# yflyl613/Tiny-NewsRec

Measured on NVIDIA B200. Metric: kd_train_impressions_per_sec, higher is better.
Workload: dtype bf16

## Files before the change

include/tinyrec.h:

```cpp
#ifndef TINYREC_H_
#define TINYREC_H_

#include <stdint.h>

#ifdef __cplusplus
extern "C" {
#endif

#define TNR_ABI_VERSION 6

const char* tnr_last_error(void);
int tnr_abi_version(void);
int tnr_device_check(int* num_sms);
int tnr_set_sm_reserve(int n_sms);
int tnr_host_copy_mt(void* dst, const void* src, long long bytes, int n_threads);

typedef struct {
  const unsigned long long* seed;
  unsigned int site;
  float p;
} tnr_dropout;

int tnr_dropout_mask(const tnr_dropout* drop, long long n, unsigned char* keep, void* stream);

enum { TNR_ACT_NONE = 0, TNR_ACT_GELU = 1, TNR_ACT_TANH = 2, TNR_ACT_DGELU = 3,
       TNR_ACT_GELU_DAUX = 4,
       TNR_ACT_MULAUX = 5 };
enum { TNR_BF16 = 0, TNR_F32 = 1 };

typedef struct {
  int M, N, K;
  const void* A; int lda; int a_mn_major;
  const void* B; int ldb; int b_mn_major;
  void* C; int ldc; int c_dtype;
  const float* bias;
  const void* residual; int ldr;
  int act;
  void* aux; int ldaux;
  int split_k;
  int accumulate;
  const tnr_dropout* drop;
  float* colsum;
} tnr_gemm_args;
int tnr_gemm_bf16(const tnr_gemm_args* args, void* stream);

int tnr_embed_ln_fwd(const int64_t* ids, int ids_ld, int n_rows, int L, int vocab, const void* word,
                     int word_dtype, const float* pos, const float* type0, const float* gamma,
                     const float* beta, float eps, int E, void* out_bf16, const tnr_dropout* drop,
                     void* stream);

int tnr_layernorm_fwd(const void* x_bf16, int rows, int E, const float* gamma, const float* beta,
                      float eps, void* y_bf16, void* stream);
int tnr_layernorm_bwd(const void* dy_bf16, const void* x_bf16, int rows, int E, const float* gamma,
                      float eps, void* dx_bf16, float* dgamma, float* dbeta, void* dx_drop_bf16,
                      float* dsum, const tnr_dropout* drop, void* stream);
int tnr_colsum_bf16(const void* x_bf16, int rows, int cols, int ld, float* out, void* stream);

int tnr_attn_relpos_fwd(const void* qkv_bf16, const int64_t* mask, int mask_ld, const float* relbias,
                        void* ctx_bf16, int n_news, int L, int A, int E, const tnr_dropout* drop,
                        void* stream);
int tnr_attn_relpos_bwd(const void* qkv_bf16, const int64_t* mask, int mask_ld, const float* relbias,
                        const void* dctx_bf16, void* dqkv_bf16, float* dbias_qkv, float* workspace, int n_news,
                        int L, int A, int E, const tnr_dropout* drop, void* stream);

int tnr_attnpool_fwd(const void* x_bf16, const void* e_bf16, int ldq, int Q, const float* w2,
                     const float* b2, const float* mask, void* out_bf16, float* a_out, int n, int S,
                     int C, void* stream);
int tnr_attnpool_bwd(const void* x_bf16, const void* e_bf16, int ldq, int Q, const float* w2,
                     const float* a_in, const float* dout, void* dx_bf16, void* du_bf16, float* dw2,
                     float* db2, int n, int S, int C, void* stream);

int tnr_user_encoder_fwd(const float* vecs, const float* mask, const float* pad_doc, const float* W1,
                         const float* b1, const float* w2, const float* b2, int use_mask, float* user,
                         float* a_out, float* e_out, int B, int H, int D, int Q, void* stream);
typedef struct {
  const float *vecs, *pad_doc, *W1, *b1, *w2, *b2;
  float *user, *a_out, *e_out;
} tnr_user_encoder_io;
int tnr_user_encoder_fwd_multi(const tnr_user_encoder_io* enc, int n_enc, const float* mask, int use_mask,
                               int B, int H, int D, int Q, void* stream);
int tnr_user_encoder_fwd_gather(const float* table, long long n_rows, const int32_t* idx, const float* mask,
                                const float* pad_doc, const float* W1, const float* b1, const float* w2,
                                const float* b2, int use_mask, float* user, float* a_out, int B, int H, int D,
                                int Q, void* stream);
long long tnr_user_encoder_packed_w1_floats(int D);
int tnr_user_encoder_pack_w1(const float* W1, const float* pad_doc, const float* b1, const float* w2, float* packed,
                             int D, int Q, void* stream);
long long tnr_user_encoder_score_ws_bytes(int B, int H);
int tnr_user_encoder_score(const float* vecs, long long n_rows, const int32_t* idx, const float* mask,
                           const float* pad_doc, const float* w1_packed, const float* b1, const float* w2,
                           const float* b2, int use_mask, float* user, float* a_out, void* workspace, int B,
                           int H, int D, int Q, void* stream);
int tnr_user_encoder_bwd(const float* vecs, const float* mask, const float* pad_doc, const float* W1,
                         const float* w2, int use_mask, const float* a_in, const float* e_in,
                         const float* d_user, float* d_vecs, float* dpad, float* dW1, float* db1,
                         float* dw2, float* db2, float* scratch, int B, int H, int D, int Q, void* stream);

int tnr_kd_loss_fwdbwd(const float* s_news, const float* s_user, const int64_t* label,
                       const float* T_ext, const float* TP_ext, int M, int B, int H, int K, int D,
                       float temperature, float coef, int want_grad, float* score_out, float* losses,
                       float* d_news, float* d_user, float* G_ext, void* stream);

int tnr_sgemm_nt(const float* A, const float* B, const float* bias, float* C, int M, int N, int K,
                 int batch, long long sA, long long sB, long long sbias, long long sC, void* stream);
int tnr_sgemm_tn_acc(const float* A, const float* B, float* C, float* cbias, int R, int N1, int N2,
                     int batch, long long sA, long long sB, long long sC, long long sbias, void* stream);

int tnr_nrms_blend_fwd(const float* vecs, const float* mask, const float* pad_doc, float* out, int rows, int D,
                       void* stream);
int tnr_nrms_blend_bwd(const float* d_blend, const float* mask, float* d_vecs, float* dpad, int rows, int D,
                       void* stream);
int tnr_nrms_attn_fwd(const float* q, const float* k, const float* v, const float* mask, float* ctx, int B, int H,
                      int n_heads, void* stream);
int tnr_nrms_attn_bwd(const float* q, const float* k, const float* v, const float* mask, const float* d_ctx,
                      float* dq, float* dk, float* dv, int B, int H, int n_heads, void* stream);
int tnr_sgemm_nn(const float* A, const float* B, float* C, int M, int N, int K, int parts, long long sA,
                 long long sB, void* stream);

int tnr_adam_amsgrad(float* p, const float* g, float* m, float* v, float* vmax, void* shadow_bf16,
                     long long n, float lr, float beta1, float beta2, float eps, int step,
                     float grad_scale, void* stream);
int tnr_adam_amsgrad_devstep(float* p, const float* g, float* m, float* v, float* vmax, void* shadow_bf16,
                             long long n, float lr, float beta1, float beta2, float eps, int* step_dev,
                             float* bc_ws, float grad_scale, int advance, void* stream);
int tnr_cast_f32_bf16(const float* x, void* y_bf16, long long n, void* stream);

long long tnr_allreduce_p2p_flag_words(void);
int tnr_allreduce_p2p(void* const* ptrs_dev, void* multicast_ptr, void* const* flags_dev, int rank, int world,
                      long long off, long long n, int n_ctas, void* stream);

int tnr_gather_rows_i32_i64(const int32_t* table, long long n_rows_table, const int32_t* idx,
                            long long n, int W, int64_t* out, void* stream);
int tnr_train_batch_gather(const int32_t* news, long long n_rows, int W, const float* const* teacher_tables,
                           float* const* teacher_out, int M, int D, long long out_ld, const int32_t* hist_idx,
                           long long n_hist, const int32_t* cand_idx, long long n_cand, long long* tokens_out,
                           void* stream);
int tnr_gather_rows_f32(const float* table, long long n_rows_table, const int32_t* idx, long long n,
                        int D, float* out, long long out_ld, void* stream);

int tnr_eval_metrics(const float* table, long long n_rows, const float* user, const long long* ptr,
                     const int32_t* cand, const int8_t* label, long long n_imp, long long nnz, int D, int max_c,
                     double* per_imp, double* sums, float* scores, void* stream);

int tnr_doc_sim(const float* table, long long n_rows, const int32_t* pairs, long long n_pairs, int D,
                double* sum_out, void* stream);

#ifdef __cplusplus
}
#endif
#endif
```

tiny-newsrec_b200/_lib.py:

```python
import ctypes
import os
from ctypes import POINTER, Structure, c_char_p, c_float, c_int, c_int64, c_uint, c_void_p

PKG = os.path.dirname(os.path.abspath(__file__))
LIB_PATH = os.path.join(PKG, "libtinyrec.so")

ACT_NONE, ACT_GELU, ACT_TANH, ACT_DGELU, ACT_GELU_DAUX, ACT_MULAUX = 0, 1, 2, 3, 4, 5
BF16, F32 = 0, 1


class TinyRecError(RuntimeError):
    pass


class Dropout(Structure):
    _fields_ = [("seed", c_void_p), ("site", c_uint), ("p", c_float)]


class UserEncoderIO(Structure):
    _fields_ = [(n, c_void_p) for n in ("vecs", "pad_doc", "W1", "b1", "w2", "b2", "user", "a_out", "e_out")]


class GemmArgs(Structure):
    _fields_ = [("M", c_int), ("N", c_int), ("K", c_int),
                ("A", c_void_p), ("lda", c_int), ("a_mn_major", c_int),
                ("B", c_void_p), ("ldb", c_int), ("b_mn_major", c_int),
                ("C", c_void_p), ("ldc", c_int), ("c_dtype", c_int),
                ("bias", c_void_p),
                ("residual", c_void_p), ("ldr", c_int),
                ("act", c_int),
                ("aux", c_void_p), ("ldaux", c_int),
                ("split_k", c_int),
                ("accumulate", c_int),
                ("drop", POINTER(Dropout)),
                ("colsum", c_void_p)]


P = c_void_p
_SIGNATURES = {
    "tnr_abi_version": ([], c_int),
    "tnr_device_check": ([POINTER(c_int)], c_int),
    "tnr_set_sm_reserve": ([c_int], c_int),
    "tnr_host_copy_mt": ([P, P, c_int64, c_int], c_int),
    "tnr_allreduce_p2p_flag_words": ([], c_int64),
    "tnr_allreduce_p2p": ([P, P, P, c_int, c_int, c_int64, c_int64, c_int, P], c_int),
    "tnr_gemm_bf16": ([POINTER(GemmArgs), P], c_int),
    "tnr_dropout_mask": ([POINTER(Dropout), c_int64, P, P], c_int),
    "tnr_embed_ln_fwd": ([P, c_int, c_int, c_int, c_int, P, c_int, P, P, P, P, c_float, c_int, P, POINTER(Dropout), P], c_int),
    "tnr_layernorm_fwd": ([P, c_int, c_int, P, P, c_float, P, P], c_int),
    "tnr_layernorm_bwd": ([P, P, c_int, c_int, P, c_float, P, P, P, P, P, POINTER(Dropout), P], c_int),
    "tnr_colsum_bf16": ([P, c_int, c_int, c_int, P, P], c_int),
    "tnr_attn_relpos_fwd": ([P, P, c_int, P, P, c_int, c_int, c_int, c_int, POINTER(Dropout), P], c_int),
    "tnr_attn_relpos_bwd": ([P, P, c_int, P, P, P, P, P, c_int, c_int, c_int, c_int, POINTER(Dropout), P], c_int),
    "tnr_attnpool_fwd": ([P, P, c_int, c_int, P, P, P, P, P, c_int, c_int, c_int, P], c_int),
    "tnr_attnpool_bwd": ([P, P, c_int, c_int, P, P, P, P, P, P, P, c_int, c_int, c_int, P], c_int),
    "tnr_user_encoder_fwd": ([P, P, P, P, P, P, P, c_int, P, P, P, c_int, c_int, c_int, c_int, P], c_int),
    "tnr_user_encoder_fwd_multi": ([P, c_int, P, c_int, c_int, c_int, c_int, c_int, P], c_int),
    "tnr_user_encoder_fwd_gather": ([P, c_int64, P, P, P, P, P, P, P, c_int, P, P, c_int, c_int, c_int, c_int, P], c_int),
    "tnr_user_encoder_packed_w1_floats": ([c_int], c_int64),
    "tnr_user_encoder_pack_w1": ([P, P, P, P, P, c_int, c_int, P], c_int),
    "tnr_user_encoder_score_ws_bytes": ([c_int, c_int], c_int64),
    "tnr_user_encoder_score": ([P, c_int64, P, P, P, P, P, P, P, c_int, P, P, P, c_int, c_int, c_int, c_int, P], c_int),
    "tnr_user_encoder_bwd": ([P, P, P, P, P, c_int, P, P, P, P, P, P, P, P, P, P, c_int, c_int, c_int, c_int, P], c_int),
    "tnr_kd_loss_fwdbwd": ([P, P, P, P, P, c_int, c_int, c_int, c_int, c_int, c_float, c_float, c_int, P, P, P, P, P, P],
                           c_int),
    "tnr_sgemm_nt": ([P, P, P, P, c_int, c_int, c_int, c_int, c_int64, c_int64, c_int64, c_int64, P], c_int),
    "tnr_sgemm_tn_acc": ([P, P, P, P, c_int, c_int, c_int, c_int, c_int64, c_int64, c_int64, c_int64, P], c_int),
    "tnr_nrms_blend_fwd": ([P, P, P, P, c_int, c_int, P], c_int),
    "tnr_nrms_blend_bwd": ([P, P, P, P, c_int, c_int, P], c_int),
    "tnr_nrms_attn_fwd": ([P, P, P, P, P, c_int, c_int, c_int, P], c_int),
    "tnr_nrms_attn_bwd": ([P, P, P, P, P, P, P, P, c_int, c_int, c_int, P], c_int),
    "tnr_sgemm_nn": ([P, P, P, c_int, c_int, c_int, c_int, c_int64, c_int64, P], c_int),
    "tnr_adam_amsgrad": ([P, P, P, P, P, P, c_int64, c_float, c_float, c_float, c_float, c_int, c_float, P], c_int),
    "tnr_adam_amsgrad_devstep": ([P, P, P, P, P, P, c_int64, c_float, c_float, c_float, c_float, P, P, c_float, c_int, P], c_int),
    "tnr_cast_f32_bf16": ([P, P, c_int64, P], c_int),
    "tnr_gather_rows_i32_i64": ([P, c_int64, P, c_int64, c_int, P, P], c_int),
    "tnr_gather_rows_f32": ([P, c_int64, P, c_int64, c_int, P, c_int64, P], c_int),
    "tnr_train_batch_gather": ([P, c_int64, c_int, POINTER(c_void_p), POINTER(c_void_p), c_int, c_int, c_int64, P, c_int64, P,
                                c_int64, P, P], c_int),
    "tnr_doc_sim": ([P, c_int64, P, c_int64, c_int, P, P], c_int),
    "tnr_eval_metrics": ([P, c_int64, P, P, P, P, c_int64, c_int64, c_int, c_int, P, P, P, P], c_int),
}

_lib = None


def exported_names():
    return sorted(list(_SIGNATURES) + ["tnr_last_error"])


def load():
    global _lib
    if _lib is not None:
        return _lib
    if not os.path.exists(LIB_PATH):
        raise TinyRecError(
            f"{LIB_PATH} not found: build it with `python -c 'import __graft_entry__ as g; g.build()'` "
            "(nvcc, sm_100a). tiny-newsrec_b200 has no CPU or PyTorch fallback path.")
    lib = ctypes.CDLL(LIB_PATH)
    lib.tnr_last_error.argtypes = []
    lib.tnr_last_error.restype = c_char_p
    for name, (args, res) in _SIGNATURES.items():
        fn = getattr(lib, name)
        fn.argtypes = args
        fn.restype = res
    if lib.tnr_abi_version() != 6:
        raise TinyRecError("libtinyrec.so ABI version mismatch; rebuild")
    _lib = lib
    return lib


def check(rc, what):
    if rc != 0:
        msg = load().tnr_last_error().decode(errors="replace")
        raise TinyRecError(f"{what} failed (rc={rc}): {msg}")


_device_ok = set()


def require_device(index):
    if index in _device_ok:
        return
    n = c_int(0)
    check(load().tnr_device_check(ctypes.byref(n)), "tnr_device_check")
    _device_ok.add(index)
```

tiny-newsrec_b200/csrc/head_kernels.cu:

```cuda
#include "common.cuh"

namespace tnr {

constexpr int UE_THREADS = 1024;

constexpr int KD_MAXM = 8;
constexpr int KD_MAXK = 32;

__global__ void __launch_bounds__(UE_THREADS)
kd_loss_kernel(const float* __restrict__ s_news, const float* __restrict__ s_user, const int64_t* __restrict__ label,
               const float* __restrict__ T_ext, const float* __restrict__ TP_ext, int M, int B, int H, int K, int D,
               float temperature, float coef, int want_grad, float* __restrict__ score_out, float* __restrict__ losses,
               float* __restrict__ d_news, float* __restrict__ d_user, float* __restrict__ G_ext) {
  __shared__ float s_sc[KD_MAXK];
  __shared__ float s_tsc[KD_MAXM][KD_MAXK];
  __shared__ float s_w[KD_MAXM];
  __shared__ float s_ds[KD_MAXK];
  __shared__ float s_mse[KD_MAXM];
  __shared__ float s_part[KD_MAXM][UE_THREADS / 32];
  __shared__ int s_last;
  const int b = blockIdx.x, tid = threadIdx.x;
  const int warp = uniform_warp_id(), lane = tid & 31;
  const int R = B * (H + K);
  const size_t Rext = (size_t)R + B;
  const float* cand = s_news + ((size_t)B * H + (size_t)b * K) * D;
  const float* usr = s_user + (size_t)b * D;
  const long long lab_raw = label[b];
  const bool lab_bad = lab_raw < 0 || lab_raw >= (long long)K;
  const int lab = lab_bad ? 0 : (int)lab_raw;
  const float invB = 1.0f / (float)B;

  for (int item = warp; item < (1 + M) * K; item += UE_THREADS / 32) {
    const int i = item / K, k = item - i * K;
    const float *c, *u;
    if (i == 0) { c = cand + (size_t)k * D; u = usr; }
    else {
      const float* Ti = T_ext + (size_t)(i - 1) * Rext * D;
      c = Ti + ((size_t)B * H + (size_t)b * K + k) * D;
      u = Ti + ((size_t)R + b) * D;
    }
    float t = 0.f;
    for (int d = lane; d < D; d += 32) t = fmaf(c[d], u[d], t);
    t = warp_sum(t);
    if (lane == 0) { if (i == 0) s_sc[k] = t; else s_tsc[i - 1][k] = t; }
  }
  {
    float ne[KD_MAXM], ue[KD_MAXM];
#pragma unroll
    for (int i = 0; i < KD_MAXM; ++i) { ne[i] = 0.f; ue[i] = 0.f; }
    for (int idx = tid; idx < (H + K) * D; idx += UE_THREADS) {
      const int r = idx / D, d = idx - r * D;
      const size_t row = r < H ? (size_t)b * H + r : (size_t)B * H + (size_t)b * K + (r - H);
      const float sv = s_news[row * D + d];
#pragma unroll
      for (int i = 0; i < KD_MAXM; ++i)
        if (i < M) { const float diff = sv - TP_ext[((size_t)i * Rext + row) * D + d]; ne[i] = fmaf(diff, diff, ne[i]); }
    }
    for (int d = tid; d < D; d += UE_THREADS) {
      const float uv = usr[d];
#pragma unroll
      for (int i = 0; i < KD_MAXM; ++i)
        if (i < M) { const float diff = uv - TP_ext[((size_t)i * Rext + R + b) * D + d]; ue[i] = fmaf(diff, diff, ue[i]); }
    }
#pragma unroll
    for (int i = 0; i < KD_MAXM; ++i)
      if (i < M) {
        ne[i] = warp_sum(ne[i]);
        ue[i] = warp_sum(ue[i]);
        if (lane == 0) { s_part[i][warp] = ne[i] / (float)((H + K) * D) + ue[i] / (float)D; }
      }
    __syncthreads();
    if (tid < M) {
      float t = 0.f;
#pragma unroll
      for (int w = 0; w < UE_THREADS / 32; ++w) t += s_part[tid][w];
      s_mse[tid] = t;
    }
  }
  __syncthreads();
  if (tid == 0) {
    float mx = -INFINITY;
    for (int k = 0; k < K; ++k) mx = fmaxf(mx, s_sc[k]);
    float se = 0.f;
    for (int k = 0; k < K; ++k) se += expf(s_sc[k] - mx);
    const float lse = mx + logf(se);
    const float target = lab_bad ? __int_as_float(0x7fc00000) : lse - s_sc[lab];
    float distill = 0.f, emb = 0.f;
    float pT[KD_MAXK];
    for (int k = 0; k < K; ++k) pT[k] = 0.f;
    if (M > 0) {
      float tl[KD_MAXM];
      float mn = INFINITY;
      for (int i = 0; i < M; ++i) {
        float m2 = -INFINITY;
        for (int k = 0; k < K; ++k) m2 = fmaxf(m2, s_tsc[i][k]);
        float s2 = 0.f;
        for (int k = 0; k < K; ++k) s2 += expf(s_tsc[i][k] - m2);
        tl[i] = m2 + logf(s2) - s_tsc[i][lab];
        mn = fminf(mn, tl[i]);
      }
      float ws = 0.f;
      for (int i = 0; i < M; ++i) { s_w[i] = expf(-(tl[i] - mn)); ws += s_w[i]; }
      for (int i = 0; i < M; ++i) { s_w[i] /= ws; emb += s_w[i] * s_mse[i]; }
      float tmx = -INFINITY, smx = -INFINITY;
      float tsc[KD_MAXK];
      for (int k = 0; k < K; ++k) {
        float t = 0.f;
        for (int i = 0; i < M; ++i) t = fmaf(s_tsc[i][k], s_w[i], t);
        tsc[k] = t / temperature;
        tmx = fmaxf(tmx, tsc[k]);
        smx = fmaxf(smx, s_sc[k] / temperature);
      }
      float tsum = 0.f, ssum = 0.f;
      for (int k = 0; k < K; ++k) { pT[k] = expf(tsc[k] - tmx); tsum += pT[k]; ssum += expf(s_sc[k] / temperature - smx); }
      const float slse = smx + logf(ssum);
      for (int k = 0; k < K; ++k) {
        pT[k] /= tsum;
        distill -= pT[k] * (s_sc[k] / temperature - slse);
        s_ds[k] = (expf(s_sc[k] / temperature - slse) - pT[k]) / temperature;
      }
    } else {
      for (int k = 0; k < K; ++k) s_ds[k] = 0.f;
    }
    for (int k = 0; k < K; ++k)
      s_ds[k] = (s_ds[k] + coef * (expf(s_sc[k] - lse) - (k == lab ? 1.0f : 0.0f))) * invB;
    float* part = losses + 4 + 4 * (size_t)b;
    part[0] = distill; part[1] = emb; part[2] = target; part[3] = distill + coef * target + emb;
    __threadfence();
    unsigned int* ticket = reinterpret_cast<unsigned int*>(losses + 4 + 4 * (size_t)B);
    s_last = (atomicAdd(ticket, 1u) == (unsigned int)B - 1) ? 1 : 0;
  }
  __syncthreads();
  if (s_last && warp == 0) {
    __threadfence();
    float acc4[4] = {0.f, 0.f, 0.f, 0.f};
    for (int i = lane; i < B; i += 32) {
      const float4 v = __ldcg(reinterpret_cast<const float4*>(losses + 4) + i);
      acc4[0] += v.x; acc4[1] += v.y; acc4[2] += v.z; acc4[3] += v.w;
    }
#pragma unroll
    for (int c = 0; c < 4; ++c) acc4[c] = warp_sum(acc4[c]);
    if (lane == 0) {
      for (int c = 0; c < 4; ++c) losses[c] = acc4[c] * invB;
      *reinterpret_cast<unsigned int*>(losses + 4 + 4 * (size_t)B) = 0u;
    }
  }
  __syncthreads();
  for (int k = tid; k < K; k += UE_THREADS) score_out[(size_t)b * K + k] = s_sc[k];
  if (!want_grad) return;
  const float cne = 2.0f / (float)((H + K) * D) * invB;
  const float cue = 2.0f / (float)D * invB;
  for (int idx = tid; idx < (H + K) * D; idx += UE_THREADS) {
    const int r = idx / D, d = idx - r * D;
    const size_t row = r < H ? (size_t)b * H + r : (size_t)B * H + (size_t)b * K + (r - H);
    const float sv = s_news[row * D + d];
    float g = 0.f;
    for (int i = 0; i < M; ++i) {
      const float gi = s_w[i] * cne * (sv - TP_ext[((size_t)i * Rext + row) * D + d]);
      g += gi;
      G_ext[((size_t)i * Rext + row) * D + d] = -gi;
    }
    if (r >= H) g = fmaf(s_ds[r - H], usr[d], g);
    d_news[row * D + d] = g;
  }
  for (int d = tid; d < D; d += UE_THREADS) {
    float g = 0.f;
    for (int k = 0; k < K; ++k) g = fmaf(s_ds[k], cand[(size_t)k * D + d], g);
    for (int i = 0; i < M; ++i) {
      const float gi = s_w[i] * cue * (usr[d] - TP_ext[((size_t)i * Rext + R + b) * D + d]);
      g += gi;
      G_ext[((size_t)i * Rext + R + b) * D + d] = -gi;
    }
    d_user[(size_t)b * D + d] = g;
  }
}

}

using namespace tnr;

#define TNR_API extern "C" __attribute__((visibility("default")))

TNR_API int tnr_kd_loss_fwdbwd(const float* s_news, const float* s_user, const int64_t* label, const float* T_ext,
                               const float* TP_ext, int M, int B, int H, int K, int D, float temperature, float coef,
                               int want_grad, float* score_out, float* losses, float* d_news, float* d_user,
                               float* G_ext, void* stream) {
  TNR_REQUIRE(M >= 0 && M <= KD_MAXM, "tnr_kd_loss_fwdbwd: num_teachers %d out of range (0..%d)", M, KD_MAXM);
  TNR_REQUIRE(K >= 1 && K <= KD_MAXK, "tnr_kd_loss_fwdbwd: candidates per impression %d out of range (1..%d)", K, KD_MAXK);
  if (B == 0) return 0;
  kd_loss_kernel<<<B, UE_THREADS, 0, reinterpret_cast<cudaStream_t>(stream)>>>(
      s_news, s_user, label, T_ext, TP_ext, M, B, H, K, D, temperature, coef, want_grad, score_out, losses, d_news, d_user,
      G_ext);
  TNR_LAUNCH_CHECK();
  return 0;
}
```

tiny-newsrec_b200/csrc/misc_kernels.cu:

```cuda
#include "common.cuh"

#define TNR_API extern "C" __attribute__((visibility("default")))

namespace tnr {

__global__ void __launch_bounds__(256)
adam_amsgrad_kernel(float* __restrict__ p, const float* __restrict__ g, float* __restrict__ m, float* __restrict__ v,
                    float* __restrict__ vmax, __nv_bfloat16* __restrict__ shadow, long long n, float lr, float b1,
                    float b2, float eps, float bc1, float rsqrt_bc2, float grad_scale, const float* __restrict__ bc_dev) {
  const long long i4 = ((long long)blockIdx.x * blockDim.x + threadIdx.x) * 4;
  if (i4 >= n) return;
  if (bc_dev != nullptr) { bc1 = bc_dev[0]; rsqrt_bc2 = bc_dev[1]; }
  if (i4 + 4 <= n) {
    float4 pp = *reinterpret_cast<float4*>(p + i4);
    const float4 gg = *reinterpret_cast<const float4*>(g + i4);
    float4 mm = *reinterpret_cast<float4*>(m + i4);
    float4 vv = *reinterpret_cast<float4*>(v + i4);
    const bool ams = vmax != nullptr;
    float4 vx = ams ? *reinterpret_cast<float4*>(vmax + i4) : make_float4(0.f, 0.f, 0.f, 0.f);
    float* P = reinterpret_cast<float*>(&pp);
    const float* G = reinterpret_cast<const float*>(&gg);
    float* Mm = reinterpret_cast<float*>(&mm);
    float* V = reinterpret_cast<float*>(&vv);
    float* VX = reinterpret_cast<float*>(&vx);
#pragma unroll
    for (int k = 0; k < 4; ++k) {
      const float gr = G[k] * grad_scale;
      Mm[k] = b1 * Mm[k] + (1.0f - b1) * gr;
      V[k] = b2 * V[k] + (1.0f - b2) * gr * gr;
      VX[k] = fmaxf(VX[k], V[k]);
      P[k] -= (lr / bc1) * Mm[k] / (sqrtf(VX[k]) * rsqrt_bc2 + eps);
    }
    *reinterpret_cast<float4*>(p + i4) = pp;
    *reinterpret_cast<float4*>(m + i4) = mm;
    *reinterpret_cast<float4*>(v + i4) = vv;
    if (ams) *reinterpret_cast<float4*>(vmax + i4) = vx;
    if (shadow != nullptr) {
      uint2 o;
      o.x = pack_bf16(P[0], P[1]);
      o.y = pack_bf16(P[2], P[3]);
      *reinterpret_cast<uint2*>(shadow + i4) = o;
    }
  } else {
    for (long long i = i4; i < n; ++i) {
      const float gr = g[i] * grad_scale;
      m[i] = b1 * m[i] + (1.0f - b1) * gr;
      v[i] = b2 * v[i] + (1.0f - b2) * gr * gr;
      float vm = v[i];
      if (vmax != nullptr) { vm = fmaxf(vmax[i], v[i]); vmax[i] = vm; }
      p[i] -= (lr / bc1) * m[i] / (sqrtf(vm) * rsqrt_bc2 + eps);
      if (shadow != nullptr) shadow[i] = __float2bfloat16_rn(p[i]);
    }
  }
}

__global__ void __launch_bounds__(256)
cast_f32_bf16_kernel(const float* __restrict__ x, __nv_bfloat16* __restrict__ y, long long n) {
  const long long i4 = ((long long)blockIdx.x * blockDim.x + threadIdx.x) * 4;
  if (i4 >= n) return;
  if (i4 + 4 <= n && (((uintptr_t)(x + i4) & 15) == 0) && (((uintptr_t)(y + i4) & 7) == 0)) {
    const float4 a = *reinterpret_cast<const float4*>(x + i4);
    uint2 o;
    o.x = pack_bf16(a.x, a.y);
    o.y = pack_bf16(a.z, a.w);
    *reinterpret_cast<uint2*>(y + i4) = o;
  } else {
    for (long long i = i4; i < n && i < i4 + 4; ++i) y[i] = __float2bfloat16_rn(x[i]);
  }
}

constexpr int GI_ROWS = 4;
__global__ void __launch_bounds__(256)
gather_rows_i32_i64_kernel(const int32_t* __restrict__ table, long long n_rows_table, const int32_t* __restrict__ idx,
                           long long n, int W, int64_t* __restrict__ out) {
  const long long r0 = ((long long)blockIdx.x * 8 + uniform_warp_id()) * GI_ROWS;
  if (r0 >= n) return;
  const int lane = threadIdx.x & 31;
  long long src[GI_ROWS];
#pragma unroll
  for (int k = 0; k < GI_ROWS; ++k) {
    src[k] = r0 + k < n ? idx[r0 + k] : 0;
    if (src[k] < 0 || src[k] >= n_rows_table) src[k] = 0;
  }
  if ((W & 1) == 0) {
    for (int c = lane; c < (W >> 1); c += 32) {
      int2 v[GI_ROWS];
#pragma unroll
      for (int k = 0; k < GI_ROWS; ++k) v[k] = reinterpret_cast<const int2*>(table + src[k] * W)[c];
#pragma unroll
      for (int k = 0; k < GI_ROWS; ++k)
        if (r0 + k < n) reinterpret_cast<longlong2*>(out + (r0 + k) * W)[c] = make_longlong2((long long)v[k].x, (long long)v[k].y);
    }
  } else {
    for (int k = 0; k < GI_ROWS && r0 + k < n; ++k)
      for (int c = lane; c < W; c += 32) out[(r0 + k) * W + c] = (int64_t)table[src[k] * W + c];
  }
}

__global__ void __launch_bounds__(256)
gather_rows_f32_kernel(const float* __restrict__ table, long long n_rows_table, const int32_t* __restrict__ idx,
                       long long n, int D, float* __restrict__ out, long long out_ld) {
  const long long r = (long long)blockIdx.x * 8 + uniform_warp_id();
  if (r >= n) return;
  long long src = idx[r];
  if (src < 0 || src >= n_rows_table) src = 0;
  const int lane = threadIdx.x & 31;
  const float4* s = reinterpret_cast<const float4*>(table + src * D);
  float4* d = reinterpret_cast<float4*>(out + r * out_ld);
  for (int c = lane; c < D / 4; c += 32) d[c] = s[c];
}

constexpr int TB_MAX_TEACHERS = 8;
struct TrainBatchGather {
  const int32_t* news; long long n_rows; int W;
  const float* teacher[TB_MAX_TEACHERS]; float* teacher_out[TB_MAX_TEACHERS]; int M, D; long long out_ld;
  const int32_t *hist_idx, *cand_idx; long long n_hist, n_cand;
  long long* tokens_out;
};

__global__ void __launch_bounds__(256)
train_batch_gather_kernel(const __grid_constant__ TrainBatchGather g) {
  const long long r = (long long)blockIdx.x * 8 + uniform_warp_id();
  if (r >= g.n_hist + g.n_cand) return;
  const int lane = threadIdx.x & 31, job = blockIdx.y;
  long long src = r < g.n_hist ? g.hist_idx[r] : g.cand_idx[r - g.n_hist];
  if (src < 0 || src >= g.n_rows) src = 0;
  if (job == 0) {
    const int32_t* s = g.news + src * g.W;
    long long* d = g.tokens_out + r * g.W;
    for (int c = lane; c < g.W; c += 32) d[c] = (long long)s[c];
  } else {
    const float4* s = reinterpret_cast<const float4*>(g.teacher[job - 1] + src * g.D);
    float4* d = reinterpret_cast<float4*>(g.teacher_out[job - 1] + r * g.out_ld);
    for (int c = lane; c < g.D / 4; c += 32) d[c] = s[c];
  }
}

__global__ void __launch_bounds__(256)
doc_sim_kernel(const float* __restrict__ table, long long n_rows, const int32_t* __restrict__ pairs, long long n_pairs,
               int D, double* __restrict__ sum_out) {
  __shared__ double s_part[8];
  const int warp = uniform_warp_id(), lane = threadIdx.x & 31;
  const long long pidx = (long long)blockIdx.x * 8 + warp;
  double c = 0.0;
  if (pidx < n_pairs) {
    const long long i = pairs[2 * pidx], j = pairs[2 * pidx + 1];
    if (i != j && i >= 0 && j >= 0 && i < n_rows && j < n_rows) {
      const float4* a = reinterpret_cast<const float4*>(table + i * D);
      const float4* b = reinterpret_cast<const float4*>(table + j * D);
      float dot = 0.f, na = 0.f, nb = 0.f;
      for (int k = lane; k < D / 4; k += 32) {
        const float4 x = a[k], y = b[k];
        dot = fmaf(x.x, y.x, fmaf(x.y, y.y, fmaf(x.z, y.z, fmaf(x.w, y.w, dot))));
        na = fmaf(x.x, x.x, fmaf(x.y, x.y, fmaf(x.z, x.z, fmaf(x.w, x.w, na))));
        nb = fmaf(y.x, y.x, fmaf(y.y, y.y, fmaf(y.z, y.z, fmaf(y.w, y.w, nb))));
      }
      dot = warp_sum(dot); na = warp_sum(na); nb = warp_sum(nb);
      c = (double)(dot / (sqrtf(na) * sqrtf(nb)));
    }
  }
  if (lane == 0) s_part[warp] = c;
  __syncthreads();
  if (threadIdx.x == 0) {
    double t = 0.0;
#pragma unroll
    for (int w = 0; w < 8; ++w) t += s_part[w];
    atomicAdd(sum_out, t);
  }
}

__constant__ double c_disc[10] = {1.0, 0.6309297535714575, 0.5, 0.43067655807339306, 0.38685280723454163,
                                  0.3562071871080222, 0.3333333333333333, 0.31546487678572877, 0.3010299956639812,
                                  0.2890648263178879};

constexpr int ES_WARPS = 8;
constexpr int ES_CPW = 32;

template <int VPL>
__global__ void __launch_bounds__(ES_WARPS * 32)
eval_score_kernel(const float* __restrict__ table, long long n_rows, const float* __restrict__ user,
                  const long long* __restrict__ ptr, const int32_t* __restrict__ cand, long long n_imp, long long nnz,
                  float* __restrict__ score) {
  const int lane = threadIdx.x & 31, grp = lane >> 3, gl = lane & 7;
  const long long warp_global = (long long)blockIdx.x * ES_WARPS + uniform_warp_id();
  const long long n_items = (nnz + ES_CPW - 1) / ES_CPW;
  constexpr int D = 32 * VPL;
  for (long long item = warp_global; item < n_items; item += (long long)gridDim.x * ES_WARPS) {
    const long long c0 = item * ES_CPW;
    const long long ci = c0 + lane;
    long long row = 0, imp = 0;
    if (ci < nnz) {
      const long long v = cand[ci];
      row = (v >= 0 && v < n_rows) ? v : 0;
      long long lo = 0, hi = n_imp;
      while (hi - lo > 1) {
        const long long mid = (lo + hi) >> 1;
        if (__ldg(ptr + mid) <= ci) lo = mid; else hi = mid;
      }
      imp = lo;
    }
    float out = 0.f;
#pragma unroll 2
    for (int pass = 0; pass < ES_CPW / 4; ++pass) {
      const int src = pass * 4 + grp;
      const long long r = __shfl_sync(0xffffffffu, row, src);
      const long long b = __shfl_sync(0xffffffffu, imp, src);
      const bool live = c0 + src < nnz;
      const float4* xr = reinterpret_cast<const float4*>(table + r * D) + gl;
      const float4* ur = reinterpret_cast<const float4*>(user + b * D) + gl;
      float4 x[VPL], u[VPL];
#pragma unroll
      for (int v = 0; v < VPL; ++v) x[v] = live ? __ldg(xr + v * 8) : make_float4(0.f, 0.f, 0.f, 0.f);
#pragma unroll
      for (int v = 0; v < VPL; ++v) u[v] = live ? __ldg(ur + v * 8) : make_float4(0.f, 0.f, 0.f, 0.f);
      float t = 0.f;
#pragma unroll
      for (int v = 0; v < VPL; ++v)
        t = fmaf(x[v].x, u[v].x, fmaf(x[v].y, u[v].y, fmaf(x[v].z, u[v].z, fmaf(x[v].w, u[v].w, t))));
      t += __shfl_xor_sync(0xffffffffu, t, 1);
      t += __shfl_xor_sync(0xffffffffu, t, 2);
      t += __shfl_xor_sync(0xffffffffu, t, 4);
      const float mine = __shfl_sync(0xffffffffu, t, (lane & 3) * 8);
      if ((lane >> 2) == pass) out = mine;
    }
    if (ci < nnz) score[ci] = out;
  }
}

constexpr int ER_WARPS = 4;

__device__ __forceinline__ double shfl_xor_f64(double v, int o) {
  return __hiloint2double(__shfl_xor_sync(0xffffffffu, __double2hiint(v), o), __shfl_xor_sync(0xffffffffu, __double2loint(v), o));
}

__device__ __forceinline__ uint32_t order_key(float f) {
  const uint32_t u = __float_as_uint(f + 0.0f);
  return u ^ ((uint32_t)((int32_t)u >> 31) | 0x80000000u);
}

__global__ void __launch_bounds__(ER_WARPS * 32)
eval_rank_kernel(const float* __restrict__ score, const long long* __restrict__ ptr, const int8_t* __restrict__ label,
                 long long n_imp, int cap, double* __restrict__ out) {
  extern __shared__ __align__(16) float sm[];
  const int warp = uniform_warp_id(), lane = threadIdx.x & 31;
  const int wpb = blockDim.x >> 5;
  const long long b = (long long)blockIdx.x * wpb + warp;
  if (b >= n_imp) return;
  uint32_t* s_key = reinterpret_cast<uint32_t*>(sm) + (size_t)warp * cap;
  int* s_pos = reinterpret_cast<int*>(sm + (size_t)wpb * cap) + (size_t)warp * cap;
  int8_t* s_lab = reinterpret_cast<int8_t*>(sm + (size_t)2 * wpb * cap) + (size_t)warp * cap;
  const long long p0 = ptr[b];
  const int C = (int)(ptr[b + 1] - p0);
  const int C4 = (C + 3) & ~3;
  for (int c = lane; c < C4; c += 32) {
    if (c < C) {
      s_key[c] = order_key(score[p0 + c]);
      s_lab[c] = label[p0 + c];
    } else {
      s_key[c] = 0u;
      s_lab[c] = 1;
    }
  }
  __syncwarp();
  int P = 0;
  for (int c0 = 0; c0 < C; c0 += 32) {
    const int c = c0 + lane;
    const bool pos = c < C && s_lab[c] != 0;
    const unsigned bal = __ballot_sync(0xffffffffu, pos);
    if (pos) s_pos[P + __popc(bal & ((1u << lane) - 1u))] = c;
    P += __popc(bal);
  }
  __syncwarp();
  const int N = C - P;
  if (P == 0 || N == 0) {
    if (lane < 5) out[(size_t)b * 5 + lane] = 0.0;
    return;
  }
  long long auc2 = 0;
  double mrr = 0.0, d5 = 0.0, d10 = 0.0;
  const int G4 = C4 >> 2;
  for (int k0 = 0; k0 < P; k0 += 32) {
    const int np = min(32, P - k0);
    int slots = 1;
    while (slots < np) slots <<= 1;
    const int nseg = 32 / slots, slot = lane & (slots - 1), seg = lane / slots;
    const bool have = slot < np;
    const int c = have ? s_pos[k0 + slot] : 0;
    const uint32_t kc = have ? s_key[c] : 0xffffffffu;
    int above = 0, lt = 0, eq = 0;
    for (int g = seg; g < G4; g += nseg) {
      const uint4 k4 = *reinterpret_cast<const uint4*>(s_key + 4 * g);
      const uint32_t l4 = *reinterpret_cast<const uint32_t*>(s_lab + 4 * g);
      const uint32_t kj[4] = {k4.x, k4.y, k4.z, k4.w};
#pragma unroll
      for (int u = 0; u < 4; ++u) {
        const int neg = ((l4 >> (8 * u)) & 0xffu) == 0u;
        const int gt = kj[u] > kc, e = kj[u] == kc;
        above += gt | (e & (int)(4 * g + u > c));
        lt += neg & (int)(kj[u] < kc);
        eq += neg & e;
      }
    }
    for (int o = slots; o < 32; o <<= 1) {
      above += __shfl_xor_sync(0xffffffffu, above, o);
      lt += __shfl_xor_sync(0xffffffffu, lt, o);
      eq += __shfl_xor_sync(0xffffffffu, eq, o);
    }
    if (have && seg == 0) {
      const int rank = above + 1;
      auc2 += 2 * lt + eq;
      mrr += 1.0 / (double)rank;
      if (rank <= 10) {
        const double disc = c_disc[rank - 1];
        if (rank <= 5) d5 += disc;
        d10 += disc;
      }
    }
  }
#pragma unroll
  for (int o = 16; o > 0; o >>= 1) {
    auc2 += __shfl_xor_sync(0xffffffffu, auc2, o);
    mrr += shfl_xor_f64(mrr, o);
    d5 += shfl_xor_f64(d5, o);
    d10 += shfl_xor_f64(d10, o);
  }
  if (lane == 0) {
    double i5 = 0.0, i10 = 0.0;
    for (int r = 1; r <= min(P, 10); ++r) {
      const double disc = c_disc[r - 1];
      if (r <= 5) i5 += disc;
      i10 += disc;
    }
    out[(size_t)b * 5 + 0] = 0.5 * (double)auc2 / ((double)P * (double)N);
    out[(size_t)b * 5 + 1] = mrr / (double)P;
    out[(size_t)b * 5 + 2] = d5 / i5;
    out[(size_t)b * 5 + 3] = d10 / i10;
    out[(size_t)b * 5 + 4] = 1.0;
  }
}

__global__ void __launch_bounds__(256)
eval_reduce_kernel(const double* __restrict__ per_imp, long long n, double* __restrict__ sums) {
  double acc[5] = {0, 0, 0, 0, 0};
  for (long long i = (long long)blockIdx.x * blockDim.x + threadIdx.x; i < n; i += (long long)gridDim.x * blockDim.x)
#pragma unroll
    for (int k = 0; k < 5; ++k) acc[k] += per_imp[i * 5 + k];
#pragma unroll
  for (int k = 0; k < 5; ++k) {
    double v = acc[k];
#pragma unroll
    for (int o = 16; o > 0; o >>= 1) v += __shfl_xor_sync(0xffffffffu, v, o);
    if ((threadIdx.x & 31) == 0) atomicAdd(sums + k, v);
  }
}

__global__ void __launch_bounds__(256)
dropout_mask_kernel(const tnr_dropout drop, long long n, unsigned char* __restrict__ keep) {
  const DropCfg dc = load_drop(drop);
  const long long g = (long long)blockIdx.x * blockDim.x + threadIdx.x;
  if (g * 8 >= n) return;
  const uint32_t m = dc.thr16 != 0 ? dropout_keep8(dc, (uint64_t)g) : 0xffu;
  for (int e = 0; e < 8 && g * 8 + e < n; ++e) keep[g * 8 + e] = (m >> e) & 1u;
}

}

using namespace tnr;

TNR_API int tnr_dropout_mask(const tnr_dropout* drop, long long n, unsigned char* keep, void* stream) {
  if (n == 0) return 0;
  const long long groups = (n + 7) / 8;
  dropout_mask_kernel<<<(int)((groups + 255) / 256), 256, 0, reinterpret_cast<cudaStream_t>(stream)>>>(drop_or_none(drop), n, keep);
  TNR_LAUNCH_CHECK();
  return 0;
}

TNR_API int tnr_adam_amsgrad(float* p, const float* g, float* m, float* v, float* vmax, void* shadow_bf16, long long n,
                             float lr, float beta1, float beta2, float eps, int step, float grad_scale, void* stream) {
  TNR_REQUIRE(step >= 1, "tnr_adam_amsgrad: step must be >= 1");
  if (n == 0) return 0;
  const double bc1 = 1.0 - pow((double)beta1, (double)step);
  const double bc2 = 1.0 - pow((double)beta2, (double)step);
  const long long threads = (n + 3) / 4;
  const int grid = (int)((threads + 255) / 256);
  adam_amsgrad_kernel<<<grid, 256, 0, reinterpret_cast<cudaStream_t>(stream)>>>(
      p, g, m, v, vmax, reinterpret_cast<__nv_bfloat16*>(shadow_bf16), n, lr, beta1, beta2, eps, (float)bc1,
      (float)(1.0 / sqrt(bc2)), grad_scale, nullptr);
  TNR_LAUNCH_CHECK();
  return 0;
}

__global__ void adam_step_prep_kernel(int* __restrict__ step_dev, float* __restrict__ bc, float b1, float b2) {
  const int step = ++(*step_dev);
  bc[0] = (float)(1.0 - pow((double)b1, (double)step));
  bc[1] = (float)(1.0 / sqrt(1.0 - pow((double)b2, (double)step)));
}

TNR_API int tnr_adam_amsgrad_devstep(float* p, const float* g, float* m, float* v, float* vmax, void* shadow_bf16,
                                     long long n, float lr, float beta1, float beta2, float eps, int* step_dev,
                                     float* bc_ws, float grad_scale, int advance, void* stream) {
  TNR_REQUIRE(step_dev != nullptr && bc_ws != nullptr, "tnr_adam_amsgrad_devstep: step_dev (int32) and bc_ws (2 floats) are required");
  cudaStream_t st = reinterpret_cast<cudaStream_t>(stream);
  if (advance) {
    adam_step_prep_kernel<<<1, 1, 0, st>>>(step_dev, bc_ws, beta1, beta2);
    TNR_LAUNCH_CHECK();
  }
  if (n == 0) return 0;
  const long long threads = (n + 3) / 4;
  const int grid = (int)((threads + 255) / 256);
  adam_amsgrad_kernel<<<grid, 256, 0, st>>>(p, g, m, v, vmax, reinterpret_cast<__nv_bfloat16*>(shadow_bf16), n, lr, beta1,
                                            beta2, eps, 1.0f, 1.0f, grad_scale, bc_ws);
  TNR_LAUNCH_CHECK();
  return 0;
}

TNR_API int tnr_cast_f32_bf16(const float* x, void* y_bf16, long long n, void* stream) {
  if (n == 0) return 0;
  const long long threads = (n + 3) / 4;
  cast_f32_bf16_kernel<<<(int)((threads + 255) / 256), 256, 0, reinterpret_cast<cudaStream_t>(stream)>>>(
      x, reinterpret_cast<__nv_bfloat16*>(y_bf16), n);
  TNR_LAUNCH_CHECK();
  return 0;
}

TNR_API int tnr_gather_rows_i32_i64(const int32_t* table, long long n_rows_table, const int32_t* idx, long long n, int W,
                                    int64_t* out, void* stream) {
  if (n == 0) return 0;
  gather_rows_i32_i64_kernel<<<(int)((n + 8 * GI_ROWS - 1) / (8 * GI_ROWS)), 256, 0, reinterpret_cast<cudaStream_t>(stream)>>>(
      table, n_rows_table, idx, n, W, out);
  TNR_LAUNCH_CHECK();
  return 0;
}

TNR_API int tnr_gather_rows_f32(const float* table, long long n_rows_table, const int32_t* idx, long long n, int D,
                                float* out, long long out_ld, void* stream) {
  TNR_REQUIRE(D % 4 == 0 && out_ld % 4 == 0, "tnr_gather_rows_f32: D and out_ld must be multiples of 4");
  if (n == 0) return 0;
  gather_rows_f32_kernel<<<(int)((n + 7) / 8), 256, 0, reinterpret_cast<cudaStream_t>(stream)>>>(table, n_rows_table, idx,
                                                                                                  n, D, out, out_ld);
  TNR_LAUNCH_CHECK();
  return 0;
}

TNR_API int tnr_train_batch_gather(const int32_t* news, long long n_rows, int W, const float* const* teacher_tables,
                                   float* const* teacher_out, int M, int D, long long out_ld, const int32_t* hist_idx,
                                   long long n_hist, const int32_t* cand_idx, long long n_cand, long long* tokens_out,
                                   void* stream) {
  TNR_REQUIRE(M >= 0 && M <= TB_MAX_TEACHERS, "tnr_train_batch_gather: at most %d teacher tables (got %d)", TB_MAX_TEACHERS, M);
  TNR_REQUIRE(M == 0 || (D % 4 == 0 && out_ld % 4 == 0 && teacher_tables != nullptr && teacher_out != nullptr),
              "tnr_train_batch_gather: D and out_ld must be multiples of 4");
  TNR_REQUIRE(news != nullptr && tokens_out != nullptr && n_rows >= 1 && W >= 1, "tnr_train_batch_gather: token table / output required");
  if (n_hist + n_cand == 0) return 0;
  TrainBatchGather g;
  g.news = news; g.n_rows = n_rows; g.W = W; g.M = M; g.D = D; g.out_ld = out_ld;
  for (int i = 0; i < TB_MAX_TEACHERS; ++i) {
    g.teacher[i] = i < M ? teacher_tables[i] : nullptr;
    g.teacher_out[i] = i < M ? teacher_out[i] : nullptr;
  }
  g.hist_idx = hist_idx; g.cand_idx = cand_idx; g.n_hist = n_hist; g.n_cand = n_cand; g.tokens_out = tokens_out;
  const dim3 grid((unsigned)((n_hist + n_cand + 7) / 8), (unsigned)(1 + M));
  train_batch_gather_kernel<<<grid, 256, 0, reinterpret_cast<cudaStream_t>(stream)>>>(g);
  TNR_LAUNCH_CHECK();
  return 0;
}

TNR_API int tnr_doc_sim(const float* table, long long n_rows, const int32_t* pairs, long long n_pairs, int D,
                        double* sum_out, void* stream) {
  TNR_REQUIRE(D % 4 == 0 && D > 0, "tnr_doc_sim: D=%d must be a positive multiple of 4", D);
  TNR_REQUIRE(sum_out != nullptr, "tnr_doc_sim: sum_out (one double, caller-initialised) is required");
  if (n_pairs == 0) return 0;
  doc_sim_kernel<<<(int)((n_pairs + 7) / 8), 256, 0, reinterpret_cast<cudaStream_t>(stream)>>>(table, n_rows, pairs, n_pairs, D,
                                                                                             sum_out);
  TNR_LAUNCH_CHECK();
  return 0;
}

template <int VPL>
static void eval_score_launch(int grid, cudaStream_t st, const float* table, long long n_rows, const float* user,
                              const long long* ptr, const int32_t* cand, long long n_imp, long long nnz, float* score) {
  eval_score_kernel<VPL><<<grid, ES_WARPS * 32, 0, st>>>(table, n_rows, user, ptr, cand, n_imp, nnz, score);
}

TNR_API int tnr_eval_metrics(const float* table, long long n_rows, const float* user, const long long* ptr,
                             const int32_t* cand, const int8_t* label, long long n_imp, long long nnz, int D, int max_c,
                             double* per_imp, double* sums, float* scores, void* stream) {
  TNR_REQUIRE(D % 32 == 0 && D >= 32 && D <= 512, "tnr_eval_metrics: D=%d must be a multiple of 32 in 32..512", D);
  TNR_REQUIRE(scores != nullptr || nnz == 0, "tnr_eval_metrics: scores fp32 [nnz] is required (output and workspace)");
  TNR_REQUIRE(n_rows >= 1, "tnr_eval_metrics: empty table");
  if (n_imp == 0) return 0;
  cudaStream_t st = reinterpret_cast<cudaStream_t>(stream);
  if (nnz > 0) {
    const long long items = (nnz + ES_CPW - 1) / ES_CPW;
    long long blocks = (items + ES_WARPS - 1) / ES_WARPS;
    const long long cap_blocks = (long long)num_sms() * 8;
    const int grid = (int)(blocks < cap_blocks ? blocks : cap_blocks);
    switch (D / 32) {
      case 1: eval_score_launch<1>(grid, st, table, n_rows, user, ptr, cand, n_imp, nnz, scores); break;
      case 2: eval_score_launch<2>(grid, st, table, n_rows, user, ptr, cand, n_imp, nnz, scores); break;
      case 4: eval_score_launch<4>(grid, st, table, n_rows, user, ptr, cand, n_imp, nnz, scores); break;
      case 8: eval_score_launch<8>(grid, st, table, n_rows, user, ptr, cand, n_imp, nnz, scores); break;
      case 16: eval_score_launch<16>(grid, st, table, n_rows, user, ptr, cand, n_imp, nnz, scores); break;
      default:
        set_error("tnr_eval_metrics: D=%d not instantiated (32, 64, 128, 256, 512)", D);
        return 1;
    }
    TNR_LAUNCH_CHECK();
  }
  const int cap = ((max_c > 1 ? max_c : 1) + 15) / 16 * 16;
  int wpb = ER_WARPS;
  while (wpb > 1 && (size_t)wpb * cap * 9 > 160 * 1024) wpb >>= 1;
  const size_t smem = (size_t)wpb * cap * 9;
  TNR_REQUIRE(smem <= 200 * 1024, "tnr_eval_metrics: max candidates %d too large", max_c);
  if (smem > 48 * 1024) TNR_SET_SMEM(eval_rank_kernel, smem);
  eval_rank_kernel<<<(unsigned)((n_imp + wpb - 1) / wpb), wpb * 32, smem, st>>>(scores, ptr, label, n_imp, cap, per_imp);
  TNR_LAUNCH_CHECK();
  if (sums != nullptr) {
    int grid = (int)((n_imp + 255) / 256);
    if (grid > 592) grid = 592;
    eval_reduce_kernel<<<grid, 256, 0, st>>>(per_imp, n_imp, sums);
    TNR_LAUNCH_CHECK();
  }
  return 0;
}
```

tiny-newsrec_b200/csrc/norm_kernels.cu:

```cuda
#include "common.cuh"
#include <cstdlib>

namespace tnr {

constexpr int ROWS_PER_BLOCK = 8;
constexpr int LNF_ROWS = 3;

template <int VPL, bool WORD_BF16>
__device__ __forceinline__ void embed_load_row(bf16x8 (&raw)[VPL * (WORD_BF16 ? 1 : 2)], const void* __restrict__ word,
                                               long long id, int lane) {
  constexpr int E = VPL * 256;
#pragma unroll
  for (int v = 0; v < VPL; ++v) {
    const int col = (v * 32 + lane) * 8;
    if (WORD_BF16) {
      raw[v] = *reinterpret_cast<const bf16x8*>(reinterpret_cast<const __nv_bfloat16*>(word) + (size_t)id * E + col);
    } else {
      const float* wp = reinterpret_cast<const float*>(word) + (size_t)id * E + col;
      raw[2 * v] = *reinterpret_cast<const bf16x8*>(wp);
      raw[2 * v + 1] = *reinterpret_cast<const bf16x8*>(wp + 4);
    }
  }
}

// ... 51 lines not shown
            w2 = pk2(bf16_lo(u), bf16_hi(u));
          } else {
            const bf16x8& rr = (k ? raw1 : raw0)[2 * v + (i >> 1)];
            w2 = pk2(__uint_as_float(rr.u[(i & 1) * 2]), __uint_as_float(rr.u[(i & 1) * 2 + 1]));
          }
          x[v * 4 + i] = add2(w2, pt[v * 4 + i]);
          s2 = add2(s2, x[v * 4 + i]);
        }
      float s0, s1;
      upk2(s2, s0, s1);
      const float mean = warp_sum(s0 + s1) * (1.0f / E);
      const f32x2 nmean2 = pk2(-mean, -mean);
      f32x2 q2 = pk2(0.f, 0.f);
#pragma unroll
      for (int i = 0; i < VPL * 4; ++i) { const f32x2 d = add2(x[i], nmean2); q2 = fma2(d, d, q2); }
      upk2(q2, s0, s1);
      const float rstd = rsqrtf(warp_sum(s0 + s1) * (1.0f / E) + eps);
      const f32x2 rstd2 = pk2(rstd, rstd), nmr2 = pk2(-mean * rstd, -mean * rstd);
      const size_t t = (size_t)n * L + l;
#pragma unroll
      for (int v = 0; v < VPL; ++v) {
        const int col = (v * 32 + lane) * 8;
        f32x2 yv[4];
#pragma unroll
        for (int i = 0; i < 4; ++i) yv[i] = fma2(fma2(x[v * 4 + i], rstd2, nmr2), g[v * 4 + i], bt[v * 4 + i]);
        if (dc.thr16 != 0) {
          f32x2 m[4];
          dropout_mul8(dc, ((uint64_t)t * (uint64_t)E + (uint64_t)col) >> 3, m);
#pragma unroll
          for (int i = 0; i < 4; ++i) yv[i] = mul2(yv[i], m[i]);
        }
        bf16x8 o;
#pragma unroll
        for (int i = 0; i < 4; ++i) { float lo, hi; upk2(yv[i], lo, hi); o.u[i] = pack_bf16(lo, hi); }
        *reinterpret_cast<bf16x8*>(out + t * E + col) = o;
      }
    }
  }
}

template <int VPL>
__global__ void __launch_bounds__(ROWS_PER_BLOCK * 32)
layernorm_fwd_kernel(const __nv_bfloat16* __restrict__ x, int rows, const float* __restrict__ gamma,
                     const float* __restrict__ beta, float eps, __nv_bfloat16* __restrict__ y, int reverse) {
  constexpr int E = VPL * 256;
  constexpr int NR = LNF_ROWS;
  const int warp = uniform_warp_id(), lane = threadIdx.x & 31;
  f32x2 g[VPL * 4], bt[VPL * 4];
#pragma unroll
  for (int v = 0; v < VPL; ++v) {
    const int col = (v * 32 + lane) * 8;
#pragma unroll
    for (int h = 0; h < 2; ++h) {
      const float4 gg = *reinterpret_cast<const float4*>(gamma + col + 4 * h);
      const float4 bb = *reinterpret_cast<const float4*>(beta + col + 4 * h);
      g[v * 4 + 2 * h] = pk2(gg.x, gg.y); g[v * 4 + 2 * h + 1] = pk2(gg.z, gg.w);
      bt[v * 4 + 2 * h] = pk2(bb.x, bb.y); bt[v * 4 + 2 * h + 1] = pk2(bb.z, bb.w);
    }
  }
  const int stride = gridDim.x * ROWS_PER_BLOCK;
  for (int r0 = blockIdx.x * ROWS_PER_BLOCK + warp; r0 < rows; r0 += NR * stride) {
    bf16x8 raw[NR][VPL];
#pragma unroll
    for (int k = 0; k < NR; ++k) {
      const int rk = r0 + k * stride;
      if (rk < rows) {
        const int a = reverse ? rows - 1 - rk : rk;
#pragma unroll
        for (int v = 0; v < VPL; ++v) raw[k][v] = *reinterpret_cast<const bf16x8*>(x + (size_t)a * E + (v * 32 + lane) * 8);
      }
    }
#pragma unroll
    for (int k = 0; k < NR; ++k) {
      const int rk = r0 + k * stride;
      if (rk >= rows) break;
      const int r = reverse ? rows - 1 - rk : rk;
      f32x2 xv[VPL * 4];
      f32x2 s2 = pk2(0.f, 0.f);
#pragma unroll
      for (int v = 0; v < VPL; ++v)
#pragma unroll
        for (int i = 0; i < 4; ++i) {
          xv[v * 4 + i] = pk2(bf16_lo(raw[k][v].u[i]), bf16_hi(raw[k][v].u[i]));
          s2 = add2(s2, xv[v * 4 + i]);
        }
      float s0, s1;
      upk2(s2, s0, s1);
      const float mean = warp_sum(s0 + s1) * (1.0f / E);
      const f32x2 nmean2 = pk2(-mean, -mean);
      f32x2 q2 = pk2(0.f, 0.f);
#pragma unroll
      for (int i = 0; i < VPL * 4; ++i) { const f32x2 d = add2(xv[i], nmean2); q2 = fma2(d, d, q2); }
      upk2(q2, s0, s1);
      const float rstd = rsqrtf(warp_sum(s0 + s1) * (1.0f / E) + eps);
      const f32x2 rstd2 = pk2(rstd, rstd), nmr2 = pk2(-mean * rstd, -mean * rstd);
#pragma unroll
      for (int v = 0; v < VPL; ++v) {
        bf16x8 o;
#pragma unroll
        for (int i = 0; i < 4; ++i) {
          float lo, hi;
          upk2(fma2(fma2(xv[v * 4 + i], rstd2, nmr2), g[v * 4 + i], bt[v * 4 + i]), lo, hi);
          o.u[i] = pack_bf16(lo, hi);
        }
        *reinterpret_cast<bf16x8*>(y + (size_t)r * E + (v * 32 + lane) * 8) = o;
      }
    }
  }
}

__device__ __forceinline__ void ln_cp_async16(void* smem_dst, const void* src) {
  const uint32_t dst = (uint32_t)__cvta_generic_to_shared(smem_dst);
  asm volatile("cp.async.cg.shared.global [%0], [%1], 16;" ::"r"(dst), "l"(src) : "memory");
}

constexpr int LNB_WARPS = 12;
constexpr int LNB_STAGES = 3;

template <int VPL>
__global__ void __launch_bounds__(LNB_WARPS * 32, 1)
layernorm_bwd_kernel(const __nv_bfloat16* __restrict__ dy, const __nv_bfloat16* __restrict__ x, int rows,
                     const float* __restrict__ gamma, float eps, __nv_bfloat16* __restrict__ dx,
                     float* __restrict__ dgamma, float* __restrict__ dbeta, __nv_bfloat16* __restrict__ dx_drop,
                     float* __restrict__ dsum, const tnr_dropout drop) {
  constexpr int E = VPL * 256;
  extern __shared__ __align__(16) uint8_t ln_smem[];
  const DropCfg dc = load_drop(drop);
  const int warp = uniform_warp_id(), lane = threadIdx.x & 31;
  __nv_bfloat16* stage = reinterpret_cast<__nv_bfloat16*>(ln_smem) + (size_t)warp * LNB_STAGES * 2 * E;
  f32x2 gm[VPL * 4], acc_dg[VPL * 4], acc_db[VPL * 4], acc_ds[VPL * 4];
#pragma unroll
  for (int v = 0; v < VPL; ++v) {
    const int col = (v * 32 + lane) * 8;
    const float4 g0 = __ldg(reinterpret_cast<const float4*>(gamma + col));
    const float4 g1 = __ldg(reinterpret_cast<const float4*>(gamma + col + 4));
    gm[v * 4 + 0] = pk2(g0.x, g0.y); gm[v * 4 + 1] = pk2(g0.z, g0.w);
    gm[v * 4 + 2] = pk2(g1.x, g1.y); gm[v * 4 + 3] = pk2(g1.z, g1.w);
  }
#pragma unroll
  for (int i = 0; i < VPL * 4; ++i) { acc_dg[i] = pk2(0.f, 0.f); acc_db[i] = pk2(0.f, 0.f); acc_ds[i] = pk2(0.f, 0.f); }
  const int stride = gridDim.x * LNB_WARPS;
  auto prefetch = [&](int st, int r) {
    if (r < rows) {
      __nv_bfloat16* sx = stage + st * 2 * E;
#pragma unroll
      for (int v = 0; v < VPL; ++v) {
        const int col = (v * 32 + lane) * 8;
        ln_cp_async16(sx + col, x + (size_t)r * E + col);
        ln_cp_async16(sx + E + col, dy + (size_t)r * E + col);
      }
    }
    asm volatile("cp.async.commit_group;" ::: "memory");
  };
  int r = blockIdx.x * LNB_WARPS + warp;
#pragma unroll
  for (int i = 0; i < LNB_STAGES - 1; ++i) prefetch(i, r + i * stride);
  int st = 0;
  for (; r < rows; r += stride) {
    int st2 = st + LNB_STAGES - 1; if (st2 >= LNB_STAGES) st2 -= LNB_STAGES;
    prefetch(st2, r + (LNB_STAGES - 1) * stride);
    asm volatile("cp.async.wait_group %0;" ::"n"(LNB_STAGES - 1) : "memory");
    __syncwarp();
    bf16x8 rx[VPL], rd[VPL];
    {
      const __nv_bfloat16* sx = stage + st * 2 * E;
#pragma unroll
      for (int v = 0; v < VPL; ++v) {
        rx[v] = *reinterpret_cast<const bf16x8*>(sx + (v * 32 + lane) * 8);
        rd[v] = *reinterpret_cast<const bf16x8*>(sx + E + (v * 32 + lane) * 8);
      }
    }
    __syncwarp();
    if (++st == LNB_STAGES) st = 0;
    const float shift = __shfl_sync(0xffffffffu, bf16_lo(rx[0].u[0]), 0);
    const f32x2 nshift2 = pk2(-shift, -shift);
    f32x2 s2 = pk2(0.f, 0.f), q2 = pk2(0.f, 0.f);
#pragma unroll
    for (int v = 0; v < VPL; ++v)
#pragma unroll
      for (int i = 0; i < 4; ++i) {
        const f32x2 d = add2(pk2(bf16_lo(rx[v].u[i]), bf16_hi(rx[v].u[i])), nshift2);
        s2 = add2(s2, d);
        q2 = fma2(d, d, q2);
      }
    float s, q;
    { float a0, a1; upk2(s2, a0, a1); s = a0 + a1; upk2(q2, a0, a1); q = a0 + a1; }
#pragma unroll
    for (int o = 16; o > 0; o >>= 1) {
      s += __shfl_xor_sync(0xffffffffu, s, o);
      q += __shfl_xor_sync(0xffffffffu, q, o);
    }
    const float ms = s * (1.0f / E);
    const float mean = shift + ms;
    const float rstd = rsqrtf(fmaxf(q * (1.0f / E) - ms * ms, 0.f) + eps);
    const f32x2 rstd2 = pk2(rstd, rstd), nmr2 = pk2(-mean * rstd, -mean * rstd);
    f32x2 sg2 = pk2(0.f, 0.f), sgx2 = pk2(0.f, 0.f);
#pragma unroll
    for (int v = 0; v < VPL; ++v)
#pragma unroll
      for (int i = 0; i < 4; ++i) {
        const f32x2 xh = fma2(pk2(bf16_lo(rx[v].u[i]), bf16_hi(rx[v].u[i])), rstd2, nmr2);
        const f32x2 d = pk2(bf16_lo(rd[v].u[i]), bf16_hi(rd[v].u[i]));
        acc_dg[v * 4 + i] = fma2(d, xh, acc_dg[v * 4 + i]);
        acc_db[v * 4 + i] = add2(acc_db[v * 4 + i], d);
        const f32x2 gg = mul2(d, gm[v * 4 + i]);
        sg2 = add2(sg2, gg);
        sgx2 = fma2(gg, xh, sgx2);
      }
    float sg, sgx;
    { float a0, a1; upk2(sg2, a0, a1); sg = a0 + a1; upk2(sgx2, a0, a1); sgx = a0 + a1; }
#pragma unroll
    for (int o = 16; o > 0; o >>= 1) {
      sg += __shfl_xor_sync(0xffffffffu, sg, o);
      sgx += __shfl_xor_sync(0xffffffffu, sgx, o);
    }
    sg *= (1.0f / E);
    sgx *= (1.0f / E);
    const f32x2 c0 = pk2(-rstd * sg, -rstd * sg), c1 = pk2(-rstd * sgx, -rstd * sgx);
#pragma unroll
    for (int v = 0; v < VPL; ++v) {
      const int col = (v * 32 + lane) * 8;
      f32x2 o[4];
#pragma unroll
      for (int i = 0; i < 4; ++i) {
        const f32x2 xh = fma2(pk2(bf16_lo(rx[v].u[i]), bf16_hi(rx[v].u[i])), rstd2, nmr2);
        const f32x2 gg = mul2(pk2(bf16_lo(rd[v].u[i]), bf16_hi(rd[v].u[i])), gm[v * 4 + i]);
        o[i] = fma2(xh, c1, fma2(gg, rstd2, c0));
      }
      bf16x8 ob;
#pragma unroll
      for (int i = 0; i < 4; ++i) { float lo, hi; upk2(o[i], lo, hi); ob.u[i] = pack_bf16(lo, hi); }
      *reinterpret_cast<bf16x8*>(dx + (size_t)r * E + col) = ob;
      if (dc.thr16 != 0) {
        f32x2 m[4];
        dropout_mul8(dc, ((uint64_t)r * (uint64_t)E + (uint64_t)col) >> 3, m);
#pragma unroll
        for (int i = 0; i < 4; ++i) o[i] = mul2(o[i], m[i]);
#pragma unroll
        for (int i = 0; i < 4; ++i) { float lo, hi; upk2(o[i], lo, hi); ob.u[i] = pack_bf16(lo, hi); }
      }
      if (dx_drop != nullptr) *reinterpret_cast<bf16x8*>(dx_drop + (size_t)r * E + col) = ob;
#pragma unroll
      for (int i = 0; i < 4; ++i) acc_ds[v * 4 + i] = add2(acc_ds[v * 4 + i], o[i]);
    }
  }
  asm volatile("cp.async.wait_group 0;" ::: "memory");
  __syncwarp();
  static_assert(LNB_STAGES >= 3, "the ring doubles as the per-warp accumulator slot");
  {
    float* mine = reinterpret_cast<float*>(stage);
#pragma unroll
    for (int v = 0; v < VPL; ++v)
#pragma unroll
      for (int i = 0; i < 4; ++i) {
        const int col = (v * 32 + lane) * 8 + 2 * i;
        float lo, hi;
        upk2(acc_dg[v * 4 + i], lo, hi);
        *reinterpret_cast<float2*>(mine + col) = make_float2(lo, hi);
        upk2(acc_db[v * 4 + i], lo, hi);
        *reinterpret_cast<float2*>(mine + E + col) = make_float2(lo, hi);
        upk2(acc_ds[v * 4 + i], lo, hi);
        *reinterpret_cast<float2*>(mine + 2 * E + col) = make_float2(lo, hi);
      }
  }
  __syncthreads();
  const float* part0 = reinterpret_cast<const float*>(ln_smem);
  constexpr int PART_STRIDE = LNB_STAGES * 2 * E * 2 / 4;
  for (int i = threadIdx.x; i < 3 * E; i += blockDim.x) {
    if (i >= 2 * E && dsum == nullptr) break;
    float t = 0.f;
#pragma unroll
    for (int w = 0; w < LNB_WARPS; ++w) t += part0[w * PART_STRIDE + i];
    float* dst = i < E ? dgamma + i : (i < 2 * E ? dbeta + (i - E) : dsum + (i - 2 * E));
    atomicAdd(dst, t);
  }
}

__global__ void __launch_bounds__(256)
colsum_kernel(const __nv_bfloat16* __restrict__ x, int rows, int cols, int ld, float* __restrict__ out) {
  const int cgroup = threadIdx.x & 7;
  const int rlane = threadIdx.x >> 3;
  const int col = (blockIdx.x * 8 + cgroup) * 8;
  float acc[8];
#pragma unroll
  for (int i = 0; i < 8; ++i) acc[i] = 0.f;
  if (col < cols) {
    for (int r = blockIdx.y * 32 + rlane; r < rows; r += gridDim.y * 32) {
      float v[8];
      unpack8(*reinterpret_cast<const bf16x8*>(x + (size_t)r * ld + col), v);
#pragma unroll
      for (int i = 0; i < 8; ++i) acc[i] += v[i];
    }
  }
  __shared__ float red[32][65];
#pragma unroll
  for (int i = 0; i < 8; ++i) red[rlane][cgroup * 8 + i] = acc[i];
  __syncthreads();
  if (threadIdx.x < 64) {
    float s = 0.f;
#pragma unroll
    for (int r = 0; r < 32; ++r) s += red[r][threadIdx.x];
    const int c = blockIdx.x * 64 + threadIdx.x;
    if (c < cols) atomicAdd(out + c, s);
  }
}

}

using namespace tnr;

#define DISPATCH_VPL(E, CALL)                                   \
  switch ((E) / 256) {                                          \
    case 1: { constexpr int VPL = 1; CALL; break; }             \
    case 2: { constexpr int VPL = 2; CALL; break; }             \
    case 3: { constexpr int VPL = 3; CALL; break; }             \
    case 4: { constexpr int VPL = 4; CALL; break; }             \
    default: set_error("hidden size %d not supported (need 256/512/768/1024)", (E)); return 1; \
  }

extern "C" __attribute__((visibility("default"))) int tnr_embed_ln_fwd(const int64_t* ids, int ids_ld, int n_rows, int L, int vocab, const void* word,
                                int word_dtype, const float* pos, const float* type0, const float* gamma,
                                const float* beta, float eps, int E, void* out_bf16, const tnr_dropout* drop, void* stream) {
  TNR_REQUIRE(E % 256 == 0, "tnr_embed_ln_fwd: E=%d must be a multiple of 256", E);
  TNR_REQUIRE(n_rows >= 0 && L > 0, "tnr_embed_ln_fwd: bad shape");
  if (n_rows == 0) return 0;
  const long long want_warps = (long long)num_sms() * EMB_WARPS;
  int groups = (int)(want_warps / L);
  if (groups < 1) groups = 1;
  if (groups > n_rows) groups = n_rows;
  const int grid = (int)(((long long)groups * L + EMB_WARPS - 1) / EMB_WARPS);
  cudaStream_t st = reinterpret_cast<cudaStream_t>(stream);
  __nv_bfloat16* out = reinterpret_cast<__nv_bfloat16*>(out_bf16);
  if (word_dtype == TNR_BF16) {
    DISPATCH_VPL(E, (embed_ln_kernel<VPL, true><<<grid, EMB_WARPS * 32, 0, st>>>(
                        ids, ids_ld, L, n_rows, groups, vocab, word, pos, type0, gamma, beta, eps, out, drop_or_none(drop))));
  } else {
    DISPATCH_VPL(E, (embed_ln_kernel<VPL, false><<<grid, EMB_WARPS * 32, 0, st>>>(
                        ids, ids_ld, L, n_rows, groups, vocab, word, pos, type0, gamma, beta, eps, out, drop_or_none(drop))));
  }
  TNR_LAUNCH_CHECK();
  return 0;
}

extern "C" __attribute__((visibility("default"))) int tnr_layernorm_fwd(const void* x_bf16, int rows, int E, const float* gamma, const float* beta, float eps,
                                 void* y_bf16, void* stream) {
  if (rows == 0) return 0;
  int grid = (rows + 2 * ROWS_PER_BLOCK - 1) / (2 * ROWS_PER_BLOCK);
  const int cap_f = num_sms() * 2;
  if (grid > cap_f) grid = cap_f;
  cudaStream_t st = reinterpret_cast<cudaStream_t>(stream);
  const int reverse = 0;
  DISPATCH_VPL(E, (layernorm_fwd_kernel<VPL><<<grid, ROWS_PER_BLOCK * 32, 0, st>>>(
                      reinterpret_cast<const __nv_bfloat16*>(x_bf16), rows, gamma, beta, eps,
                      reinterpret_cast<__nv_bfloat16*>(y_bf16), reverse)));
  TNR_LAUNCH_CHECK();
  return 0;
}

extern "C" __attribute__((visibility("default"))) int tnr_layernorm_bwd(const void* dy_bf16, const void* x_bf16, int rows, int E, const float* gamma, float eps,
                                 void* dx_bf16, float* dgamma, float* dbeta, void* dx_drop_bf16, float* dsum,
                                 const tnr_dropout* drop, void* stream) {
  if (rows == 0) return 0;
  int grid = (rows + LNB_WARPS - 1) / LNB_WARPS;
  const int cap = num_sms();
  if (grid > cap) grid = cap;
  cudaStream_t st = reinterpret_cast<cudaStream_t>(stream);
  const int smem = LNB_WARPS * LNB_STAGES * 2 * E * 2;
  DISPATCH_VPL(E, (cudaFuncSetAttribute(layernorm_bwd_kernel<VPL>, cudaFuncAttributeMaxDynamicSharedMemorySize, smem)));
  DISPATCH_VPL(E, (layernorm_bwd_kernel<VPL><<<grid, LNB_WARPS * 32, smem, st>>>(
                      reinterpret_cast<const __nv_bfloat16*>(dy_bf16), reinterpret_cast<const __nv_bfloat16*>(x_bf16),
                      rows, gamma, eps, reinterpret_cast<__nv_bfloat16*>(dx_bf16), dgamma, dbeta,
                      reinterpret_cast<__nv_bfloat16*>(dx_drop_bf16), dsum, drop_or_none(drop))));
  TNR_LAUNCH_CHECK();
  return 0;
}

extern "C" __attribute__((visibility("default"))) int tnr_colsum_bf16(const void* x_bf16, int rows, int cols, int ld, float* out, void* stream) {
  TNR_REQUIRE(cols % 8 == 0 && ld % 8 == 0, "tnr_colsum_bf16: cols/ld must be multiples of 8");
  if (rows == 0) return 0;
  dim3 grid((cols + 63) / 64, 1);
  int gy = (num_sms() * 8) / (int)grid.x;
  if (gy < 1) gy = 1;
  const int max_gy = (rows + 31) / 32;
  grid.y = gy < max_gy ? gy : max_gy;
  colsum_kernel<<<grid, 256, 0, reinterpret_cast<cudaStream_t>(stream)>>>(
      reinterpret_cast<const __nv_bfloat16*>(x_bf16), rows, cols, ld, out);
  TNR_LAUNCH_CHECK();
  return 0;
}
```

tiny-newsrec_b200/csrc/pooling.cu:

```cuda
#include "common.cuh"

namespace tnr {

constexpr int POOL_SMAX = 512;
constexpr int PW_WARPS = 4;
constexpr int PW_THREADS = PW_WARPS * 32;
constexpr int PW_RING = 6;

__device__ __forceinline__ void pw_cp16(void* smem_dst, const void* src) {
  const uint32_t dst = (uint32_t)__cvta_generic_to_shared(smem_dst);
  asm volatile("cp.async.cg.shared.global [%0], [%1], 16;" ::"r"(dst), "l"(src) : "memory");
}
__device__ __forceinline__ void pw_commit() { asm volatile("cp.async.commit_group;" ::: "memory"); }
template <int N>
__device__ __forceinline__ void pw_wait() { asm volatile("cp.async.wait_group %0;" ::"n"(N) : "memory"); }

template <int VPL>
__global__ void __launch_bounds__(PW_THREADS)
attnpool_fwd_kernel(const __nv_bfloat16* __restrict__ x, const __nv_bfloat16* __restrict__ e, int ldq, int Q,
                    const float* __restrict__ w2, const float* __restrict__ b2, const float* __restrict__ mask,
                    __nv_bfloat16* __restrict__ out, float* __restrict__ a_out, int n_news, int S) {
  constexpr int C = VPL * 256;
  constexpr int ROW16 = (VPL + 1) * 32;
  extern __shared__ __align__(16) unsigned char pw_sm[];
  const int warp = uniform_warp_id(), lane = threadIdx.x & 31;
  const int n = blockIdx.x * PW_WARPS + warp;
  if (n >= n_news) return;
  bf16x8* ring = reinterpret_cast<bf16x8*>(pw_sm) + (size_t)warp * PW_RING * ROW16;
  float* s_a = reinterpret_cast<float*>(pw_sm + (size_t)PW_WARPS * PW_RING * ROW16 * 16) + warp * POOL_SMAX;
  const float bias2 = b2[0];
  const int q0 = lane * 8;
  const bool has_e = q0 < Q;
  float wv[8];
#pragma unroll
  for (int i = 0; i < 8; ++i) wv[i] = has_e ? w2[q0 + i] : 0.f;
  const __nv_bfloat16* xn = x + (size_t)n * S * C;
  const __nv_bfloat16* en = e + (size_t)n * S * ldq;
  auto issue = [&](int s, int slot) {
    if (s < S) {
      bf16x8* dst = ring + slot * ROW16;
#pragma unroll
      for (int v = 0; v < VPL; ++v) pw_cp16(dst + v * 32 + lane, xn + (size_t)s * C + (v * 32 + lane) * 8);
      if (has_e) pw_cp16(dst + VPL * 32 + lane, en + (size_t)s * ldq + q0);
    }
    pw_commit();
  };
#pragma unroll
  for (int s = 0; s < PW_RING; ++s) issue(s, s);
  float acc[VPL * 8];
#pragma unroll
  for (int i = 0; i < VPL * 8; ++i) acc[i] = 0.f;
  float asum = 0.f;
  int slot = 0;
  for (int s = 0; s < S; ++s) {
    pw_wait<PW_RING - 1>();
    const bf16x8* row = ring + slot * ROW16;
    float f[8];
    float d = 0.f;
    if (has_e) {
      unpack8(row[VPL * 32 + lane], f);
#pragma unroll
      for (int i = 0; i < 8; ++i) d = fmaf(f[i], wv[i], d);
    }
    for (int q = q0 + 256; q < Q; q += 256) {
      unpack8(*reinterpret_cast<const bf16x8*>(en + (size_t)s * ldq + q), f);
#pragma unroll
      for (int i = 0; i < 8; ++i) d = fmaf(f[i], w2[q + i], d);
    }
    bf16x8 xr[VPL];
#pragma unroll
    for (int v = 0; v < VPL; ++v) xr[v] = row[v * 32 + lane];
    issue(s + PW_RING, slot);
    slot = slot + 1 == PW_RING ? 0 : slot + 1;
    d = warp_sum(d);
    float al = __expf(d + bias2);
    if (mask != nullptr) al *= mask[(size_t)n * S + s];
    if (lane == 0) s_a[s] = al;
    asum += al;
#pragma unroll
    for (int v = 0; v < VPL; ++v) {
      unpack8(xr[v], f);
#pragma unroll
      for (int i = 0; i < 8; ++i) acc[v * 8 + i] = fmaf(al, f[i], acc[v * 8 + i]);
    }
  }
  pw_wait<0>();
  const float inv = 1.0f / (asum + 1e-8f);
  __syncwarp();
  for (int s = lane; s < S; s += 32) a_out[(size_t)n * S + s] = s_a[s] * inv;
#pragma unroll
  for (int v = 0; v < VPL; ++v) {
    float o[8];
#pragma unroll
    for (int i = 0; i < 8; ++i) o[i] = acc[v * 8 + i] * inv;
    *reinterpret_cast<bf16x8*>(out + (size_t)n * C + (v * 32 + lane) * 8) = pack8(o);
  }
}

template <int VPL>
__global__ void __launch_bounds__(PW_THREADS)
attnpool_bwd_kernel(const __nv_bfloat16* __restrict__ x, const __nv_bfloat16* __restrict__ e, int ldq, int Q,
                    const float* __restrict__ w2, const float* __restrict__ a_in, const float* __restrict__ dout,
                    __nv_bfloat16* __restrict__ dx, __nv_bfloat16* __restrict__ du, float* __restrict__ dw2,
                    float* __restrict__ db2, int n_news, int S) {
  constexpr int C = VPL * 256;
  constexpr int ROW16 = VPL * 32;
  extern __shared__ __align__(16) unsigned char pw_sm[];
  __shared__ float s_gw[PW_WARPS][256];
  __shared__ float s_gb[PW_WARPS];
  const int warp = uniform_warp_id(), lane = threadIdx.x & 31;
  const int n = blockIdx.x * PW_WARPS + warp;
  const bool active = n < n_news;
  bf16x8* ring = reinterpret_cast<bf16x8*>(pw_sm) + (size_t)warp * PW_RING * ROW16;
  float* s_a = reinterpret_cast<float*>(pw_sm + (size_t)PW_WARPS * PW_RING * ROW16 * 16) + warp * 2 * POOL_SMAX;
  float* s_dz = s_a + POOL_SMAX;
  const int q0 = lane * 8;
  const bool has_e = q0 < Q;
  float gw[8];
#pragma unroll
  for (int i = 0; i < 8; ++i) gw[i] = 0.f;
  float gb = 0.f;
  if (active) {
    const __nv_bfloat16* xn = x + (size_t)n * S * C;
    const __nv_bfloat16* en = e + (size_t)n * S * ldq;
    __nv_bfloat16* dxn = dx + (size_t)n * S * C;
    __nv_bfloat16* dun = du + (size_t)n * S * ldq;
    for (int s = lane; s < S; s += 32) s_a[s] = a_in[(size_t)n * S + s];
    float dr[VPL * 8];
#pragma unroll
    for (int v = 0; v < VPL; ++v) {
      const float4 d0 = *reinterpret_cast<const float4*>(dout + (size_t)n * C + (v * 32 + lane) * 8);
      const float4 d1 = *reinterpret_cast<const float4*>(dout + (size_t)n * C + (v * 32 + lane) * 8 + 4);
      dr[v * 8 + 0] = d0.x; dr[v * 8 + 1] = d0.y; dr[v * 8 + 2] = d0.z; dr[v * 8 + 3] = d0.w;
      dr[v * 8 + 4] = d1.x; dr[v * 8 + 5] = d1.y; dr[v * 8 + 6] = d1.z; dr[v * 8 + 7] = d1.w;
    }
    __syncwarp();
    auto issue_x = [&](int s, int slot) {
      if (s < S) {
#pragma unroll
        for (int v = 0; v < VPL; ++v) pw_cp16(ring + slot * ROW16 + v * 32 + lane, xn + (size_t)s * C + (v * 32 + lane) * 8);
      }
      pw_commit();
    };
#pragma unroll
    for (int s = 0; s < PW_RING; ++s) issue_x(s, s);
    int slot = 0;
    for (int s = 0; s < S; ++s) {
      pw_wait<PW_RING - 1>();
      bf16x8 xr[VPL];
#pragma unroll
      for (int v = 0; v < VPL; ++v) xr[v] = ring[slot * ROW16 + v * 32 + lane];
      issue_x(s + PW_RING, slot);
      slot = slot + 1 == PW_RING ? 0 : slot + 1;
      const float a = s_a[s];
      float da = 0.f;
#pragma unroll
      for (int v = 0; v < VPL; ++v) {
        float f[8], o[8];
        unpack8(xr[v], f);
#pragma unroll
        for (int i = 0; i < 8; ++i) { da = fmaf(dr[v * 8 + i], f[i], da); o[i] = a * dr[v * 8 + i]; }
        *reinterpret_cast<bf16x8*>(dxn + (size_t)s * C + (v * 32 + lane) * 8) = pack8(o);
      }
      da = warp_sum(da);
      if (lane == 0) s_dz[s] = da;
    }
    pw_wait<0>();
    __syncwarp();
    float dot = 0.f;
    for (int s = lane; s < S; s += 32) dot = fmaf(s_a[s], s_dz[s], dot);
    dot = warp_sum(dot);
    for (int s = lane; s < S; s += 32) {
      const float dz = s_a[s] * (s_dz[s] - dot);
      s_dz[s] = dz;
      gb += dz;
    }
    __syncwarp();
    float wv[8];
#pragma unroll
    for (int i = 0; i < 8; ++i) wv[i] = has_e ? w2[q0 + i] : 0.f;
    auto issue_e = [&](int s, int sl) {
      if (s < S && has_e) pw_cp16(ring + sl * ROW16 + lane, en + (size_t)s * ldq + q0);
      pw_commit();
    };
#pragma unroll
    for (int s = 0; s < PW_RING; ++s) issue_e(s, s);
    slot = 0;
    for (int s = 0; s < S; ++s) {
      pw_wait<PW_RING - 1>();
      const float dz = s_dz[s];
      if (has_e) {
        float f[8], o[8];
        unpack8(ring[slot * ROW16 + lane], f);
#pragma unroll
        for (int i = 0; i < 8; ++i) {
          gw[i] = fmaf(dz, f[i], gw[i]);
          o[i] = dz * wv[i] * (1.0f - f[i] * f[i]);
        }
        *reinterpret_cast<bf16x8*>(dun + (size_t)s * ldq + q0) = pack8(o);
      }
      issue_e(s + PW_RING, slot);
      slot = slot + 1 == PW_RING ? 0 : slot + 1;
      for (int q = q0 + 256; q < Q; q += 256) {
        float f[8], o[8];
        unpack8(*reinterpret_cast<const bf16x8*>(en + (size_t)s * ldq + q), f);
#pragma unroll
        for (int i = 0; i < 8; ++i) {
          atomicAdd(dw2 + q + i, dz * f[i]);
          o[i] = dz * w2[q + i] * (1.0f - f[i] * f[i]);
        }
        *reinterpret_cast<bf16x8*>(dun + (size_t)s * ldq + q) = pack8(o);
      }
    }
    pw_wait<0>();
    gb = warp_sum(gb);
  }
#pragma unroll
  for (int i = 0; i < 8; ++i) s_gw[warp][q0 + i] = gw[i];
  if (lane == 0) s_gb[warp] = gb;
  __syncthreads();
  for (int q = threadIdx.x; q < min(Q, 256); q += PW_THREADS) {
    float t = 0.f;
#pragma unroll
    for (int w = 0; w < PW_WARPS; ++w) t += s_gw[w][q];
    atomicAdd(dw2 + q, t);
  }
  if (threadIdx.x == 0) {
    float t = 0.f;
#pragma unroll
    for (int w = 0; w < PW_WARPS; ++w) t += s_gb[w];
    atomicAdd(db2, t);
  }
}

}

using namespace tnr;

template <int VPL>
static int pool_fwd_launch(const void* x, const void* e, int ldq, int Q, const float* w2, const float* b2, const float* mask,
                           void* out, float* a_out, int n, int S, cudaStream_t st) {
  const int smem = PW_WARPS * (PW_RING * (VPL + 1) * 512 + POOL_SMAX * 4);
  TNR_SET_SMEM(attnpool_fwd_kernel<VPL>, smem);
  attnpool_fwd_kernel<VPL><<<(n + PW_WARPS - 1) / PW_WARPS, PW_THREADS, smem, st>>>(
      reinterpret_cast<const __nv_bfloat16*>(x), reinterpret_cast<const __nv_bfloat16*>(e), ldq, Q, w2, b2, mask,
      reinterpret_cast<__nv_bfloat16*>(out), a_out, n, S);
  TNR_LAUNCH_CHECK();
  return 0;
}

template <int VPL>
static int pool_bwd_launch(const void* x, const void* e, int ldq, int Q, const float* w2, const float* a_in, const float* dout,
                           void* dx, void* du, float* dw2, float* db2, int n, int S, cudaStream_t st) {
  const int smem = PW_WARPS * (PW_RING * VPL * 512 + 2 * POOL_SMAX * 4);
  TNR_SET_SMEM(attnpool_bwd_kernel<VPL>, smem);
  attnpool_bwd_kernel<VPL><<<(n + PW_WARPS - 1) / PW_WARPS, PW_THREADS, smem, st>>>(
      reinterpret_cast<const __nv_bfloat16*>(x), reinterpret_cast<const __nv_bfloat16*>(e), ldq, Q, w2, a_in, dout,
      reinterpret_cast<__nv_bfloat16*>(dx), reinterpret_cast<__nv_bfloat16*>(du), dw2, db2, n, S);
  TNR_LAUNCH_CHECK();
  return 0;
}

extern "C" __attribute__((visibility("default"))) int tnr_attnpool_fwd(const void* x_bf16, const void* e_bf16, int ldq, int Q, const float* w2, const float* b2,
                                const float* mask, void* out_bf16, float* a_out, int n, int S, int C, void* stream) {
  TNR_REQUIRE(S >= 1 && S <= POOL_SMAX, "tnr_attnpool_fwd: S=%d out of range (1..%d)", S, POOL_SMAX);
  TNR_REQUIRE(C % 256 == 0 && C <= 1024 && Q % 8 == 0 && ldq % 8 == 0,
              "tnr_attnpool_fwd: C must be 256/512/768/1024 and Q, ldq multiples of 8 (C=%d Q=%d ldq=%d)", C, Q, ldq);
  TNR_REQUIRE(((uintptr_t)x_bf16 | (uintptr_t)e_bf16 | (uintptr_t)out_bf16) % 16 == 0, "tnr_attnpool_fwd: 16-byte alignment required");
  if (n == 0) return 0;
  cudaStream_t st = reinterpret_cast<cudaStream_t>(stream);
  switch (C / 256) {
    case 1: return pool_fwd_launch<1>(x_bf16, e_bf16, ldq, Q, w2, b2, mask, out_bf16, a_out, n, S, st);
    case 2: return pool_fwd_launch<2>(x_bf16, e_bf16, ldq, Q, w2, b2, mask, out_bf16, a_out, n, S, st);
    case 3: return pool_fwd_launch<3>(x_bf16, e_bf16, ldq, Q, w2, b2, mask, out_bf16, a_out, n, S, st);
    default: return pool_fwd_launch<4>(x_bf16, e_bf16, ldq, Q, w2, b2, mask, out_bf16, a_out, n, S, st);
  }
}

extern "C" __attribute__((visibility("default"))) int tnr_attnpool_bwd(const void* x_bf16, const void* e_bf16, int ldq, int Q, const float* w2, const float* a_in,
                                const float* dout, void* dx_bf16, void* du_bf16, float* dw2, float* db2, int n, int S,
                                int C, void* stream) {
  TNR_REQUIRE(S >= 1 && S <= POOL_SMAX, "tnr_attnpool_bwd: S=%d out of range (1..%d)", S, POOL_SMAX);
  TNR_REQUIRE(C % 256 == 0 && C <= 1024 && Q % 8 == 0 && ldq % 8 == 0,
              "tnr_attnpool_bwd: C must be 256/512/768/1024 and Q, ldq multiples of 8 (C=%d Q=%d ldq=%d)", C, Q, ldq);
  TNR_REQUIRE(((uintptr_t)x_bf16 | (uintptr_t)e_bf16 | (uintptr_t)dx_bf16 | (uintptr_t)du_bf16 | (uintptr_t)dout) % 16 == 0,
              "tnr_attnpool_bwd: 16-byte alignment required");
  if (n == 0) return 0;
  cudaStream_t st = reinterpret_cast<cudaStream_t>(stream);
  switch (C / 256) {
    case 1: return pool_bwd_launch<1>(x_bf16, e_bf16, ldq, Q, w2, a_in, dout, dx_bf16, du_bf16, dw2, db2, n, S, st);
    case 2: return pool_bwd_launch<2>(x_bf16, e_bf16, ldq, Q, w2, a_in, dout, dx_bf16, du_bf16, dw2, db2, n, S, st);
    case 3: return pool_bwd_launch<3>(x_bf16, e_bf16, ldq, Q, w2, a_in, dout, dx_bf16, du_bf16, dw2, db2, n, S, st);
    default: return pool_bwd_launch<4>(x_bf16, e_bf16, ldq, Q, w2, a_in, dout, dx_bf16, du_bf16, dw2, db2, n, S, st);
  }
}
```

tiny-newsrec_b200/engine.py:

```python
import math

import torch

from . import ops
from ._lib import TinyRecError

BF = torch.bfloat16
F32 = torch.float32
LN_EPS = 1e-12

SITE_EMB = 0
KIND_ATTN, KIND_ATT_OUT, KIND_FFN_OUT = 0, 1, 2


def drop_site(layer, kind):
    return 8 * (layer + 1) + kind


class DropState:

    def __init__(self, device, p_hidden=0.1, p_attn=0.1, seed=None):
        self.p_hidden, self.p_attn = float(p_hidden), float(p_attn)
        if seed is None:
            seed = torch.initial_seed() & 0x7FFFFFFFFFFFFFFF
        self.seed = torch.tensor([seed], device=device, dtype=torch.int64)

    def advance(self):
        self.seed.add_(1)

    def make(self, site, p):
        return ops.make_drop(self.seed, site, p)

    def offset(self, site_base):
        return _DropView(self, site_base)


class _DropView:
    def __init__(self, state, site_base):
        self.p_hidden, self.p_attn, self.seed, self.site_base = state.p_hidden, state.p_attn, state.seed, int(site_base)

    def make(self, site, p):
        return ops.make_drop(self.seed, site + self.site_base, p)


def _align8(n):
    return (n + 7) // 8 * 8


def rel_pos_bucket_table(L, num_buckets=32, max_distance=128):
    pos = torch.arange(L)
    rel = pos[None, :] - pos[:, None]
    half = num_buckets // 2
    ret = (rel > 0).long() * half
    n = rel.abs()
    exact = half // 2
    big = exact + (torch.log(n.float() / exact) / math.log(max_distance / exact) * (half - exact)).to(torch.long)
    big = torch.min(big, torch.full_like(big, half - 1))
    return ret + torch.where(n < exact, n, big)


class LayerRefs:

    def __init__(self, layer):
        s, a = layer.attention.self, layer.attention.output
        self.q, self.k, self.v = s.query, s.key, s.value
        self.o, self.ln1 = a.dense, a.LayerNorm
        self.f1, self.f2, self.ln2 = layer.intermediate.dense, layer.output.dense, layer.output.LayerNorm

    def params(self):
        return [self.q.weight, self.k.weight, self.v.weight, self.q.bias, self.k.bias, self.v.bias,
                self.o.weight, self.o.bias, self.ln1.weight, self.ln1.bias,
                self.f1.weight, self.f1.bias, self.f2.weight, self.f2.bias, self.ln2.weight, self.ln2.bias]


class FlatParams:

    def __init__(self, ordered_params, device):
        self.params = ordered_params
        self.offsets = []
        off = 0
        for p in ordered_params:
            self.offsets.append(off)
            off += p.numel()
            off = _align8(off)
        self.numel = off
        self.data = torch.zeros(off, device=device, dtype=F32)
        self.symm, self.symm_error = None, None
        from . import parallel as _par
        if _par.SymmetricGradBuffer.wanted() and torch.device(device).type == "cuda":
            try:
                self.symm = _par.SymmetricGradBuffer(off, torch.device(device))
            except Exception as exc:
                self.symm, self.symm_error = None, f"{type(exc).__name__}: {exc}"
        self.grad = self.symm.grad if self.symm is not None else torch.zeros(off, device=device, dtype=F32)
        self.shadow = torch.zeros(off, device=device, dtype=BF)
        for p, o in zip(ordered_params, self.offsets):
            view = self.data[o:o + p.numel()].view(p.shape)
            view.copy_(p.data)
            p.data = view
            p.grad = self.grad[o:o + p.numel()].view(p.shape)
        self._index = {id(p): i for i, p in enumerate(ordered_params)}
        self.refresh_shadow()

    def refresh_shadow(self):
        ops.cast_f32_bf16(self.data, self.shadow)
        self.versions = [p._version for p in self.params]

    def stale(self):
        return any(p._version != v for p, v in zip(self.params, self.versions))

    def attached(self):
        for p, o in zip(self.params, self.offsets):
            if p.data_ptr() != self.data.data_ptr() + 4 * o:
                return False
        return True

    def reattach_grads(self):
        for p, o in zip(self.params, self.offsets):
            g = p.grad
            if g is None or g.data_ptr() != self.grad.data_ptr() + 4 * o:
                view = self.grad[o:o + p.numel()].view(p.shape)
                if g is None:
                    view.zero_()
                else:
                    view.copy_(g)
                p.grad = view

    def has(self, p):
        return id(p) in self._index

    def off(self, p):
        return self.offsets[self._index[id(p)]]

    def w_shadow(self, p, rows=None):
        o = self.off(p)
        n = p.numel() if rows is None else rows * p.shape[1]
        return self.shadow[o:o + n].view(-1, p.shape[1])

    def g_view(self, p, numel=None, shape=None):
        o = self.off(p)
        n = p.numel() if numel is None else numel
        v = self.grad[o:o + n]
        return v.view(shape) if shape is not None else v.view(p.shape) if numel is None else v


class _Frozen:

    def __init__(self):
        self.cache = {}

    def get(self, key, tensors, build):
        sig = tuple((t.data_ptr(), t._version) for t in tensors)
        hit = self.cache.get(key)
        if hit is not None and hit[0] == sig:
            return hit[1]
        val = build()
        self.cache[key] = (sig, val)
        return val


class Encoder:

    def __init__(self, news_encoder_module):
        self.mod = news_encoder_module
        bert = news_encoder_module.bert_model.bert
        self.bert = bert
        self.layers = [LayerRefs(l) for l in bert.encoder.layer]
        self.E = bert.embeddings.word_embeddings.weight.shape[1]
        self.A = bert.rel_pos_bias.weight.shape[0]
        self.F = self.layers[0].f1.weight.shape[0] if self.layers else 4 * self.E
        self.Q = news_encoder_module.attn.att_fc1.weight.shape[0]
        self.D = news_encoder_module.dense.weight.shape[0]
        cfg = getattr(news_encoder_module, "bert_config", None) or {}
        self.ln_eps = float(cfg.get("layer_norm_eps", LN_EPS))
        self.rel_bins = int(cfg.get("rel_pos_bins", 32))
        self.max_rel = int(cfg.get("max_rel_pos", 128))
        if bert.rel_pos_bias.weight.shape[1] != self.rel_bins:
            raise TinyRecError(f"rel_pos_bias has {bert.rel_pos_bias.weight.shape[1]} buckets, config says {self.rel_bins}")
        self.frozen = _Frozen()
        self.ws = {}
        self.scratch_ln = None

    def trainable_order(self):
        out = []
        for lr in self.layers:
            ps = lr.params()
            flags = [p.requires_grad for p in ps]
            if any(flags):
                if not all(flags):
                    raise TinyRecError("a BertLayer must be trainable or frozen as a whole (run.py:101-112 policy)")
                out += ps
        for p in (self.mod.attn.att_fc1.weight, self.mod.attn.att_fc1.bias, self.mod.attn.att_fc2.weight,
                  self.mod.attn.att_fc2.bias, self.mod.dense.weight, self.mod.dense.bias):
            if p.requires_grad:
                out.append(p)
        return out

    def lowest_trainable_layer(self):
        for i, lr in enumerate(self.layers):
            if lr.q.weight.requires_grad:
                return i
        return len(self.layers)

    def check_supported(self):
        emb = self.bert.embeddings
        for p in list(emb.parameters()) + [self.bert.rel_pos_bias.weight]:
            if p.requires_grad:
                raise TinyRecError(
                    "training the embeddings / rel_pos_bias is outside the supported hot path "
                    "(the reference freezes them, run.py:103-104); set requires_grad=False")

    def _w(self, flat, p):
        if flat is not None and flat.has(p):
            return flat.w_shadow(p)
        return self.frozen.get(("w", id(p)), [p], lambda: p.detach().to(BF).contiguous())

    def layer_weights(self, flat, i):
        lr = self.layers[i]
        if flat is not None and flat.has(lr.q.weight):
            E = self.E
            o = flat.off(lr.q.weight)
            wqkv = flat.shadow[o:o + 3 * E * E].view(3 * E, E)
            ob = flat.off(lr.q.bias)
            bqkv = flat.data[ob:ob + 3 * E]
        else:
            wqkv = self.frozen.get(("wqkv", i), [lr.q.weight, lr.k.weight, lr.v.weight],
                                   lambda: torch.cat([lr.q.weight, lr.k.weight, lr.v.weight], 0).detach().to(BF).contiguous())
            bqkv = self.frozen.get(("bqkv", i), [lr.q.bias, lr.k.bias, lr.v.bias],
                                   lambda: torch.cat([lr.q.bias, lr.k.bias, lr.v.bias], 0).detach().float().contiguous())
        return wqkv, bqkv, self._w(flat, lr.o.weight), self._w(flat, lr.f1.weight), self._w(flat, lr.f2.weight)

    def relpos(self, L):
        w = self.bert.rel_pos_bias.weight

        def build():
            tab = rel_pos_bucket_table(L, self.rel_bins, self.max_rel)
            vec = torch.cat([tab[1:, 0].flip(0), tab[0, :]])
            return w.detach().float()[:, vec.to(w.device)].contiguous()
        return self.frozen.get(("relpos", L), [w], build)

    def word_table(self):
        w = self.bert.embeddings.word_embeddings.weight
        return self.frozen.get(("word",), [w], lambda: w.detach().to(BF).contiguous())

    def workspace(self, n, L, n_saved_layers, dev, tag=None):
        key = (n, L, n_saved_layers, tag)
        ws = self.ws.get(key)
        if ws is not None:
            return ws
        T, E, Fd = n * L, self.E, self.F
        mk = lambda *s, dt=BF: torch.empty(*s, device=dev, dtype=dt)
        ws = dict(x0=mk(T, E), xa=mk(T, E), xb=mk(T, E), qkv=mk(T, 3 * E), ctx=mk(T, E), pre=mk(T, E), x1=mk(T, E),
                  h=mk(T, Fd), e=mk(T, self.Q), a=mk(n, L, dt=F32), pooled=mk(n, E), saved=[])
        for _ in range(n_saved_layers):
            ws["saved"].append(dict(xin=None, qkv=mk(T, 3 * E), ctx=mk(T, E), pre1=mk(T, E), x1=mk(T, E),
                                    z=mk(T, Fd), h=mk(T, Fd), pre2=mk(T, E), xout=mk(T, E)))
        if n_saved_layers:
            ws.update(dx=mk(T, E), dx2=mk(T, E), dpre=mk(T, E), dpre_drop=mk(T, E), dz=mk(T, Fd), dqkv=mk(T, 3 * E), dctx=mk(T, E),
                      du=mk(T, self.Q), dnews_bf=mk(n, self.D), dpooled=mk(n, E, dt=F32))
        if len(self.ws) > 8:
            self.ws.clear()
        self.ws[key] = ws
        return ws

    def forward(self, x, flat=None, save=False, out=None, drop=None, tag=None):
        if x.dtype != torch.int64 or x.dim() != 2 or x.shape[1] % 2:
            raise TinyRecError(f"news encoder input must be int64 [n, 2L], got {x.dtype} {tuple(x.shape)}")
        x = x.contiguous()
        n, L = x.shape[0], x.shape[1] // 2
        dev = x.device
        nl = len(self.layers)
        low = self.lowest_trainable_layer() if save else nl
        ws = self.workspace(n, L, nl - low if save else 0, dev, tag)
        emb = self.bert.embeddings
        relpos = self.relpos(L)
        cur = ws["x0"]
        dmk = (lambda site, p: drop.make(site, p)) if drop is not None else (lambda site, p: None)
        ph, pa = (drop.p_hidden, drop.p_attn) if drop is not None else (0.0, 0.0)
        ops.embed_ln(x, L, self.word_table(), emb.position_embeddings.weight, emb.token_type_embeddings.weight[0],
                     emb.LayerNorm.weight, emb.LayerNorm.bias, self.ln_eps, cur, drop=dmk(SITE_EMB, ph))
        for i, lr in enumerate(self.layers):
            wqkv, bqkv, wo, w1, w2 = self.layer_weights(flat, i)
            if i >= low:
                sv = ws["saved"][i - low]
                sv["xin"] = cur
                qkv, ctx, pre1, x1, h, pre2, xout, z = sv["qkv"], sv["ctx"], sv["pre1"], sv["x1"], sv["h"], sv["pre2"], sv["xout"], sv["z"]
            else:
                qkv, ctx, pre1, x1, h, pre2, z = ws["qkv"], ws["ctx"], ws["pre"], ws["x1"], ws["h"], ws["pre"], None
                xout = ws["xb"] if cur is ws["xa"] else ws["xa"]
            ops.gemm(cur, wqkv, qkv, bias=bqkv)
            ops.attn_fwd(qkv, x, L, relpos, ctx, self.A, drop=dmk(drop_site(i, KIND_ATTN), pa))
            ops.gemm(ctx, wo, pre1, bias=lr.o.bias, residual=cur, drop=dmk(drop_site(i, KIND_ATT_OUT), ph))
            ops.layernorm_fwd(pre1, lr.ln1.weight, lr.ln1.bias, self.ln_eps, x1)
            ops.gemm(x1, w1, h, bias=lr.f1.bias, act=ops.ACT_GELU_DAUX if z is not None else ops.ACT_GELU, aux=z)
            ops.gemm(h, w2, pre2, bias=lr.f2.bias, residual=x1, drop=dmk(drop_site(i, KIND_FFN_OUT), ph))
            ops.layernorm_fwd(pre2, lr.ln2.weight, lr.ln2.bias, self.ln_eps, xout)
            cur = xout
        at = self.mod.attn
        ops.gemm(cur, self._w(flat, at.att_fc1.weight), ws["e"], bias=at.att_fc1.bias, act=ops.ACT_TANH)
        ops.attnpool_fwd(cur, ws["e"], self.Q, at.att_fc2.weight.view(-1), at.att_fc2.bias, None, ws["pooled"], ws["a"], n, L)
        if out is None:
            out = torch.empty(n, self.D, device=dev, dtype=F32)
        ops.gemm(ws["pooled"], self._w(flat, self.mod.dense.weight), out, bias=self.mod.dense.bias)
        if save:
            ws["xlast"], ws["x"], ws["n"], ws["L"], ws["low"], ws["drop"] = cur, x, n, L, low, drop
        self.last_ws = ws
        return out

    def _splitk(self, M, N, K):
        tiles = ((M + 127) // 128) * ((N + (255 if N > 128 else 127)) // (256 if N > 128 else 128))
        sms = 148
        s = max(1, int(round(2.0 * sms / tiles)))
        return max(1, min(s, (K + 63) // 64 // 4 or 1))

    def _wgrad(self, flat, p, dy, xin, rows=None):
        M = dy.shape[1]
        g = flat.g_view(p) if rows is None else flat.grad[flat.off(p):flat.off(p) + rows * p.shape[1]].view(rows, p.shape[1])
        ops.gemm(dy, xin, g, a_t=True, b_t=True, split_k=self._splitk(M, xin.shape[1], dy.shape[0]), accumulate=True)

    def backward(self, d_news, flat, on_layer_done=None, ws=None, on_grads_ready=None):
        ws = self.last_ws if ws is None else ws
        n, L, low, x = ws["n"], ws["L"], ws["low"], ws["x"]
        drop = ws.get("drop")
        dmk = (lambda site, p: drop.make(site, p)) if drop is not None else (lambda site, p: None)
        ph, pa = (drop.p_hidden, drop.p_attn) if drop is not None else (0.0, 0.0)
        T, E = n * L, self.E
        nl = len(self.layers)
        at, dense = self.mod.attn, self.mod.dense
        if self.scratch_ln is None or self.scratch_ln.device != d_news.device:
            self.scratch_ln = torch.zeros(2 * E, device=d_news.device, dtype=F32)
        ops.cast_f32_bf16(d_news, ws["dnews_bf"])
        dnb = ws["dnews_bf"]
        if flat.has(dense.weight):
            self._wgrad(flat, dense.weight, dnb, ws["pooled"])
            ops.colsum(dnb, flat.g_view(dense.bias))
        ops.gemm(dnb, self._w(flat, dense.weight), ws["dpooled"], b_t=True)
        xl = ws["xlast"]
        if flat.has(at.att_fc1.weight):
            dw2, db2 = flat.g_view(at.att_fc2.weight).view(-1), flat.g_view(at.att_fc2.bias)
        else:
            dw2, db2 = self.scratch_ln[:self.Q], self.scratch_ln[E:E + 1]
        ops.attnpool_bwd(xl, ws["e"], self.Q, at.att_fc2.weight.view(-1), ws["a"], ws["dpooled"], ws["dx2"], ws["du"],
                         dw2, db2, n, L)
        if flat.has(at.att_fc1.weight):
            self._wgrad(flat, at.att_fc1.weight, ws["du"], xl)
            ops.colsum(ws["du"], flat.g_view(at.att_fc1.bias))
        if low >= nl:
            return
        dx = ws["dx"]
        ops.gemm(ws["du"], self._w(flat, at.att_fc1.weight), dx, b_t=True, residual=ws["dx2"])
        for i in range(nl - 1, low - 1, -1):
            lr, sv = self.layers[i], ws["saved"][i - low]
            train = flat.has(lr.q.weight)
            fine = train and i == low and on_grads_ready is not None
            wqkv, bqkv, wo, w1, w2 = self.layer_weights(flat, i)
            dpre, dz, dqkv, dctx, dx2 = ws["dpre"], ws["dz"], ws["dqkv"], ws["dctx"], ws["dx2"]
            sg, sb = (flat.g_view(lr.ln2.weight), flat.g_view(lr.ln2.bias)) if train else (self.scratch_ln[:E], self.scratch_ln[E:])
            d2 = dmk(drop_site(i, KIND_FFN_OUT), ph)
            dd = ws["dpre_drop"] if d2 is not None else dpre
            ops.layernorm_bwd(dx, sv["pre2"], lr.ln2.weight, self.ln_eps, dpre, sg, sb,
                              dx_drop=dd if d2 is not None else None, drop=d2,
                              dsum=flat.g_view(lr.f2.bias) if train else None)
            if train:
                self._wgrad(flat, lr.f2.weight, dd, sv["h"])
                if fine:
                    on_grads_ready(lr.f2.weight, lr.ln2.bias)
            ops.gemm(dd, w2, dz, b_t=True, act=ops.ACT_MULAUX, aux=sv["z"],
                     colsum=flat.g_view(lr.f1.bias) if train else None)
            if train:
                self._wgrad(flat, lr.f1.weight, dz, sv["x1"])
                if fine:
                    on_grads_ready(lr.f1.weight, lr.f1.bias)
            ops.gemm(dz, w1, dx2, b_t=True, residual=dpre)
            sg, sb = (flat.g_view(lr.ln1.weight), flat.g_view(lr.ln1.bias)) if train else (self.scratch_ln[:E], self.scratch_ln[E:])
            d1 = dmk(drop_site(i, KIND_ATT_OUT), ph)
            dd = ws["dpre_drop"] if d1 is not None else dpre
            ops.layernorm_bwd(dx2, sv["pre1"], lr.ln1.weight, self.ln_eps, dpre, sg, sb,
                              dx_drop=dd if d1 is not None else None, drop=d1,
                              dsum=flat.g_view(lr.o.bias) if train else None)
            if train and not fine:
                self._wgrad(flat, lr.o.weight, dd, sv["ctx"])
            ops.gemm(dd, wo, dctx, b_t=True)
            dbq = None
            if train:
                ob = flat.off(lr.q.bias)
                dbq = flat.grad[ob:ob + 3 * E]
            ops.attn_bwd(sv["qkv"], x, L, self.relpos(L), dctx, dqkv, self.A, drop=dmk(drop_site(i, KIND_ATTN), pa),
                         dbias=dbq)
            if train:
                self._wgrad(flat, lr.q.weight, dqkv, sv["xin"], rows=3 * E)
            if fine:
                on_grads_ready(lr.q.weight, lr.v.bias)
                self._wgrad(flat, lr.o.weight, dd, sv["ctx"])
                on_grads_ready(lr.o.weight, lr.ln1.bias)
            if i > low:
                ops.gemm(dqkv, wqkv, dx, b_t=True, residual=dpre)
            if on_layer_done is not None and train:
                on_layer_done(i)
```

tiny-newsrec_b200/model_bert.py:

```python
import json

import torch
from torch import nn

from . import ops
from ._lib import TinyRecError
from .engine import F32, DropState, Encoder, FlatParams, _align8
from .synth import BERT_BASE



class _Holder(nn.Module):
    def forward(self, *a, **k):
        raise TinyRecError(f"{type(self).__name__} is a parameter holder; compute goes through the CUDA engine")


def _bert_init(module, std):
    if isinstance(module, (nn.Linear, nn.Embedding)):
        module.weight.data.normal_(mean=0.0, std=std)
    elif isinstance(module, nn.LayerNorm):
        module.bias.data.zero_()
        module.weight.data.fill_(1.0)
    if isinstance(module, nn.Linear) and module.bias is not None:
        module.bias.data.zero_()


def load_bert_config(config_name, **over):
    cfg = dict(BERT_BASE, initializer_range=0.02)
    if config_name:
        with open(config_name, "r", encoding="utf-8") as f:
            cfg.update(json.load(f))
    cfg.update(over)
    return cfg


def _bert_layer(cfg):
    E, Fd, eps = cfg["hidden_size"], cfg["intermediate_size"], cfg["layer_norm_eps"]
    layer = _Holder()
    layer.attention = _Holder()
    layer.attention.self = _Holder()
    layer.attention.self.query = nn.Linear(E, E)
    layer.attention.self.key = nn.Linear(E, E)
    layer.attention.self.value = nn.Linear(E, E)
    layer.attention.output = _Holder()
    layer.attention.output.dense = nn.Linear(E, E)
    layer.attention.output.LayerNorm = nn.LayerNorm(E, eps=eps)
    layer.intermediate = _Holder()
    layer.intermediate.dense = nn.Linear(E, Fd)
    layer.output = _Holder()
    layer.output.dense = nn.Linear(Fd, E)
    layer.output.LayerNorm = nn.LayerNorm(E, eps=eps)
    return layer


def build_bert_model(cfg, num_layers):
    E = cfg["hidden_size"]
    m = _Holder()
    m.bert = _Holder()
    emb = _Holder()
    emb.word_embeddings = nn.Embedding(cfg["vocab_size"], E, padding_idx=0)
    emb.position_embeddings = nn.Embedding(cfg["max_position_embeddings"], E)
    emb.token_type_embeddings = nn.Embedding(cfg["type_vocab_size"], E)
    emb.LayerNorm = nn.LayerNorm(E, eps=cfg["layer_norm_eps"])
    m.bert.embeddings = emb
    m.bert.encoder = _Holder()
    m.bert.encoder.layer = nn.ModuleList([_bert_layer(cfg) for _ in range(num_layers)])
    m.bert.pooler = _Holder()
    m.bert.pooler.dense = nn.Linear(E, E)
    m.bert.rel_pos_bias = nn.Linear(cfg["rel_pos_bins"], cfg["num_attention_heads"], bias=False)
    m.classifier = nn.Linear(E, cfg.get("num_labels", 2))
    std = cfg.get("initializer_range", 0.02)
    m.apply(lambda mod: _bert_init(mod, std))
    return m


class AttentionPooling(nn.Module):

    def __init__(self, emb_size, hidden_size):
        super().__init__()
        self.att_fc1 = nn.Linear(emb_size, hidden_size)
        self.att_fc2 = nn.Linear(hidden_size, 1)

    def forward(self, x, attn_mask=None):
        B, S, C = x.shape
        x = x.contiguous().float()
        mask = torch.ones(B, S, device=x.device, dtype=F32) if attn_mask is None else attn_mask.contiguous().float()
        out = torch.empty(B, C, device=x.device, dtype=F32)
        a = torch.empty(B, S, device=x.device, dtype=F32)
        ops.user_encoder_fwd(x.view(B * S, C), mask, self.att_fc1.bias, self.att_fc1.weight, self.att_fc1.bias,
                             self.att_fc2.weight.view(-1), self.att_fc2.bias, True, out, a, None, B, S)
        return out


class NewsEncoder(nn.Module):

    def __init__(self, args, is_teacher=False, num_layers=None):
        super().__init__()
        if getattr(args, "pooling", "att") != "att":
            raise TinyRecError("only pooling='att' is on the supported hot path (demo.sh:28)")
        if getattr(args, "model_type", "tnlrv3") != "tnlrv3":
            raise TinyRecError("only model_type='tnlrv3' is supported (the reference's bert/roberta branch is broken)")
        if num_layers is None:
            num_layers = args.num_teacher_layers if is_teacher else args.num_student_layers
        self.pooling = args.pooling
        self.bert_config = load_bert_config(getattr(args, "config_name", None), num_hidden_layers=num_layers)
        self.bert_model = build_bert_model(self.bert_config, num_layers)
        model_name = getattr(args, "model_name", None)
        if model_name:
            import os
            from . import checkpoint
            if not os.path.isfile(model_name):
                raise TinyRecError(f"args.model_name={model_name!r} is not a file: pass the UniLM/TNLRv3 .bin the reference "
                                   "loads with from_pretrained, or model_name=None for a random-init encoder")
            missing, _ = checkpoint.load_unilm_bin(self.bert_model, model_name,
                                                   initializer_range=self.bert_config.get("initializer_range", 0.02))
            self.pretrained_missing_keys = missing
        self.attn = AttentionPooling(self.bert_config["hidden_size"], args.news_query_vector_dim)
        self.dense = nn.Linear(self.bert_config["hidden_size"], args.news_dim)
        self._engine = None
        self._flat = None
        self._drop = None

    def drop_state(self, device):
        if self._drop is None or self._drop.seed.device != device:
            c = self.bert_config
            self._drop = DropState(device, c.get("hidden_dropout_prob", 0.1), c.get("attention_probs_dropout_prob", 0.1))
        return self._drop

    def engine(self):
        if self._engine is None:
            self._engine = Encoder(self)
        return self._engine

    def forward(self, x, chunk=2048):
        if not x.is_cuda:
            raise TinyRecError("tinyrec NewsEncoder needs CUDA tensors (no CPU path)")
        eng = self.engine()
        flat = self._flat
        if flat is not None:
            if not flat.attached():
                flat = self._flat = None
            elif flat.stale():
                flat.refresh_shadow()
        n = x.shape[0]
        drop = None
        if self.training:
            drop = self.drop_state(x.device)
        out = torch.empty(n, eng.D, device=x.device, dtype=F32)
        for s in range(0, n, chunk):
            if drop is not None:
                drop.advance()
            eng.forward(x[s:s + chunk], flat, out=out[s:s + chunk], drop=drop)
        return out


class MultiHeadSelfAttention(_Holder):

    def __init__(self, d_model, n_heads, d_k, d_v):
        super().__init__()
        if d_k != 16 or d_v != 16:
            raise TinyRecError("NRMS self-attention: d_k = d_v = 16 (as the reference hard-wires, model_bert.py:146)")
        self.d_model, self.n_heads, self.d_k, self.d_v = d_model, n_heads, d_k, d_v
        self.W_Q = nn.Linear(d_model, d_k * n_heads)
        self.W_K = nn.Linear(d_model, d_k * n_heads)
        self.W_V = nn.Linear(d_model, d_v * n_heads)
        for m in (self.W_Q, self.W_K, self.W_V):
            nn.init.xavier_uniform_(m.weight, gain=1)

    def stacked(self):
        ws = [self.W_Q.weight, self.W_K.weight, self.W_V.weight]
        bs = [self.W_Q.bias, self.W_K.bias, self.W_V.bias]
        sw, sb = _const_stride(ws), _const_stride(bs)
        if sw is not None and sb is not None:
            return ws[0].detach(), bs[0].detach(), sw, sb
        Dh, D = ws[0].shape
        return (torch.stack([w.detach() for w in ws]).contiguous(), torch.stack([b.detach() for b in bs]).contiguous(),
                Dh * D, Dh)


def nrms_self_attention(mh, pad_doc, vecs, mask, use_mask, B, H, buf=None):
    R, D = vecs.shape
    Dh = mh.W_Q.weight.shape[0]
    dev = vecs.device
    buf = {} if buf is None else buf

    def get(name, *shape):
        t = buf.get(name)
        if t is None or tuple(t.shape) != shape:
            t = buf[name] = torch.empty(*shape, device=dev, dtype=F32)
        return t

    if use_mask:
        xb, pool_mask = vecs, mask
    else:
        xb = ops.nrms_blend_fwd(vecs, mask.reshape(-1), pad_doc.reshape(-1), get("xb", R, D))
        pool_mask = buf.get("ones")
        if pool_mask is None or tuple(pool_mask.shape) != (B, H):
            pool_mask = buf["ones"] = torch.ones(B, H, device=dev, dtype=F32)
    Wc, bc, sw, sb = mh.stacked()
    qkv = get("qkv", 3, R, Dh)
    ops.sgemm_nt(xb, Wc, bc, qkv, R, Dh, D, 3, 0, sw, sb, R * Dh)
    ctx = ops.nrms_attn_fwd(qkv, mask if use_mask else None, get("ctx", R, Dh), B, H)
    return dict(xb=xb, qkv=qkv, ctx=ctx, pool_mask=pool_mask, Wc=Wc, sw=sw)


class UserEncoder(nn.Module):

    def __init__(self, args):
        super().__init__()
        self.args = args
        self.nrms = getattr(args, "model", "NAML") == "NRMS"
        if self.nrms:
            self.multi_head_self_attn = MultiHeadSelfAttention(args.news_dim, args.num_attention_heads, 16, 16)
            self.attn = AttentionPooling(args.num_attention_heads * 16, args.user_query_vector_dim)
        else:
            self.attn = AttentionPooling(args.news_dim, args.user_query_vector_dim)
        self.pad_doc = nn.Parameter(torch.empty(1, args.news_dim).uniform_(-1, 1))

    def _packed_w1(self):
        at = self.attn
        src = (at.att_fc1.weight, self.pad_doc, at.att_fc1.bias, at.att_fc2.weight)
        key = tuple((t.data_ptr(), t._version) for t in src) + (src[0].device, ops.param_generation)
        c = getattr(self, "_w1_pack", None)
        if c is None or c[0] != key:
            c = (key, ops.user_encoder_pack_w1(src[0].detach(), src[1].detach().view(-1), src[2].detach(),
                                               src[3].detach().view(-1)))
            object.__setattr__(self, "_w1_pack", c)
        return c[1]

    def _pool(self, v, idx, m, use_mask, B, H):
        at = self.attn
        Q, D = at.att_fc1.weight.shape
        user = torch.empty(B, D, device=v.device, dtype=F32)
        a = torch.empty(B, H, device=v.device, dtype=F32)
        if ops.user_encoder_score_supported(B, H, D, Q):
            return ops.user_encoder_score(v, idx, m, self.pad_doc.view(-1), self._packed_w1(), Q, at.att_fc1.bias,
                                          at.att_fc2.weight.view(-1), at.att_fc2.bias, use_mask, user, a, B, H)
        if idx is not None:
            return ops.user_encoder_fwd_gather(v, idx, m, self.pad_doc.view(-1), at.att_fc1.weight, at.att_fc1.bias,
                                               at.att_fc2.weight.view(-1), at.att_fc2.bias, use_mask, user, a)
        return ops.user_encoder_fwd(v, m, self.pad_doc.view(-1), at.att_fc1.weight, at.att_fc1.bias,
                                    at.att_fc2.weight.view(-1), at.att_fc2.bias, use_mask, user, a, None, B, H)

    def forward(self, news_vecs, log_mask=None):
        B, H, D = news_vecs.shape
        v = news_vecs.contiguous().float().view(B * H, D)
        m = log_mask.contiguous().float()
        use_mask = bool(self.args.user_log_mask)
        if self.nrms:
            fr = nrms_self_attention(self.multi_head_self_attn, self.pad_doc, v, m, use_mask, B, H)
            v, m, use_mask = fr["ctx"], fr["pool_mask"], True
        return self._pool(v, None, m, use_mask, B, H)

    def forward_gather(self, table, idx, log_mask):
        B, H = idx.shape
        if self.nrms:
            vecs = torch.empty(B * H, table.shape[1], device=table.device, dtype=F32)
            ops.gather_rows_f32(table, idx.reshape(-1), vecs)
            return self.forward(vecs.view(B, H, -1), log_mask)
        return self._pool(table, idx.contiguous(), log_mask.contiguous().float(), bool(self.args.user_log_mask), B, H)


class TrainState:

    def __init__(self, news_encoder, user_encoder, teachers, transform, device):
        self.ne, self.ue, self.teachers, self.transform = news_encoder, user_encoder, teachers, transform
        self.enc = news_encoder.engine()
        self.enc.check_supported()
        enc_params = self.enc.trainable_order()
        at = user_encoder.attn
        head_all = [user_encoder.pad_doc, at.att_fc1.weight, at.att_fc1.bias, at.att_fc2.weight, at.att_fc2.bias]
        self.nrms = bool(getattr(user_encoder, "nrms", False))
        if self.nrms:
            mh = user_encoder.multi_head_self_attn
            head_all += [mh.W_Q.weight, mh.W_K.weight, mh.W_V.weight, mh.W_Q.bias, mh.W_K.bias, mh.W_V.bias]
        head = [p for p in head_all if p.requires_grad]
        if head and len(head) != len(head_all):
            raise TinyRecError("the user encoder must be trainable or frozen as a whole")
        self.ue_trainable = bool(head)
        tparams = []
        for lin in transform:
            if lin.weight.requires_grad != lin.bias.requires_grad:
                raise TinyRecError("transform_matrix weight/bias must share requires_grad")
            if lin.weight.requires_grad:
                tparams += [lin.weight, lin.bias]
        self.tm_trainable = bool(tparams)
        if tparams and len(tparams) != 2 * len(transform):
            raise TinyRecError("transform_matrix modules must be trainable or frozen together")
        ordered = enc_params + head + tparams
        self.sig = tuple(id(p) for p in ordered)
        self.flat = FlatParams(ordered, device) if ordered else None
        self.head_begin = self.flat.off(head[0]) if head else (self.flat.off(tparams[0]) if tparams else (self.flat.numel if self.flat else 0))
        self.head_end = self.flat.numel if self.flat else 0
        self.stage = torch.zeros(max(self.head_end - self.head_begin, 1), device=device, dtype=F32)
        news_encoder._flat = self.flat
        self.hw = {}
        self.anchor = torch.zeros(1, device=device, requires_grad=True)
        self.comm_hook = None

    def valid(self, module):
        want = tuple(id(p) for p in _trainable_signature(module))
        if set(want) != set(self.sig):
            return False
        return self.flat is None or self.flat.attached()

    def _stage_view(self, p):
        o = self.flat.off(p) - self.head_begin
        return self.stage[o:o + p.numel()]

    def head_ws(self, B, H, K, M, D, Q, dev):
        key = (B, H, K, M)
        w = self.hw.get(key)
        if w is None:
            R = B * (H + K)
            mk = lambda *s: torch.empty(*s, device=dev, dtype=F32)
            w = dict(news=mk(R, D), user=mk(B, D), a=mk(B, H), e=mk(B, H, Q), ta=mk(max(M, 1), B, H), score=mk(B, K),
                     ue_scratch=mk(B * H * (Q + D)),
                     losses=torch.zeros(4 + 4 * B + 1, device=dev, dtype=F32), d_news=mk(R, D), d_user=mk(B, D),
                     T=mk(max(M, 1), R + B, D), TP=mk(max(M, 1), R + B, D), G=mk(max(M, 1), R + B, D))
            self.hw[key] = w
        return w

    def step_forward(self, history, history_mask, candidate, label, th_list, tc_list, temperature, coef, use_mask,
                     want_grad, training=False):
        B, H, W = history.shape
        K = candidate.shape[1]
        M = len(th_list)
        dev = history.device
        flat = self.flat
        if flat is not None:
            if flat.stale():
                flat.refresh_shadow()
            if want_grad:
                flat.reattach_grads()
        x = _rows_of(history, candidate)
        D = self.enc.D
        Q = self.ue.attn.att_fc1.weight.shape[0]
        w = self.head_ws(B, H, K, M, D, Q, dev)
        R = B * (H + K)
        drop = None
        if training:
            drop = self.ne.drop_state(dev)
            drop.advance()
        news = self.enc.forward(x, flat, save=want_grad, out=w["news"], drop=drop)
        mask = history_mask.contiguous().float()
        label = label.contiguous()
        at = self.ue.attn
        T, TP, G = w["T"], w["TP"], w["G"]
        ext = getattr(th_list, "ext", None)
        adopted = (M > 0 and ext is not None and ext is getattr(tc_list, "ext", None) and ext.is_cuda
                   and tuple(ext.shape) == tuple(T.shape) and ext.dtype == F32 and ext.is_contiguous())
        if adopted:
            T = ext
        pool_vecs, pool_mask, pool_use_mask = news[:B * H], mask, use_mask
        if self.nrms:
            nb = w.setdefault("nrms", [dict() for _ in range(1 + M)])
            fr = w["fr"] = nrms_self_attention(self.ue.multi_head_self_attn, self.ue.pad_doc, news[:B * H], mask, use_mask,
                                               B, H, nb[0])
            if fr["ctx"].shape[1] != D:
                raise TinyRecError("NRMS: num_attention_heads * 16 must equal news_dim (the click score is a dot product)")
            pool_vecs, pool_mask, pool_use_mask = fr["ctx"], fr["pool_mask"], True
        encs = [dict(vecs=pool_vecs, pad_doc=self.ue.pad_doc.view(-1), W1=at.att_fc1.weight, b1=at.att_fc1.bias,
                     w2=at.att_fc2.weight.view(-1), b2=at.att_fc2.bias, user=w["user"], a=w["a"], e=w["e"])]
        for i in range(M):
            if not adopted:
                T[i, :B * H].copy_(th_list[i].reshape(B * H, D))
                T[i, B * H:R].copy_(tc_list[i].reshape(B * K, D))
            t = self.teachers[i]
            tv = T[i, :B * H]
            if self.nrms:
                tv = nrms_self_attention(t.multi_head_self_attn, t.pad_doc, tv, mask, use_mask, B, H, nb[1 + i])["ctx"]
            encs.append(dict(vecs=tv, pad_doc=t.pad_doc.view(-1), W1=t.attn.att_fc1.weight, b1=t.attn.att_fc1.bias,
                             w2=t.attn.att_fc2.weight.view(-1), b2=t.attn.att_fc2.bias, user=T[i, R:], a=w["ta"][i], e=None))
        ops.user_encoder_fwd_multi(encs, pool_mask, pool_use_mask, B, H)
        if M:
            ws, bs = [lin.weight for lin in self.transform], [lin.bias for lin in self.transform]
            sw, sb = _const_stride(ws), _const_stride(bs)
            if sw is not None and sb is not None:
                ops.sgemm_nt(T, ws[0], bs[0], TP, R + B, D, D, M, (R + B) * D, sw, sb, (R + B) * D)
            else:
                for i in range(M):
                    ops.sgemm_nt(T[i], ws[i], bs[i], TP[i], R + B, D, D, 1, 0, 0, 0, 0)
        ops.kd_loss(news, w["user"], label, T if M else None, TP if M else None, M, B, H, K, D, temperature, coef,
                    want_grad, w["score"], w["losses"], w["d_news"], w["d_user"], G if M else None)
        if want_grad:
            self.stage.zero_()
            if self.ue_trainable:
                sv = self._stage_view
                dpad, dW1, db1, dw2, db2 = (sv(self.ue.pad_doc), sv(at.att_fc1.weight), sv(at.att_fc1.bias),
                                            sv(at.att_fc2.weight), sv(at.att_fc2.bias))
            else:
                scratch = torch.zeros(D + Q * D + 2 * Q + 1, device=dev, dtype=F32)
                dpad, dW1, db1 = scratch[:D], scratch[D:D + Q * D], scratch[D + Q * D:D + Q * D + Q]
                dw2, db2 = scratch[D + Q * D + Q:D + Q * D + 2 * Q], scratch[D + Q * D + 2 * Q:]
            if not self.nrms:
                ops.user_encoder_bwd(news[:B * H], mask, self.ue.pad_doc.view(-1), at.att_fc1.weight, at.att_fc2.weight.view(-1),
                                     use_mask, w["a"], w["e"], w["d_user"], w["d_news"], dpad, dW1, db1, dw2, db2, w["ue_scratch"],
                                     B, H)
            else:
                self._nrms_backward(w, mask, use_mask, dpad, dW1, db1, dw2, db2, B, H, D)
            if self.tm_trainable and M:
                gw = [self._stage_view(lin.weight) for lin in self.transform]
                gb = [self._stage_view(lin.bias) for lin in self.transform]
                sw, sb = _const_stride(gw), _const_stride(gb)
                if sw is not None and sb is not None:
                    ops.sgemm_tn_acc(G, T, gw[0], gb[0], R + B, D, D, M, (R + B) * D, (R + B) * D, sw, sb)
                else:
                    for i in range(M):
                        ops.sgemm_tn_acc(G[i], T[i], gw[i], gb[i], R + B, D, D, 1, 0, 0, 0, 0)
        self.last = w
        return w

    def _nrms_backward(self, w, mask, use_mask, dpad, dW1, db1, dw2, db2, B, H, D):
        fr, at, mh = w["fr"], self.ue.attn, self.ue.multi_head_self_attn
        Rh, Dh, dev = B * H, fr["ctx"].shape[1], mask.device
        nb = w["nrms"][0]
        for name, shape in (("d_ctx", (Rh, Dh)), ("dqkv", (3, Rh, Dh)), ("dxb", (Rh, D))):
            if name not in nb:
                nb[name] = torch.empty(*shape, device=dev, dtype=F32)
        d_ctx = nb["d_ctx"].zero_()
        ops.user_encoder_bwd(fr["ctx"], fr["pool_mask"], self.ue.pad_doc.view(-1), at.att_fc1.weight, at.att_fc2.weight.view(-1),
                             True, w["a"], w["e"], w["d_user"], d_ctx, dpad, dW1, db1, dw2, db2, w["ue_scratch"], B, H)
        ops.nrms_attn_bwd(fr["qkv"], mask if use_mask else None, d_ctx, nb["dqkv"], B, H)
        if self.ue_trainable:
            o = self.flat.off(mh.W_Q.weight) - self.head_begin
            gW = self.stage[o:o + 3 * Dh * D]
            o = self.flat.off(mh.W_Q.bias) - self.head_begin
            gb = self.stage[o:o + 3 * Dh]
            if self.flat.off(mh.W_V.weight) - self.flat.off(mh.W_Q.weight) != 2 * Dh * D or \
                    self.flat.off(mh.W_V.bias) - self.flat.off(mh.W_Q.bias) != 2 * Dh:
                raise TinyRecError("NRMS: W_Q / W_K / W_V are not contiguous in the flat buffer")
            ops.sgemm_tn_acc(nb["dqkv"], fr["xb"], gW, gb, Rh, Dh, D, 3, Rh * Dh, 0, Dh * D, Dh)
        ops.sgemm_nn(nb["dqkv"], fr["Wc"], nb["dxb"], Rh, D, Dh, 3, Rh * Dh, fr["sw"])
        ops.nrms_blend_bwd(nb["dxb"], None if use_mask else mask.reshape(-1), w["d_news"][:Rh], dpad)

    def step_backward(self, g_total):
        w = self.last
        flat = self.flat
        w["d_news"].mul_(g_total)
        if self.head_end > self.head_begin:
            self.stage.mul_(g_total)
            flat.grad[self.head_begin:self.head_end].add_(self.stage[:self.head_end - self.head_begin])
        if self.comm_hook is None:
            self.enc.backward(w["d_news"], flat)
            return
        done_to = [flat.numel]
        sent = []

        def layer_done(i):
            lo = flat.off(self.enc.layers[i].q.weight)
            if lo >= done_to[0]:
                return
            if sent:
                cur = lo
                for a, b in sorted(sent):
                    if a > cur:
                        self.comm_hook(flat, cur, a)
                    cur = max(cur, b)
                if done_to[0] > cur:
                    self.comm_hook(flat, cur, done_to[0])
            else:
                self.comm_hook(flat, lo, done_to[0])
            done_to[0] = lo

        def grads_ready(first, last):
            if not sent:
                lr_low = self.enc.layers[self.enc.lowest_trainable_layer()]
                top = _align8(flat.off(lr_low.ln2.bias) + lr_low.ln2.bias.numel())
                if done_to[0] > top:
                    self.comm_hook(flat, top, done_to[0])
                    done_to[0] = top
            lo, hi = flat.off(first), _align8(flat.off(last) + last.numel())
            hi = min(hi, done_to[0])
            if hi > lo:
                self.comm_hook(flat, lo, hi)
                sent.append((lo, hi))

        self.enc.backward(w["d_news"], flat, on_layer_done=layer_done,
                          on_grads_ready=grads_ready if getattr(self, "fine_grained_comm", True) else None)
        if done_to[0] > 0:
            self.comm_hook(flat, 0, done_to[0])


def _rows_of(history, candidate):
    B, H, W = history.shape
    K = candidate.shape[1]
    if (history.is_contiguous() and candidate.is_contiguous() and history.dtype == candidate.dtype
            and history.untyped_storage().data_ptr() == candidate.untyped_storage().data_ptr()
            and candidate.storage_offset() == history.storage_offset() + B * H * W):
        return torch.as_strided(history, (B * (H + K), W), (W, 1))
    return torch.cat([history.reshape(B * H, W), candidate.reshape(B * K, W)], 0)


def _const_stride(tensors):
    if len(tensors) == 1:
        return 0
    base = tensors[0].data_ptr()
    d = tensors[1].data_ptr() - base
    if d <= 0 or d % 16:
        return None
    for i, t in enumerate(tensors):
        if t.data_ptr() - base != i * d or not t.is_contiguous():
            return None
    return d // 4


def _trainable_signature(module):
    return [p for p in module.parameters() if p.requires_grad]


class _StepFn(torch.autograd.Function):
    @staticmethod
    def forward(ctx, anchor, state, args):
        w = state.step_forward(*args)
        ctx.state = state
        losses = w["losses"]
        return losses[3].clone(), losses[0].clone(), losses[1].clone(), losses[2].clone(), w["score"].clone()

    @staticmethod
    def backward(ctx, g_total, g_distill, g_emb, g_target, g_score):
        ctx.state.step_backward(g_total)
        return None, None, None


def _get_state(module, build):
    st = getattr(module, "_tnr_state", None)
    if st is None or not st.valid(module):
        st = build()
        object.__setattr__(module, "_tnr_state", st)
    return st


class ModelBert(nn.Module):

    def __init__(self, args, is_teacher=False):
        super().__init__()
        self.args = args
        self.news_encoder = NewsEncoder(args, is_teacher)
        self.user_encoder = UserEncoder(args)

    def forward(self, history, history_mask, candidate):
        B, H, W = history.shape
        K = candidate.shape[1]
        x = torch.cat([history.reshape(B * H, W), candidate.reshape(B * K, W)], 0)
        vec = self.news_encoder(x)
        hist = vec[:B * H].view(B, H, -1)
        cand = vec[B * H:].view(B, K, -1)
        user = self.user_encoder(hist, history_mask)
        w = torch.zeros(4 + 4 * B + 1, device=vec.device, dtype=F32)
        score = torch.empty(B, K, device=vec.device, dtype=F32)
        label = torch.zeros(B, device=vec.device, dtype=torch.int64)
        ops.kd_loss(vec, user, label, None, None, 0, B, H, K, vec.shape[1], 1.0, 1.0, False, score, w, None, None, None)
        return score, hist, cand, user


def kd_ce_loss(logits_S, logits_T, temperature=1):
    p_T = torch.softmax(logits_T / temperature, dim=-1)
    return -(p_T * torch.log_softmax(logits_S / temperature, dim=-1)).sum(dim=-1).mean()


def hid_mse_loss(state_S, state_T, mask=None, reduce=True):
    se = (state_S - state_T) ** 2
    if mask is None:
        return se.mean() if reduce else se.mean(dim=-1)
    if not reduce:
        return (se * mask.unsqueeze(-1)).mean(dim=-1)
    return (se * mask.unsqueeze(-1)).sum() / (mask.sum() * state_S.size(-1))


class Model(nn.Module):

    def __init__(self, args):
        super().__init__()
        self.args = args
        self.teachers = nn.ModuleList([UserEncoder(args) for _ in range(args.num_teachers)])
        self.student = ModelBert(args, is_teacher=False)
        self.target_loss_fn = nn.CrossEntropyLoss()
        self.transform_matrix = nn.ModuleList([nn.Linear(args.news_dim, args.news_dim) for _ in range(args.num_teachers)])
        for module in self.transform_matrix:
            nn.init.xavier_uniform_(module.weight, gain=1.0)
            nn.init.constant_(module.bias, 0.0)

    def train_state(self):
        dev = self.transform_matrix[0].weight.device if len(self.transform_matrix) else self.student.user_encoder.pad_doc.device
        if dev.type != "cuda":
            raise TinyRecError("tinyrec Model needs its parameters on a CUDA device (no CPU path)")
        return _get_state(self, lambda: TrainState(self.student.news_encoder, self.student.user_encoder,
                                                   list(self.teachers), list(self.transform_matrix), dev))

    def forward(self, history, history_mask, candidate, label, teacher_history_embs, teacher_candidate_embs):
        st = self.train_state()
        want_grad = torch.is_grad_enabled() and st.flat is not None
        keep = lambda t: t if isinstance(t, list) else list(t)
        args = (history, history_mask, candidate, label, keep(teacher_history_embs), keep(teacher_candidate_embs),
                float(self.args.temperature), float(self.args.coef), bool(self.args.user_log_mask), want_grad,
                bool(self.training))
        if want_grad:
            return _StepFn.apply(st.anchor, st, args)
        w = st.step_forward(*args)
        ls = w["losses"]
        return ls[3].clone(), ls[0].clone(), ls[1].clone(), ls[2].clone(), w["score"].clone()
```

tiny-newsrec_b200/ops.py:

```python
import ctypes

import torch

from . import _lib
from ._lib import ACT_DGELU, ACT_GELU, ACT_GELU_DAUX, ACT_MULAUX, ACT_NONE, ACT_TANH, BF16, F32, Dropout, GemmArgs

_bf16 = torch.bfloat16
_f32 = torch.float32


def _stream():
    return ctypes.c_void_p(torch.cuda.current_stream().cuda_stream)


def _chk(t, dtype, name):
    if t.dtype != dtype or not t.is_cuda:
        raise _lib.TinyRecError(f"{name}: expected CUDA {dtype}, got {t.dtype} on {t.device}")
    return t


def _ptr(t):
    return ctypes.c_void_p(t.data_ptr()) if t is not None else ctypes.c_void_p(0)


def make_drop(seed_tensor, site, p):
    if seed_tensor is None or not p > 0.0:
        return None
    d = Dropout()
    d.seed, d.site, d.p = seed_tensor.data_ptr(), int(site), float(p)
    return d


def _dp(d):
    return ctypes.byref(d) if d is not None else None


def dropout_mask(drop, n, device):
    keep = torch.empty(n, device=device, dtype=torch.uint8)
    lib = _ready(keep)
    _lib.check(lib.tnr_dropout_mask(_dp(drop), n, _ptr(keep), _stream()), "tnr_dropout_mask")
    return keep


class _Stats:
    launches = 0
    gemm_events = None
    op_events = None


stats = _Stats()

param_generation = 0


def bump_param_generation():
    global param_generation
    param_generation += 1


def _timed(fn):
    import functools

    @functools.wraps(fn)
    def wrap(*a, **k):
        if stats.op_events is None:
            return fn(*a, **k)
        e0, e1 = torch.cuda.Event(enable_timing=True), torch.cuda.Event(enable_timing=True)
        e0.record()
        r = fn(*a, **k)
        e1.record()
        tag = ""
        if fn.__name__ == "gemm":
            A, Bm = a[0], a[1]
            M, K = (A.shape[1], A.shape[0]) if k.get("a_t") else (A.shape[0], A.shape[1])
            N = Bm.shape[1] if k.get("b_t") else Bm.shape[0]
            tag = f"{M}x{N}x{K}" + ("/wgrad" if k.get("a_t") else "/dgrad" if k.get("b_t") else "") + \
                  {ACT_NONE: "", ACT_GELU: "+gelu", ACT_TANH: "+tanh", ACT_DGELU: "+dgelu", ACT_GELU_DAUX: "+gelu",
                   ACT_MULAUX: "+mulaux"}[k.get("act", ACT_NONE)] + \
                  ("+aux" if k.get("aux") is not None and k.get("act") in (ACT_GELU, ACT_GELU_DAUX) else "") + \
                  ("+res" if k.get("residual") is not None else "") + ("+bias" if k.get("bias") is not None else "")
        stats.op_events.append((fn.__name__, tag, e0, e1))
        return r
    return wrap


def _ready(t, kernels=1):
    _lib.require_device(t.device.index)
    stats.launches += kernels
    return _lib.load()


@_timed
def gemm(a, b, out, *, a_t=False, b_t=False, bias=None, residual=None, act=ACT_NONE, aux=None,
         split_k=1, accumulate=False, drop=None, colsum=None):
    lib = _ready(a)
    _chk(a, _bf16, "gemm.a"); _chk(b, _bf16, "gemm.b")
    if a.stride(1) != 1 or b.stride(1) != 1 or out.stride(1) != 1:
        raise _lib.TinyRecError("gemm: operands must have unit inner stride")
    M, K = (a.shape[1], a.shape[0]) if a_t else (a.shape[0], a.shape[1])
    N, Kb = (b.shape[1], b.shape[0]) if b_t else (b.shape[0], b.shape[1])
    if K != Kb or out.shape[0] != M or out.shape[1] != N:
        raise _lib.TinyRecError(f"gemm: shape mismatch A{tuple(a.shape)} B{tuple(b.shape)} C{tuple(out.shape)} "
                                f"a_t={a_t} b_t={b_t}")
    g = GemmArgs()
    g.M, g.N, g.K = M, N, K
    g.A, g.lda, g.a_mn_major = a.data_ptr(), a.stride(0), int(a_t)
    g.B, g.ldb, g.b_mn_major = b.data_ptr(), b.stride(0), int(b_t)
    g.C, g.ldc = out.data_ptr(), out.stride(0)
    if out.dtype == _bf16:
        g.c_dtype = BF16
    elif out.dtype == _f32:
        g.c_dtype = F32
    else:
        raise _lib.TinyRecError("gemm: out must be bf16 or fp32")
    g.bias = _chk(bias, _f32, "gemm.bias").data_ptr() if bias is not None else None
    if residual is not None:
        _chk(residual, _bf16, "gemm.residual")
        g.residual, g.ldr = residual.data_ptr(), residual.stride(0)
    g.act = act
    if aux is not None:
        _chk(aux, _bf16, "gemm.aux")
        g.aux, g.ldaux = aux.data_ptr(), aux.stride(0)
    g.split_k = split_k
    g.accumulate = int(accumulate)
    if drop is not None:
        g.drop = ctypes.pointer(drop)
    if colsum is not None:
        g.colsum = _chk(colsum, _f32, "gemm.colsum").data_ptr()
    if stats.gemm_events is not None:
        e0, e1 = torch.cuda.Event(enable_timing=True), torch.cuda.Event(enable_timing=True)
        e0.record()
        _lib.check(lib.tnr_gemm_bf16(ctypes.byref(g), _stream()), "tnr_gemm_bf16")
        e1.record()
        stats.gemm_events.append((2.0 * M * N * K, e0, e1))
        return out
    _lib.check(lib.tnr_gemm_bf16(ctypes.byref(g), _stream()), "tnr_gemm_bf16")
    return out


@_timed
def embed_ln(x, L, word, pos, type0, gamma, beta, eps, out, drop=None):
    lib = _ready(x)
    _chk(x, torch.int64, "embed_ln.x")
    n = x.shape[0]
    E = word.shape[1]
    wd = BF16 if word.dtype == _bf16 else F32
    _lib.check(lib.tnr_embed_ln_fwd(_ptr(x), x.stride(0), n, L, word.shape[0], _ptr(word), wd,
                                    _ptr(_chk(pos, _f32, "pos")), _ptr(_chk(type0, _f32, "type0")),
                                    _ptr(_chk(gamma, _f32, "gamma")), _ptr(_chk(beta, _f32, "beta")),
                                    eps, E, _ptr(_chk(out, _bf16, "out")), _dp(drop), _stream()), "tnr_embed_ln_fwd")
    return out


@_timed
def layernorm_fwd(x, gamma, beta, eps, out):
    lib = _ready(x)
    rows, E = x.shape
    _lib.check(lib.tnr_layernorm_fwd(_ptr(_chk(x, _bf16, "ln.x")), rows, E, _ptr(gamma), _ptr(beta), eps,
                                     _ptr(_chk(out, _bf16, "ln.out")), _stream()), "tnr_layernorm_fwd")
    return out


@_timed
def layernorm_bwd(dy, x, gamma, eps, dx, dgamma, dbeta, dx_drop=None, drop=None, dsum=None):
    lib = _ready(x)
    rows, E = x.shape
    _lib.check(lib.tnr_layernorm_bwd(_ptr(_chk(dy, _bf16, "ln.dy")), _ptr(_chk(x, _bf16, "ln.x")), rows, E,
                                     _ptr(gamma), eps, _ptr(_chk(dx, _bf16, "ln.dx")),
                                     _ptr(_chk(dgamma, _f32, "dgamma")), _ptr(_chk(dbeta, _f32, "dbeta")),
                                     _ptr(dx_drop), _ptr(dsum), _dp(drop), _stream()), "tnr_layernorm_bwd")
    return dx


@_timed
def colsum(x, out):
    lib = _ready(x)
    _lib.check(lib.tnr_colsum_bf16(_ptr(_chk(x, _bf16, "colsum.x")), x.shape[0], x.shape[1], x.stride(0),
                                   _ptr(_chk(out, _f32, "colsum.out")), _stream()), "tnr_colsum_bf16")
    return out


def _chk_relbias(relpos, A, L):
    _chk(relpos, _f32, "relpos")
    if tuple(relpos.shape) != (A, 2 * L - 1) or not relpos.is_contiguous():
        raise _lib.TinyRecError(f"attention: rel-pos bias must be contiguous fp32 [A, 2L-1] = [{A}, {2 * L - 1}], "
                                f"got {tuple(relpos.shape)}")


@_timed
def attn_fwd(qkv, x, L, relpos, ctx, A, drop=None):
    lib = _ready(qkv)
    n = x.shape[0]
    E = qkv.shape[1] // 3
    mask_ptr = ctypes.c_void_p(x.data_ptr() + 8 * L)
    _chk_relbias(relpos, A, L)
    _lib.check(lib.tnr_attn_relpos_fwd(_ptr(_chk(qkv, _bf16, "attn.qkv")), mask_ptr, x.stride(0),
                                       _ptr(_chk(relpos, _f32, "relpos")), _ptr(_chk(ctx, _bf16, "ctx")),
                                       n, L, A, E, _dp(drop), _stream()), "tnr_attn_relpos_fwd")
    return ctx


_attn_ws = {}


@_timed
def attn_bwd(qkv, x, L, relpos, dctx, dqkv, A, drop=None, dbias=None, workspace=None):
    n = x.shape[0]
    lib = _ready(qkv, 1 if L <= 32 else 2)
    E = qkv.shape[1] // 3
    mask_ptr = ctypes.c_void_p(x.data_ptr() + 8 * L)
    _chk_relbias(relpos, A, L)
    if L > 32 and workspace is None:
        key = (qkv.device, 2 * n * A * L)
        workspace = _attn_ws.get(key)
        if workspace is None:
            _attn_ws.clear()
            workspace = _attn_ws[key] = torch.empty(2 * n * A * L, device=qkv.device, dtype=_f32)
    if workspace is not None:
        _chk(workspace, _f32, "attn.workspace")
        if workspace.numel() < 2 * n * A * L:
            raise _lib.TinyRecError("attn_bwd: workspace too small")
    _lib.check(lib.tnr_attn_relpos_bwd(_ptr(_chk(qkv, _bf16, "attn.qkv")), mask_ptr, x.stride(0),
                                       _ptr(relpos), _ptr(_chk(dctx, _bf16, "dctx")),
                                       _ptr(_chk(dqkv, _bf16, "dqkv")), _ptr(dbias), _ptr(workspace), n, L, A, E, _dp(drop),
                                       _stream()),
               "tnr_attn_relpos_bwd")
    return dqkv


@_timed
def attnpool_fwd(x, e, Q, w2, b2, mask, out, a_out, n, S):
    lib = _ready(x)
    C = x.shape[1]
    _lib.check(lib.tnr_attnpool_fwd(_ptr(_chk(x, _bf16, "pool.x")), _ptr(_chk(e, _bf16, "pool.e")), e.stride(0), Q,
                                    _ptr(_chk(w2, _f32, "w2")), _ptr(_chk(b2, _f32, "b2")), _ptr(mask),
                                    _ptr(_chk(out, _bf16, "pool.out")), _ptr(_chk(a_out, _f32, "a_out")),
                                    n, S, C, _stream()), "tnr_attnpool_fwd")
    return out


@_timed
def attnpool_bwd(x, e, Q, w2, a_in, dout, dx, du, dw2, db2, n, S):
    lib = _ready(x)
    C = x.shape[1]
    _lib.check(lib.tnr_attnpool_bwd(_ptr(x), _ptr(e), e.stride(0), Q, _ptr(w2), _ptr(_chk(a_in, _f32, "a_in")),
                                    _ptr(_chk(dout, _f32, "dout")), _ptr(_chk(dx, _bf16, "dx")),
                                    _ptr(_chk(du, _bf16, "du")), _ptr(_chk(dw2, _f32, "dw2")),
                                    _ptr(_chk(db2, _f32, "db2")), n, S, C, _stream()), "tnr_attnpool_bwd")


@_timed
def cast_f32_bf16(x, y):
    lib = _ready(x)
    _lib.check(lib.tnr_cast_f32_bf16(_ptr(_chk(x, _f32, "cast.x")), _ptr(_chk(y, _bf16, "cast.y")), x.numel(),
                                     _stream()), "tnr_cast_f32_bf16")
    return y


@_timed
def user_encoder_fwd(vecs, mask, pad_doc, W1, b1, w2, b2, use_mask, user, a_out, e_out, B, H):
    lib = _ready(vecs)
    D, Q = W1.shape[1], W1.shape[0]
    for t, nm in ((vecs, "vecs"), (mask, "mask"), (pad_doc, "pad_doc"), (W1, "W1"), (b1, "b1"), (w2, "w2"), (b2, "b2"),
                  (user, "user"), (a_out, "a")):
        _chk(t, _f32, "user_encoder." + nm)
    _lib.check(lib.tnr_user_encoder_fwd(_ptr(vecs), _ptr(mask), _ptr(pad_doc), _ptr(W1), _ptr(b1), _ptr(w2), _ptr(b2),
                                        int(use_mask), _ptr(user), _ptr(a_out), _ptr(e_out), B, H, D, Q, _stream()),
               "tnr_user_encoder_fwd")
    return user


@_timed
def user_encoder_fwd_gather(table, idx, mask, pad_doc, W1, b1, w2, b2, use_mask, user, a_out=None):
    lib = _ready(table)
    B, H = idx.shape
    D, Q = W1.shape[1], W1.shape[0]
    for t, nm in ((table, "table"), (mask, "mask"), (pad_doc, "pad_doc"), (W1, "W1"), (b1, "b1"), (w2, "w2"), (b2, "b2"),
                  (user, "user")):
        _chk(t, _f32, "user_encoder_gather." + nm)
    _chk(idx, torch.int32, "user_encoder_gather.idx")
    if table.shape[1] != D or not table.is_contiguous() or not idx.is_contiguous() or tuple(mask.shape) != (B, H):
        raise _lib.TinyRecError("user_encoder_fwd_gather: shape / layout mismatch")
    _lib.check(lib.tnr_user_encoder_fwd_gather(_ptr(table), table.shape[0], _ptr(idx), _ptr(mask), _ptr(pad_doc), _ptr(W1),
                                               _ptr(b1), _ptr(w2), _ptr(b2), int(use_mask), _ptr(user), _ptr(a_out), B, H, D, Q,
                                               _stream()), "tnr_user_encoder_fwd_gather")
    return user


def user_encoder_score_supported(B, H, D, Q):
    return B >= 64 and H <= 64 and D % 32 == 0 and D <= 256 and Q <= 208


def user_encoder_pack_w1(W1, pad_doc, b1, w2, packed=None):
    lib = _ready(W1, 2)
    Q, D = W1.shape
    n = int(lib.tnr_user_encoder_packed_w1_floats(D))
    if packed is None or packed.numel() != n:
        packed = torch.empty(n, device=W1.device, dtype=_f32)
    for t, nm in ((W1, "W1"), (pad_doc, "pad_doc"), (b1, "b1"), (w2, "w2")):
        _chk(t, _f32, "pack_w1." + nm)
    _lib.check(lib.tnr_user_encoder_pack_w1(_ptr(W1.contiguous()), _ptr(pad_doc.contiguous()), _ptr(b1.contiguous()),
                                            _ptr(w2.contiguous()), _ptr(packed), D, Q, _stream()),
               "tnr_user_encoder_pack_w1")
    return packed


_score_ws = {}


@_timed
def user_encoder_score(vecs, idx, mask, pad_doc, w1_packed, Q, b1, w2, b2, use_mask, user, a_out, B, H):
    lib = _ready(vecs, 3)
    D = vecs.shape[1]
    for t, nm in ((vecs, "vecs"), (mask, "mask"), (pad_doc, "pad_doc"), (w1_packed, "w1_packed"), (b1, "b1"), (w2, "w2"),
                  (b2, "b2"), (user, "user"), (a_out, "a")):
        _chk(t, _f32, "user_encoder_score." + nm)
    if idx is not None:
        _chk(idx, torch.int32, "user_encoder_score.idx")
        if tuple(idx.shape) != (B, H) or not idx.is_contiguous():
            raise _lib.TinyRecError("user_encoder_score: idx must be contiguous int32 [B, H]")
    elif vecs.shape[0] != B * H:
        raise _lib.TinyRecError("user_encoder_score: vecs must be [B*H, D]")
    if not vecs.is_contiguous() or tuple(mask.shape) != (B, H) or a_out.numel() != B * H or user.numel() != B * D:
        raise _lib.TinyRecError("user_encoder_score: shape / layout mismatch")
    nbytes = int(lib.tnr_user_encoder_score_ws_bytes(B, H))
    key = (vecs.device, nbytes)
    ws = _score_ws.get(key)
    if ws is None:
        _score_ws.clear()
        ws = _score_ws[key] = torch.empty(nbytes, device=vecs.device, dtype=torch.uint8)
    _lib.check(lib.tnr_user_encoder_score(_ptr(vecs), vecs.shape[0], _ptr(idx), _ptr(mask), _ptr(pad_doc), _ptr(w1_packed),
                                          _ptr(b1), _ptr(w2), _ptr(b2), int(use_mask), _ptr(user), _ptr(a_out), _ptr(ws),
                                          B, H, D, Q, _stream()), "tnr_user_encoder_score")
    return user


@_timed
def user_encoder_fwd_multi(encoders, mask, use_mask, B, H):
    lib = _ready(mask, 1)
    n = len(encoders)
    arr = (_lib.UserEncoderIO * n)()
    D, Q = encoders[0]["W1"].shape[1], encoders[0]["W1"].shape[0]
    for io, enc in zip(arr, encoders):
        for k in ("vecs", "pad_doc", "W1", "b1", "w2", "b2", "user", "a"):
            _chk(enc[k], _f32, "user_encoder." + k)
        if tuple(enc["W1"].shape) != (Q, D) or not enc["W1"].is_contiguous():
            raise _lib.TinyRecError("user_encoder_fwd_multi: all encoders must share [Q, D] contiguous fc1 weights")
        io.vecs, io.pad_doc, io.W1, io.b1 = enc["vecs"].data_ptr(), enc["pad_doc"].data_ptr(), enc["W1"].data_ptr(), enc["b1"].data_ptr()
        io.w2, io.b2, io.user, io.a_out = enc["w2"].data_ptr(), enc["b2"].data_ptr(), enc["user"].data_ptr(), enc["a"].data_ptr()
        io.e_out = enc["e"].data_ptr() if enc.get("e") is not None else None
    _lib.check(lib.tnr_user_encoder_fwd_multi(arr, n, _ptr(_chk(mask, _f32, "user_encoder.mask")), int(use_mask), B, H, D, Q,
                                              _stream()), "tnr_user_encoder_fwd_multi")


@_timed
def user_encoder_bwd(vecs, mask, pad_doc, W1, w2, use_mask, a_in, e_in, d_user, d_vecs, dpad, dW1, db1, dw2, db2, scratch, B, H):
    lib = _ready(vecs, 2)
    D, Q = W1.shape[1], W1.shape[0]
    for t, nm in ((d_user, "d_user"), (d_vecs, "d_vecs"), (dpad, "dpad"), (dW1, "dW1"), (db1, "db1"), (dw2, "dw2"),
                  (db2, "db2"), (a_in, "a"), (e_in, "e"), (scratch, "scratch")):
        _chk(t, _f32, "user_encoder_bwd." + nm)
    if scratch.numel() < B * H * (Q + D):
        raise _lib.TinyRecError("user_encoder_bwd: scratch too small")
    _lib.check(lib.tnr_user_encoder_bwd(_ptr(vecs), _ptr(mask), _ptr(pad_doc), _ptr(W1), _ptr(w2), int(use_mask),
                                        _ptr(a_in), _ptr(e_in), _ptr(d_user), _ptr(d_vecs), _ptr(dpad), _ptr(dW1),
                                        _ptr(db1), _ptr(dw2), _ptr(db2), _ptr(scratch), B, H, D, Q, _stream()),
               "tnr_user_encoder_bwd")


@_timed
def kd_loss(s_news, s_user, label, T_ext, TP_ext, M, B, H, K, D, temperature, coef, want_grad, score_out, losses,
            d_news, d_user, G_ext):
    lib = _ready(s_news)
    _chk(label, torch.int64, "kd_loss.label")
    for t, nm in ((s_news, "s_news"), (s_user, "s_user"), (score_out, "score"), (losses, "losses")):
        _chk(t, _f32, "kd_loss." + nm)
    if losses.numel() < 4 + 4 * B + 1:
        raise _lib.TinyRecError("kd_loss: losses must hold 4 + 4B + 1 floats (zero-initialised once)")
    _lib.check(lib.tnr_kd_loss_fwdbwd(_ptr(s_news), _ptr(s_user), _ptr(label), _ptr(T_ext), _ptr(TP_ext), M, B, H, K, D,
                                      float(temperature), float(coef), int(want_grad), _ptr(score_out), _ptr(losses),
                                      _ptr(d_news), _ptr(d_user), _ptr(G_ext), _stream()), "tnr_kd_loss_fwdbwd")


@_timed
def sgemm_nt(A, Bm, bias, C, M, N, K, batch, sA, sB, sbias, sC):
    lib = _ready(A)
    _lib.check(lib.tnr_sgemm_nt(_ptr(_chk(A, _f32, "sgemm.A")), _ptr(_chk(Bm, _f32, "sgemm.B")), _ptr(bias),
                                _ptr(_chk(C, _f32, "sgemm.C")), M, N, K, batch, sA, sB, sbias, sC, _stream()),
               "tnr_sgemm_nt")


@_timed
def sgemm_tn_acc(A, Bm, C, cbias, R, N1, N2, batch, sA, sB, sC, sbias):
    lib = _ready(A)
    _lib.check(lib.tnr_sgemm_tn_acc(_ptr(_chk(A, _f32, "sgemm.A")), _ptr(_chk(Bm, _f32, "sgemm.B")),
                                    _ptr(_chk(C, _f32, "sgemm.C")), _ptr(cbias), R, N1, N2, batch, sA, sB, sC, sbias,
                                    _stream()), "tnr_sgemm_tn_acc")


@_timed
def sgemm_nn(A, Bm, C, M, N, K, parts=1, sA=0, sB=0):
    lib = _ready(A)
    _lib.check(lib.tnr_sgemm_nn(_ptr(_chk(A, _f32, "sgemm_nn.A")), _ptr(_chk(Bm, _f32, "sgemm_nn.B")),
                                _ptr(_chk(C, _f32, "sgemm_nn.C")), M, N, K, parts, sA, sB, _stream()), "tnr_sgemm_nn")


@_timed
def nrms_blend_fwd(vecs, mask, pad_doc, out):
    lib = _ready(vecs)
    R, D = vecs.shape
    for t, nm in ((vecs, "vecs"), (mask, "mask"), (pad_doc, "pad_doc"), (out, "out")):
        _chk(t, _f32, "nrms_blend_fwd." + nm)
    if mask.numel() != R or pad_doc.numel() != D or not vecs.is_contiguous() or not out.is_contiguous():
        raise _lib.TinyRecError("nrms_blend_fwd: shape / layout mismatch")
    _lib.check(lib.tnr_nrms_blend_fwd(_ptr(vecs), _ptr(mask), _ptr(pad_doc), _ptr(out), R, D, _stream()), "tnr_nrms_blend_fwd")
    return out


@_timed
def nrms_blend_bwd(d_blend, mask, d_vecs, dpad):
    lib = _ready(d_blend)
    R, D = d_blend.shape
    for t, nm in ((d_blend, "d_blend"), (d_vecs, "d_vecs")):
        _chk(t, _f32, "nrms_blend_bwd." + nm)
    if not d_blend.is_contiguous() or not d_vecs.is_contiguous() or d_vecs.numel() != R * D:
        raise _lib.TinyRecError("nrms_blend_bwd: shape / layout mismatch")
    _lib.check(lib.tnr_nrms_blend_bwd(_ptr(d_blend), _ptr(mask), _ptr(d_vecs), _ptr(dpad), R, D, _stream()), "tnr_nrms_blend_bwd")


def _nrms_planes(qkv, B, H):
    _chk(qkv, _f32, "nrms.qkv")
    if qkv.dim() != 3 or qkv.shape[0] != 3 or qkv.shape[1] != B * H or qkv.shape[2] % 16 or not qkv.is_contiguous():
        raise _lib.TinyRecError(f"nrms: qkv must be contiguous fp32 [3, B*H, n_heads*16], got {tuple(qkv.shape)}")
    return qkv.shape[2] // 16


@_timed
def nrms_attn_fwd(qkv, mask, ctx, B, H):
    lib = _ready(qkv)
    heads = _nrms_planes(qkv, B, H)
    _chk(ctx, _f32, "nrms.ctx")
    _lib.check(lib.tnr_nrms_attn_fwd(_ptr(qkv[0]), _ptr(qkv[1]), _ptr(qkv[2]), _ptr(mask), _ptr(ctx), B, H, heads, _stream()),
               "tnr_nrms_attn_fwd")
    return ctx


@_timed
def nrms_attn_bwd(qkv, mask, d_ctx, dqkv, B, H):
    lib = _ready(qkv)
    heads = _nrms_planes(qkv, B, H)
    _nrms_planes(dqkv, B, H)
    _chk(d_ctx, _f32, "nrms.d_ctx")
    _lib.check(lib.tnr_nrms_attn_bwd(_ptr(qkv[0]), _ptr(qkv[1]), _ptr(qkv[2]), _ptr(mask), _ptr(d_ctx), _ptr(dqkv[0]),
                                     _ptr(dqkv[1]), _ptr(dqkv[2]), B, H, heads, _stream()), "tnr_nrms_attn_bwd")


@_timed
def adam_amsgrad(p, g, m, v, vmax, shadow, lr, beta1, beta2, eps, step, grad_scale=1.0):
    lib = _ready(p)
    for t, nm in ((p, "p"), (g, "g"), (m, "m"), (v, "v")) + (((vmax, "vmax"),) if vmax is not None else ()):
        _chk(t, _f32, "adam." + nm)
    _lib.check(lib.tnr_adam_amsgrad(_ptr(p), _ptr(g), _ptr(m), _ptr(v), _ptr(vmax), _ptr(shadow), p.numel(), lr, beta1,
                                    beta2, eps, step, grad_scale, _stream()), "tnr_adam_amsgrad")


@_timed
def adam_amsgrad_devstep(p, g, m, v, vmax, shadow, lr, beta1, beta2, eps, step_dev, bc_ws, grad_scale=1.0, advance=True):
    lib = _ready(p, 2 if advance else 1)
    for t, nm in ((p, "p"), (g, "g"), (m, "m"), (v, "v"), (bc_ws, "bc_ws")) + (((vmax, "vmax"),) if vmax is not None else ()):
        _chk(t, _f32, "adam." + nm)
    _chk(step_dev, torch.int32, "adam.step_dev")
    _lib.check(lib.tnr_adam_amsgrad_devstep(_ptr(p), _ptr(g), _ptr(m), _ptr(v), _ptr(vmax), _ptr(shadow), p.numel(), lr, beta1,
                                            beta2, eps, _ptr(step_dev), _ptr(bc_ws), grad_scale, int(bool(advance)),
                                            _stream()),
               "tnr_adam_amsgrad_devstep")


def host_copy(dst, src, n_threads=4):
    import numpy as np
    src = np.ascontiguousarray(src)
    nbytes = src.size * src.itemsize
    if dst.is_cuda or not dst.is_contiguous() or dst.numel() * dst.element_size() < nbytes or dst.element_size() != src.itemsize:
        raise _lib.TinyRecError("host_copy: dst must be a contiguous CPU tensor of the source's element size, large enough")
    _lib.check(_lib.load().tnr_host_copy_mt(ctypes.c_void_p(dst.data_ptr()), ctypes.c_void_p(src.ctypes.data), nbytes,
                                            int(n_threads)), "tnr_host_copy_mt")
    return dst


def allreduce_p2p(ptrs_dev, multicast_ptr, flags_dev, rank, world, off, n, n_ctas):
    lib = _lib.load()
    stats.launches += 1
    _lib.check(lib.tnr_allreduce_p2p(ctypes.c_void_p(int(ptrs_dev)), ctypes.c_void_p(int(multicast_ptr) or None),
                                     ctypes.c_void_p(int(flags_dev)), int(rank), int(world), int(off), int(n), int(n_ctas),
                                     _stream()), "tnr_allreduce_p2p")


def set_sm_reserve(n_sms, device=None):
    lib = _lib.load()
    if device is not None and torch.cuda.current_device() != torch.device(device).index:
        with torch.cuda.device(device):
            _lib.check(lib.tnr_set_sm_reserve(int(n_sms)), "tnr_set_sm_reserve")
        return
    _lib.check(lib.tnr_set_sm_reserve(int(n_sms)), "tnr_set_sm_reserve")


@_timed
def gather_rows_i32_i64(table, idx, out):
    lib = _ready(table)
    _chk(table, torch.int32, "gather.table"); _chk(idx, torch.int32, "gather.idx"); _chk(out, torch.int64, "gather.out")
    _lib.check(lib.tnr_gather_rows_i32_i64(_ptr(table), table.shape[0], _ptr(idx), idx.numel(), table.shape[1], _ptr(out),
                                           _stream()), "tnr_gather_rows_i32_i64")
    return out


@_timed
def train_batch_gather(news, teacher_tables, hist_idx, cand_idx, tokens_out, teacher_out):
    lib = _ready(news)
    _chk(news, torch.int32, "batch_gather.news"); _chk(hist_idx, torch.int32, "batch_gather.hist_idx")
    _chk(cand_idx, torch.int32, "batch_gather.cand_idx"); _chk(tokens_out, torch.int64, "batch_gather.tokens")
    M = len(teacher_tables)
    nh, nc, W = hist_idx.numel(), cand_idx.numel(), news.shape[1]
    if tokens_out.numel() != (nh + nc) * W or not tokens_out.is_contiguous() or len(teacher_out) != M:
        raise _lib.TinyRecError("train_batch_gather: shape / layout mismatch")
    D = teacher_tables[0].shape[1] if M else 4
    tabs = (ctypes.c_void_p * max(M, 1))()
    outs = (ctypes.c_void_p * max(M, 1))()
    ld = D
    for i in range(M):
        _chk(teacher_tables[i], _f32, "batch_gather.teacher"); _chk(teacher_out[i], _f32, "batch_gather.teacher_out")
        if teacher_tables[i].shape[1] != D or teacher_out[i].shape[-1] != D or teacher_out[i].stride(-1) != 1:
            raise _lib.TinyRecError("train_batch_gather: teacher tables / outputs must share the row width")
        tabs[i], outs[i] = teacher_tables[i].data_ptr(), teacher_out[i].data_ptr()
        ld = teacher_out[i].stride(-2)
    _lib.check(lib.tnr_train_batch_gather(_ptr(news), news.shape[0], W, tabs, outs, M, D, ld, _ptr(hist_idx), nh, _ptr(cand_idx), nc,
                                          _ptr(tokens_out), _stream()), "tnr_train_batch_gather")


@_timed
def gather_rows_f32(table, idx, out, out_ld=None):
    lib = _ready(table)
    _chk(table, _f32, "gather.table"); _chk(idx, torch.int32, "gather.idx"); _chk(out, _f32, "gather.out")
    D = table.shape[1]
    _lib.check(lib.tnr_gather_rows_f32(_ptr(table), table.shape[0], _ptr(idx), idx.numel(), D, _ptr(out),
                                       D if out_ld is None else out_ld, _stream()), "tnr_gather_rows_f32")
    return out


_eval_ws = {}


@_timed
def eval_metrics(table, user, ptr, cand, label, max_c, per_imp, sums=None, score_out=None):
    lib = _ready(table, 3 if sums is not None else 2)
    _chk(table, _f32, "eval.table"); _chk(user, _f32, "eval.user"); _chk(ptr, torch.int64, "eval.ptr")
    _chk(cand, torch.int32, "eval.cand"); _chk(label, torch.int8, "eval.label"); _chk(per_imp, torch.float64, "eval.per_imp")
    n_imp = ptr.numel() - 1
    nnz = cand.numel()
    if label.numel() != nnz or user.shape[0] < n_imp or per_imp.numel() < 5 * n_imp or not table.is_contiguous():
# ... 28 lines not shown
```

tiny-newsrec_b200/post_train.py:

```python
from types import SimpleNamespace

import torch
from torch import nn

from . import ops
from ._lib import TinyRecError
from .engine import F32, FlatParams
from .model_bert import NewsEncoder as _NewsEncoder, _const_stride, _get_state, _trainable_signature


def _encoder_args(args):
    return SimpleNamespace(pooling="att", model_type="tnlrv3", config_name=getattr(args, "config_name", None),
                           model_name=getattr(args, "model_name", None), num_student_layers=args.num_hidden_layers,
                           num_teacher_layers=args.num_hidden_layers, news_query_vector_dim=args.news_query_vector_dim,
                           news_dim=args.news_dim)


TITLE_SITE_BASE = 1 << 12


class TitleBodySimModel(nn.Module):

    def __init__(self, args):
        super().__init__()
        self.news_encoder = _NewsEncoder(_encoder_args(args), False)

    def forward(self, title, body):
        bz, candi_num, input_num = title.shape
        body_emb = self.news_encoder(body)
        title_emb = self.news_encoder(title.reshape(-1, input_num)).reshape(bz, candi_num, -1)
        scores = torch.bmm(title_emb, body_emb.unsqueeze(-1)).squeeze(-1)
        return scores, title_emb, body_emb


class _DistillState:

    def __init__(self, news_encoder, transform, device):
        self.ne, self.transform = news_encoder, transform
        self.enc = news_encoder.engine()
        self.enc.check_supported()
        enc_params = self.enc.trainable_order()
        tparams = []
        for lin in transform:
            if lin.weight.requires_grad != lin.bias.requires_grad:
                raise TinyRecError("transform_matrix weight/bias must share requires_grad")
            if lin.weight.requires_grad:
                tparams += [lin.weight, lin.bias]
        if tparams and len(tparams) != 2 * len(transform):
            raise TinyRecError("transform_matrix modules must be trainable or frozen together")
        self.tm_trainable = bool(tparams)
        ordered = enc_params + tparams
        self.sig = tuple(id(p) for p in ordered)
        self.flat = FlatParams(ordered, device) if ordered else None
        self.head_begin = self.flat.off(tparams[0]) if tparams else (self.flat.numel if self.flat else 0)
        self.head_end = self.flat.numel if self.flat else 0
        self.stage = torch.zeros(max(self.head_end - self.head_begin, 1), device=device, dtype=F32)
        news_encoder._flat = self.flat
        self.hw = {}
        self.anchor = torch.zeros(1, device=device, requires_grad=True)
        self.comm_hook = None

    def valid(self, module):
        want = tuple(id(p) for p in _trainable_signature(module))
        return set(want) == set(self.sig) and (self.flat is None or self.flat.attached())

    def _stage_view(self, p):
        o = self.flat.off(p) - self.head_begin
        return self.stage[o:o + p.numel()]

    def step_forward(self, title, body, labels, t_titles, t_bodies, want_grad, training):
        B, K1, Wt = title.shape
        M = len(t_titles)
        dev = title.device
        flat = self.flat
        if flat is not None:
            if flat.stale():
                flat.refresh_shadow()
            if want_grad:
                flat.reattach_grads()
        D = self.enc.D
        R = B * K1
        key = (B, K1, M)
        w = self.hw.get(key)
        if w is None:
            mk = lambda *s: torch.empty(*s, device=dev, dtype=F32)
            w = dict(news=mk(R, D), user=mk(B, D), score=mk(B, K1), losses=torch.zeros(4 + 4 * B + 1, device=dev, dtype=F32),
                     d_news=mk(R, D), d_user=mk(B, D), T=mk(max(M, 1), R + B, D), TP=mk(max(M, 1), R + B, D),
                     G=mk(max(M, 1), R + B, D))
            self.hw[key] = w
        drop = None
        if training:
            drop = self.ne.drop_state(dev)
            drop.advance()
        body_emb = self.enc.forward(body, flat, save=want_grad, out=w["user"], drop=drop, tag="body")
        w["ws_body"] = self.enc.last_ws
        title_emb = self.enc.forward(title.reshape(R, Wt), flat, save=want_grad, out=w["news"],
                                     drop=drop.offset(TITLE_SITE_BASE) if drop is not None else None, tag="title")
        w["ws_title"] = self.enc.last_ws
        T, TP, G = w["T"], w["TP"], w["G"]
        for i in range(M):
            T[i, :R].copy_(t_titles[i].reshape(R, D))
            T[i, R:].copy_(t_bodies[i].reshape(B, D))
        if M:
            ws_, bs_ = [lin.weight for lin in self.transform], [lin.bias for lin in self.transform]
            sw, sb = _const_stride(ws_), _const_stride(bs_)
            if sw is not None and sb is not None:
                ops.sgemm_nt(T, ws_[0], bs_[0], TP, R + B, D, D, M, (R + B) * D, sw, sb, (R + B) * D)
            else:
                for i in range(M):
                    ops.sgemm_nt(T[i], ws_[i], bs_[i], TP[i], R + B, D, D, 1, 0, 0, 0, 0)
        ops.kd_loss(title_emb, body_emb, labels.contiguous(), T if M else None, TP if M else None, M, B, 0, K1, D, 1.0, 1.0,
                    want_grad, w["score"], w["losses"], w["d_news"], w["d_user"], G if M else None)
        if want_grad:
            self.stage.zero_()
            if self.tm_trainable and M:
                gw = [self._stage_view(lin.weight) for lin in self.transform]
                gb = [self._stage_view(lin.bias) for lin in self.transform]
                sw, sb = _const_stride(gw), _const_stride(gb)
                if sw is not None and sb is not None:
                    ops.sgemm_tn_acc(G, T, gw[0], gb[0], R + B, D, D, M, (R + B) * D, (R + B) * D, sw, sb)
                else:
                    for i in range(M):
                        ops.sgemm_tn_acc(G[i], T[i], gw[i], gb[i], R + B, D, D, 1, 0, 0, 0, 0)
        self.last = w
        return w

    def step_backward(self, g_total):
        w, flat = self.last, self.flat
        w["d_news"].mul_(g_total)
        w["d_user"].mul_(g_total)
        if self.head_end > self.head_begin:
            self.stage.mul_(g_total)
            flat.grad[self.head_begin:self.head_end].add_(self.stage[:self.head_end - self.head_begin])
        self.enc.backward(w["d_news"], flat, ws=w["ws_title"])
        self.enc.backward(w["d_user"], flat, ws=w["ws_body"])


class _DistillFn(torch.autograd.Function):
    @staticmethod
    def forward(ctx, anchor, state, args):
        w = state.step_forward(*args)
        ctx.state = state
        ls = w["losses"]
        return ls[3].clone(), ls[2].clone(), ls[0].clone(), ls[1].clone(), w["score"].clone()

    @staticmethod
    def backward(ctx, g_total, g_target, g_distill, g_emb, g_score):
        ctx.state.step_backward(g_total)
        return None, None, None


class DistillModel(nn.Module):

    def __init__(self, args):
        super().__init__()
        self.args = args
        self.student = TitleBodySimModel(args)
        self.target_loss = nn.CrossEntropyLoss()
        self.transform_matrix = nn.ModuleList([nn.Linear(args.news_dim, args.news_dim) for _ in range(args.num_teachers)])
        for module in self.transform_matrix:
            nn.init.xavier_uniform_(module.weight, gain=1.0)
            nn.init.constant_(module.bias, 0.0)

    def train_state(self):
        dev = self.student.news_encoder.dense.weight.device
        if dev.type != "cuda":
            raise TinyRecError("tinyrec DistillModel needs its parameters on a CUDA device (no CPU path)")
        return _get_state(self, lambda: _DistillState(self.student.news_encoder, list(self.transform_matrix), dev))

    def lr_ranges(self, lr_bert=1e-6, lr_rest=1e-5):
        st = self.train_state()
        ne = self.student.news_encoder
        rest = [p for p in (ne.attn.att_fc1.weight, ne.dense.weight) if st.flat.has(p)]
        rest += [lin.weight for lin in self.transform_matrix if st.flat.has(lin.weight)]
        cut = min(st.flat.off(p) for p in rest) if rest else st.flat.numel
        return [(0, cut, lr_bert), (cut, st.flat.numel, lr_rest)]

    def forward(self, title, body, labels, teacher_titles, teacher_bodies):
        st = self.train_state()
        want_grad = torch.is_grad_enabled() and st.flat is not None
        args = (title, body, labels, list(teacher_titles), list(teacher_bodies), want_grad, bool(self.training))
        if want_grad:
            return _DistillFn.apply(st.anchor, st, args)
        w = st.step_forward(*args)
        ls = w["losses"]
        return ls[3].clone(), ls[2].clone(), ls[0].clone(), ls[1].clone(), w["score"].clone()


class DomainTitleBodySimModel(nn.Module):

    def __init__(self, args):
        super().__init__()
        self.news_encoder = _NewsEncoder(_encoder_args(args), False)
        self.loss = nn.CrossEntropyLoss()

    def train_state(self):
        dev = self.news_encoder.dense.weight.device
        if dev.type != "cuda":
            raise TinyRecError("tinyrec DomainTitleBodySimModel needs its parameters on a CUDA device (no CPU path)")
        return _get_state(self, lambda: _DistillState(self.news_encoder, [], dev))

    def forward(self, title, body, labels):
        st = self.train_state()
        want_grad = torch.is_grad_enabled() and st.flat is not None
        args = (title, body, labels, [], [], want_grad, bool(self.training))
        if want_grad:
            total, _, _, _, score = _DistillFn.apply(st.anchor, st, args)
            return score, total
        w = st.step_forward(*args)
        return w["score"].clone(), w["losses"][3].clone()
```

Baseline: 4821.

## Split KD loss over cluster slices, fuse grad scaling, overlap teacher forward on side stream

The KD loss kernel now launches as a cluster of four blocks per impression. Each block computes the MSE and gradient terms for a slice of rows in one fused pass, and the per-slice MSE partials are combined through distributed shared memory. Backward gradient scaling is folded into an on-device axpy and a fused scale-cast-colsum kernel, and an attnpool db1 output is added, which replaces separate mul_/add_ passes. The teacher forward and transform GEMM move into a helper that appears to run on a side stream overlapping the student work. This adds cluster-launch constraints and more code complexity, and risks redundant per-slice work such as every slice recomputing the scores.

```diff
diff --git a/include/tinyrec.h b/include/tinyrec.h
--- a/include/tinyrec.h
+++ b/include/tinyrec.h
@@ -55,6 +55,8 @@
                       float eps, void* dx_bf16, float* dgamma, float* dbeta, void* dx_drop_bf16,
                       float* dsum, const tnr_dropout* drop, void* stream);
 int tnr_colsum_bf16(const void* x_bf16, int rows, int cols, int ld, float* out, void* stream);
+int tnr_scale_cast_colsum(const float* x, const float* scale, int rows, int cols, void* y_bf16, float* colsum,
+                          void* stream);
 
 int tnr_attn_relpos_fwd(const void* qkv_bf16, const int64_t* mask, int mask_ld, const float* relbias,
                         void* ctx_bf16, int n_news, int L, int A, int E, const tnr_dropout* drop,
@@ -68,7 +70,7 @@
                      int C, void* stream);
 int tnr_attnpool_bwd(const void* x_bf16, const void* e_bf16, int ldq, int Q, const float* w2,
                      const float* a_in, const float* dout, void* dx_bf16, void* du_bf16, float* dw2,
-                     float* db2, int n, int S, int C, void* stream);
+                     float* db2, float* db1, int n, int S, int C, void* stream);
 
 int tnr_user_encoder_fwd(const float* vecs, const float* mask, const float* pad_doc, const float* W1,
                          const float* b1, const float* w2, const float* b2, int use_mask, float* user,
@@ -124,6 +126,7 @@
                              long long n, float lr, float beta1, float beta2, float eps, int* step_dev,
                              float* bc_ws, float grad_scale, int advance, void* stream);
 int tnr_cast_f32_bf16(const float* x, void* y_bf16, long long n, void* stream);
+int tnr_axpy_dev(const float* x, const float* scale, float* y, long long n, void* stream);
 
 long long tnr_allreduce_p2p_flag_words(void);
 int tnr_allreduce_p2p(void* const* ptrs_dev, void* multicast_ptr, void* const* flags_dev, int rank, int world,
diff --git a/tiny-newsrec_b200/_lib.py b/tiny-newsrec_b200/_lib.py
--- a/tiny-newsrec_b200/_lib.py
+++ b/tiny-newsrec_b200/_lib.py
@@ -50,10 +50,11 @@
     "tnr_layernorm_fwd": ([P, c_int, c_int, P, P, c_float, P, P], c_int),
     "tnr_layernorm_bwd": ([P, P, c_int, c_int, P, c_float, P, P, P, P, P, POINTER(Dropout), P], c_int),
     "tnr_colsum_bf16": ([P, c_int, c_int, c_int, P, P], c_int),
+    "tnr_scale_cast_colsum": ([P, P, c_int, c_int, P, P, P], c_int),
     "tnr_attn_relpos_fwd": ([P, P, c_int, P, P, c_int, c_int, c_int, c_int, POINTER(Dropout), P], c_int),
     "tnr_attn_relpos_bwd": ([P, P, c_int, P, P, P, P, P, c_int, c_int, c_int, c_int, POINTER(Dropout), P], c_int),
     "tnr_attnpool_fwd": ([P, P, c_int, c_int, P, P, P, P, P, c_int, c_int, c_int, P], c_int),
-    "tnr_attnpool_bwd": ([P, P, c_int, c_int, P, P, P, P, P, P, P, c_int, c_int, c_int, P], c_int),
+    "tnr_attnpool_bwd": ([P, P, c_int, c_int, P, P, P, P, P, P, P, P, c_int, c_int, c_int, P], c_int),
     "tnr_user_encoder_fwd": ([P, P, P, P, P, P, P, c_int, P, P, P, c_int, c_int, c_int, c_int, P], c_int),
     "tnr_user_encoder_fwd_multi": ([P, c_int, P, c_int, c_int, c_int, c_int, c_int, P], c_int),
     "tnr_user_encoder_fwd_gather": ([P, c_int64, P, P, P, P, P, P, P, c_int, P, P, c_int, c_int, c_int, c_int, P], c_int),
@@ -74,6 +75,7 @@
     "tnr_adam_amsgrad": ([P, P, P, P, P, P, c_int64, c_float, c_float, c_float, c_float, c_int, c_float, P], c_int),
     "tnr_adam_amsgrad_devstep": ([P, P, P, P, P, P, c_int64, c_float, c_float, c_float, c_float, P, P, c_float, c_int, P], c_int),
     "tnr_cast_f32_bf16": ([P, P, c_int64, P], c_int),
+    "tnr_axpy_dev": ([P, P, P, c_int64, P], c_int),
     "tnr_gather_rows_i32_i64": ([P, c_int64, P, c_int64, c_int, P, P], c_int),
     "tnr_gather_rows_f32": ([P, c_int64, P, c_int64, c_int, P, c_int64, P], c_int),
     "tnr_train_batch_gather": ([P, c_int64, c_int, POINTER(c_void_p), POINTER(c_void_p), c_int, c_int, c_int64, P, c_int64, P,
diff --git a/tiny-newsrec_b200/csrc/head_kernels.cu b/tiny-newsrec_b200/csrc/head_kernels.cu
--- a/tiny-newsrec_b200/csrc/head_kernels.cu
+++ b/tiny-newsrec_b200/csrc/head_kernels.cu
@@ -1,13 +1,18 @@
 #include "common.cuh"
 
+#include <cooperative_groups.h>
+
+namespace cg = cooperative_groups;
+
 namespace tnr {
 
-constexpr int UE_THREADS = 1024;
+constexpr int KD_THREADS = 512;
 
 constexpr int KD_MAXM = 8;
 constexpr int KD_MAXK = 32;
-
-__global__ void __launch_bounds__(UE_THREADS)
+constexpr int KD_SLICES = 4;
+
+__global__ void __cluster_dims__(KD_SLICES, 1, 1) __launch_bounds__(KD_THREADS)
 kd_loss_kernel(const float* __restrict__ s_news, const float* __restrict__ s_user, const int64_t* __restrict__ label,
                const float* __restrict__ T_ext, const float* __restrict__ TP_ext, int M, int B, int H, int K, int D,
                float temperature, float coef, int want_grad, float* __restrict__ score_out, float* __restrict__ losses,
@@ -16,10 +21,11 @@
   __shared__ float s_tsc[KD_MAXM][KD_MAXK];
   __shared__ float s_w[KD_MAXM];
   __shared__ float s_ds[KD_MAXK];
+  __shared__ float s_ce[2];
+  __shared__ float s_part[KD_MAXM][KD_THREADS / 32];
   __shared__ float s_mse[KD_MAXM];
-  __shared__ float s_part[KD_MAXM][UE_THREADS / 32];
   __shared__ int s_last;
-  const int b = blockIdx.x, tid = threadIdx.x;
+  const int b = blockIdx.y, slice = blockIdx.x, tid = threadIdx.x;
   const int warp = uniform_warp_id(), lane = tid & 31;
   const int R = B * (H + K);
   const size_t Rext = (size_t)R + B;
@@ -30,7 +36,7 @@
   const int lab = lab_bad ? 0 : (int)lab_raw;
   const float invB = 1.0f / (float)B;
 
-  for (int item = warp; item < (1 + M) * K; item += UE_THREADS / 32) {
+  for (int item = warp; item < (1 + M) * K; item += KD_THREADS / 32) {
     const int i = item / K, k = item - i * K;
     const float *c, *u;
     if (i == 0) { c = cand + (size_t)k * D; u = usr; }
@@ -43,39 +49,6 @@
     for (int d = lane; d < D; d += 32) t = fmaf(c[d], u[d], t);
     t = warp_sum(t);
     if (lane == 0) { if (i == 0) s_sc[k] = t; else s_tsc[i - 1][k] = t; }
-  }
-  {
-    float ne[KD_MAXM], ue[KD_MAXM];
-#pragma unroll
-    for (int i = 0; i < KD_MAXM; ++i) { ne[i] = 0.f; ue[i] = 0.f; }
-    for (int idx = tid; idx < (H + K) * D; idx += UE_THREADS) {
-      const int r = idx / D, d = idx - r * D;
-      const size_t row = r < H ? (size_t)b * H + r : (size_t)B * H + (size_t)b * K + (r - H);
-      const float sv = s_news[row * D + d];
-#pragma unroll
-      for (int i = 0; i < KD_MAXM; ++i)
-        if (i < M) { const float diff = sv - TP_ext[((size_t)i * Rext + row) * D + d]; ne[i] = fmaf(diff, diff, ne[i]); }
-    }
-    for (int d = tid; d < D; d += UE_THREADS) {
-      const float uv = usr[d];
-#pragma unroll
-      for (int i = 0; i < KD_MAXM; ++i)
-        if (i < M) { const float diff = uv - TP_ext[((size_t)i * Rext + R + b) * D + d]; ue[i] = fmaf(diff, diff, ue[i]); }
-    }
-#pragma unroll
-    for (int i = 0; i < KD_MAXM; ++i)
-      if (i < M) {
-        ne[i] = warp_sum(ne[i]);
-        ue[i] = warp_sum(ue[i]);
-        if (lane == 0) { s_part[i][warp] = ne[i] / (float)((H + K) * D) + ue[i] / (float)D; }
-      }
-    __syncthreads();
-    if (tid < M) {
-      float t = 0.f;
-#pragma unroll
-      for (int w = 0; w < UE_THREADS / 32; ++w) t += s_part[tid][w];
-      s_mse[tid] = t;
-    }
   }
   __syncthreads();
   if (tid == 0) {
@@ -85,7 +58,7 @@
     for (int k = 0; k < K; ++k) se += expf(s_sc[k] - mx);
     const float lse = mx + logf(se);
     const float target = lab_bad ? __int_as_float(0x7fc00000) : lse - s_sc[lab];
-    float distill = 0.f, emb = 0.f;
+    float distill = 0.f;
     float pT[KD_MAXK];
     for (int k = 0; k < K; ++k) pT[k] = 0.f;
     if (M > 0) {
@@ -101,7 +74,7 @@
       }
       float ws = 0.f;
       for (int i = 0; i < M; ++i) { s_w[i] = expf(-(tl[i] - mn)); ws += s_w[i]; }
-      for (int i = 0; i < M; ++i) { s_w[i] /= ws; emb += s_w[i] * s_mse[i]; }
+      for (int i = 0; i < M; ++i) s_w[i] /= ws;
       float tmx = -INFINITY, smx = -INFINITY;
       float tsc[KD_MAXK];
       for (int k = 0; k < K; ++k) {
@@ -124,13 +97,93 @@
     }
     for (int k = 0; k < K; ++k)
       s_ds[k] = (s_ds[k] + coef * (expf(s_sc[k] - lse) - (k == lab ? 1.0f : 0.0f))) * invB;
+    s_ce[0] = distill;
+    s_ce[1] = target;
+  }
+  __syncthreads();
+  const float cne = 2.0f / (float)((H + K) * D) * invB;
+  const float cue = 2.0f / (float)D * invB;
+  const int rows_per = (H + K + KD_SLICES - 1) / KD_SLICES;
+  const int r0 = min(H + K, slice * rows_per), r1 = min(H + K, r0 + rows_per);
+  {
+    float ne[KD_MAXM], ue[KD_MAXM];
+#pragma unroll
+    for (int i = 0; i < KD_MAXM; ++i) { ne[i] = 0.f; ue[i] = 0.f; }
+    for (int idx = r0 * D + tid; idx < r1 * D; idx += KD_THREADS) {
+      const int r = idx / D, d = idx - r * D;
+      const size_t row = r < H ? (size_t)b * H + r : (size_t)B * H + (size_t)b * K + (r - H);
+      const float sv = s_news[row * D + d];
+      float g = 0.f;
+#pragma unroll
+      for (int i = 0; i < KD_MAXM; ++i)
+        if (i < M) {
+          const size_t o = ((size_t)i * Rext + row) * D + d;
+          const float diff = sv - TP_ext[o];
+          ne[i] = fmaf(diff, diff, ne[i]);
+          if (want_grad) {
+            const float gi = s_w[i] * cne * diff;
+            g += gi;
+            G_ext[o] = -gi;
+          }
+        }
+      if (want_grad) {
+        if (r >= H) g = fmaf(s_ds[r - H], usr[d], g);
+        d_news[row * D + d] = g;
+      }
+    }
+    if (slice == 0)
+      for (int d = tid; d < D; d += KD_THREADS) {
+        const float uv = usr[d];
+        float g = 0.f;
+        if (want_grad)
+          for (int k = 0; k < K; ++k) g = fmaf(s_ds[k], cand[(size_t)k * D + d], g);
+#pragma unroll
+        for (int i = 0; i < KD_MAXM; ++i)
+          if (i < M) {
+            const size_t o = ((size_t)i * Rext + R + b) * D + d;
+            const float diff = uv - TP_ext[o];
+            ue[i] = fmaf(diff, diff, ue[i]);
+            if (want_grad) {
+              const float gi = s_w[i] * cue * diff;
+              g += gi;
+              G_ext[o] = -gi;
+            }
+          }
+        if (want_grad) d_user[(size_t)b * D + d] = g;
+      }
+#pragma unroll
+    for (int i = 0; i < KD_MAXM; ++i)
+      if (i < M) {
+        ne[i] = warp_sum(ne[i]);
+        ue[i] = warp_sum(ue[i]);
+        if (lane == 0) { s_part[i][warp] = ne[i] / (float)((H + K) * D) + ue[i] / (float)D; }
+      }
+    __syncthreads();
+    if (tid < M) {
+      float t = 0.f;
+#pragma unroll
+      for (int w = 0; w < KD_THREADS / 32; ++w) t += s_part[tid][w];
+      s_mse[tid] = t;
+    }
+  }
+  cg::cluster_group cluster = cg::this_cluster();
+  cluster.sync();
+  if (slice == 0 && tid == 0) {
+    float emb = 0.f;
+    for (int i = 0; i < M; ++i) {
+      float t = 0.f;
+      for (int s = 0; s < KD_SLICES; ++s) t += cluster.map_shared_rank(s_mse, s)[i];
+      emb += s_w[i] * t;
+    }
+    const float distill = s_ce[0], target = s_ce[1];
     float* part = losses + 4 + 4 * (size_t)b;
     part[0] = distill; part[1] = emb; part[2] = target; part[3] = distill + coef * target + emb;
     __threadfence();
     unsigned int* ticket = reinterpret_cast<unsigned int*>(losses + 4 + 4 * (size_t)B);
     s_last = (atomicAdd(ticket, 1u) == (unsigned int)B - 1) ? 1 : 0;
   }
-  __syncthreads();
+  cluster.sync();
+  if (slice != 0) return;
   if (s_last && warp == 0) {
     __threadfence();
     float acc4[4] = {0.f, 0.f, 0.f, 0.f};
@@ -145,34 +198,7 @@
       *reinterpret_cast<unsigned int*>(losses + 4 + 4 * (size_t)B) = 0u;
     }
   }
-  __syncthreads();
-  for (int k = tid; k < K; k += UE_THREADS) score_out[(size_t)b * K + k] = s_sc[k];
-  if (!want_grad) return;
-  const float cne = 2.0f / (float)((H + K) * D) * invB;
-  const float cue = 2.0f / (float)D * invB;
-  for (int idx = tid; idx < (H + K) * D; idx += UE_THREADS) {
-    const int r = idx / D, d = idx - r * D;
-    const size_t row = r < H ? (size_t)b * H + r : (size_t)B * H + (size_t)b * K + (r - H);
-    const float sv = s_news[row * D + d];
-    float g = 0.f;
-    for (int i = 0; i < M; ++i) {
-      const float gi = s_w[i] * cne * (sv - TP_ext[((size_t)i * Rext + row) * D + d]);
-      g += gi;
-      G_ext[((size_t)i * Rext + row) * D + d] = -gi;
-    }
-    if (r >= H) g = fmaf(s_ds[r - H], usr[d], g);
-    d_news[row * D + d] = g;
-  }
-  for (int d = tid; d < D; d += UE_THREADS) {
-    float g = 0.f;
-    for (int k = 0; k < K; ++k) g = fmaf(s_ds[k], cand[(size_t)k * D + d], g);
-    for (int i = 0; i < M; ++i) {
-      const float gi = s_w[i] * cue * (usr[d] - TP_ext[((size_t)i * Rext + R + b) * D + d]);
-      g += gi;
-      G_ext[((size_t)i * Rext + R + b) * D + d] = -gi;
-    }
-    d_user[(size_t)b * D + d] = g;
-  }
+  for (int k = tid; k < K; k += KD_THREADS) score_out[(size_t)b * K + k] = s_sc[k];
 }
 
 }
@@ -187,8 +213,9 @@
                                float* G_ext, void* stream) {
   TNR_REQUIRE(M >= 0 && M <= KD_MAXM, "tnr_kd_loss_fwdbwd: num_teachers %d out of range (0..%d)", M, KD_MAXM);
   TNR_REQUIRE(K >= 1 && K <= KD_MAXK, "tnr_kd_loss_fwdbwd: candidates per impression %d out of range (1..%d)", K, KD_MAXK);
+  TNR_REQUIRE(B <= 65535, "tnr_kd_loss_fwdbwd: %d impressions per launch, at most 65535", B);
   if (B == 0) return 0;
-  kd_loss_kernel<<<B, UE_THREADS, 0, reinterpret_cast<cudaStream_t>(stream)>>>(
+  kd_loss_kernel<<<dim3(KD_SLICES, B), KD_THREADS, 0, reinterpret_cast<cudaStream_t>(stream)>>>(
       s_news, s_user, label, T_ext, TP_ext, M, B, H, K, D, temperature, coef, want_grad, score_out, losses, d_news, d_user,
       G_ext);
   TNR_LAUNCH_CHECK();
diff --git a/tiny-newsrec_b200/csrc/misc_kernels.cu b/tiny-newsrec_b200/csrc/misc_kernels.cu
--- a/tiny-newsrec_b200/csrc/misc_kernels.cu
+++ b/tiny-newsrec_b200/csrc/misc_kernels.cu
@@ -51,6 +51,21 @@
       p[i] -= (lr / bc1) * m[i] / (sqrtf(vm) * rsqrt_bc2 + eps);
       if (shadow != nullptr) shadow[i] = __float2bfloat16_rn(p[i]);
     }
+  }
+}
+
+__global__ void __launch_bounds__(256)
+axpy_dev_kernel(const float* __restrict__ x, const float* __restrict__ scale, float* __restrict__ y, long long n) {
+  const float g = scale[0];
+  const long long i4 = ((long long)blockIdx.x * blockDim.x + threadIdx.x) * 4;
+  if (i4 >= n) return;
+  if (i4 + 4 <= n && (((uintptr_t)(x + i4) | (uintptr_t)(y + i4)) & 15) == 0) {
+    const float4 a = *reinterpret_cast<const float4*>(x + i4);
+    float4 b = *reinterpret_cast<const float4*>(y + i4);
+    b.x = fmaf(g, a.x, b.x); b.y = fmaf(g, a.y, b.y); b.z = fmaf(g, a.z, b.z); b.w = fmaf(g, a.w, b.w);
+    *reinterpret_cast<float4*>(y + i4) = b;
+  } else {
+    for (long long i = i4; i < n && i < i4 + 4; ++i) y[i] = fmaf(g, x[i], y[i]);
   }
 }
 
@@ -423,6 +438,14 @@
   return 0;
 }
 
+TNR_API int tnr_axpy_dev(const float* x, const float* scale, float* y, long long n, void* stream) {
+  if (n == 0) return 0;
+  const long long threads = (n + 3) / 4;
+  axpy_dev_kernel<<<(int)((threads + 255) / 256), 256, 0, reinterpret_cast<cudaStream_t>(stream)>>>(x, scale, y, n);
+  TNR_LAUNCH_CHECK();
+  return 0;
+}
+
 TNR_API int tnr_gather_rows_i32_i64(const int32_t* table, long long n_rows_table, const int32_t* idx, long long n, int W,
                                     int64_t* out, void* stream) {
   if (n == 0) return 0;
diff --git a/tiny-newsrec_b200/csrc/norm_kernels.cu b/tiny-newsrec_b200/csrc/norm_kernels.cu
--- a/tiny-newsrec_b200/csrc/norm_kernels.cu
+++ b/tiny-newsrec_b200/csrc/norm_kernels.cu
@@ -377,6 +377,44 @@
     for (int r = 0; r < 32; ++r) s += red[r][threadIdx.x];
     const int c = blockIdx.x * 64 + threadIdx.x;
     if (c < cols) atomicAdd(out + c, s);
+  }
+}
+
+
+__global__ void __launch_bounds__(256)
+scale_cast_colsum_kernel(const float* __restrict__ x, const float* __restrict__ scale, int rows, int cols,
+                         __nv_bfloat16* __restrict__ y, float* __restrict__ colsum) {
+  const int cgroup = threadIdx.x & 7;
+  const int rlane = threadIdx.x >> 3;
+  const int col = (blockIdx.x * 8 + cgroup) * 8;
+  const float g = scale != nullptr ? scale[0] : 1.0f;
+  float acc[8];
+#pragma unroll
+  for (int i = 0; i < 8; ++i) acc[i] = 0.f;
+  if (col < cols) {
+    for (int r = blockIdx.y * 32 + rlane; r < rows; r += gridDim.y * 32) {
+      const float4* src = reinterpret_cast<const float4*>(x + (size_t)r * cols + col);
+      const float4 a = src[0], b = src[1];
+      const float v[8] = {a.x * g, a.y * g, a.z * g, a.w * g, b.x * g, b.y * g, b.z * g, b.w * g};
+      const bf16x8 o = pack8(v);
+      *reinterpret_cast<bf16x8*>(y + (size_t)r * cols + col) = o;
+      float w[8];
+      unpack8(o, w);
+#pragma unroll
+      for (int i = 0; i < 8; ++i) acc[i] += w[i];
+    }
+  }
+  if (colsum == nullptr) return;
+  __shared__ float red[32][65];
+#pragma unroll
+  for (int i = 0; i < 8; ++i) red[rlane][cgroup * 8 + i] = acc[i];
+  __syncthreads();
+  if (threadIdx.x < 64) {
+    float t = 0.f;
+#pragma unroll
+    for (int r = 0; r < 32; ++r) t += red[r][threadIdx.x];
+    const int c = blockIdx.x * 64 + threadIdx.x;
+    if (c < cols) atomicAdd(colsum + c, t);
   }
 }
 
@@ -463,3 +501,20 @@
   TNR_LAUNCH_CHECK();
   return 0;
 }
+
+extern "C" __attribute__((visibility("default"))) int tnr_scale_cast_colsum(const float* x, const float* scale, int rows,
+                                                                           int cols, void* y_bf16, float* colsum,
+                                                                           void* stream) {
+  TNR_REQUIRE(cols % 8 == 0, "tnr_scale_cast_colsum: cols=%d must be a multiple of 8", cols);
+  TNR_REQUIRE((uintptr_t)x % 16 == 0 && (uintptr_t)y_bf16 % 16 == 0, "tnr_scale_cast_colsum: x and y must be 16-byte aligned");
+  if (rows == 0) return 0;
+  dim3 grid((cols + 63) / 64, 1);
+  int gy = (num_sms() * 8) / (int)grid.x;
+  if (gy < 1) gy = 1;
+  const int max_gy = (rows + 31) / 32;
+  grid.y = gy < max_gy ? gy : max_gy;
+  scale_cast_colsum_kernel<<<grid, 256, 0, reinterpret_cast<cudaStream_t>(stream)>>>(
+      x, scale, rows, cols, reinterpret_cast<__nv_bfloat16*>(y_bf16), colsum);
+  TNR_LAUNCH_CHECK();
+  return 0;
+}
diff --git a/tiny-newsrec_b200/csrc/pooling.cu b/tiny-newsrec_b200/csrc/pooling.cu
--- a/tiny-newsrec_b200/csrc/pooling.cu
+++ b/tiny-newsrec_b200/csrc/pooling.cu
@@ -102,11 +102,12 @@
 attnpool_bwd_kernel(const __nv_bfloat16* __restrict__ x, const __nv_bfloat16* __restrict__ e, int ldq, int Q,
                     const float* __restrict__ w2, const float* __restrict__ a_in, const float* __restrict__ dout,
                     __nv_bfloat16* __restrict__ dx, __nv_bfloat16* __restrict__ du, float* __restrict__ dw2,
-                    float* __restrict__ db2, int n_news, int S) {
+                    float* __restrict__ db2, float* __restrict__ db1, int n_news, int S) {
   constexpr int C = VPL * 256;
   constexpr int ROW16 = VPL * 32;
   extern __shared__ __align__(16) unsigned char pw_sm[];
   __shared__ float s_gw[PW_WARPS][256];
+  __shared__ float s_gd[PW_WARPS][256];
   __shared__ float s_gb[PW_WARPS];
   const int warp = uniform_warp_id(), lane = threadIdx.x & 31;
   const int n = blockIdx.x * PW_WARPS + warp;
@@ -116,9 +117,9 @@
   float* s_dz = s_a + POOL_SMAX;
   const int q0 = lane * 8;
   const bool has_e = q0 < Q;
-  float gw[8];
-#pragma unroll
-  for (int i = 0; i < 8; ++i) gw[i] = 0.f;
+  float gw[8], gd[8];
+#pragma unroll
+  for (int i = 0; i < 8; ++i) { gw[i] = 0.f; gd[i] = 0.f; }
   float gb = 0.f;
   if (active) {
     const __nv_bfloat16* xn = x + (size_t)n * S * C;
@@ -197,7 +198,11 @@
           gw[i] = fmaf(dz, f[i], gw[i]);
           o[i] = dz * wv[i] * (1.0f - f[i] * f[i]);
         }
-        *reinterpret_cast<bf16x8*>(dun + (size_t)s * ldq + q0) = pack8(o);
+        const bf16x8 ob = pack8(o);
+        *reinterpret_cast<bf16x8*>(dun + (size_t)s * ldq + q0) = ob;
+        unpack8(ob, o);
+#pragma unroll
+        for (int i = 0; i < 8; ++i) gd[i] += o[i];
       }
       issue_e(s + PW_RING, slot);
       slot = slot + 1 == PW_RING ? 0 : slot + 1;
@@ -209,21 +214,28 @@
           atomicAdd(dw2 + q + i, dz * f[i]);
           o[i] = dz * w2[q + i] * (1.0f - f[i] * f[i]);
         }
-        *reinterpret_cast<bf16x8*>(dun + (size_t)s * ldq + q) = pack8(o);
+        const bf16x8 ob = pack8(o);
+        *reinterpret_cast<bf16x8*>(dun + (size_t)s * ldq + q) = ob;
+        if (db1 != nullptr) {
+          unpack8(ob, o);
+#pragma unroll
+          for (int i = 0; i < 8; ++i) atomicAdd(db1 + q + i, o[i]);
+        }
       }
     }
     pw_wait<0>();
     gb = warp_sum(gb);
   }
 #pragma unroll
-  for (int i = 0; i < 8; ++i) s_gw[warp][q0 + i] = gw[i];
+  for (int i = 0; i < 8; ++i) { s_gw[warp][q0 + i] = gw[i]; s_gd[warp][q0 + i] = gd[i]; }
   if (lane == 0) s_gb[warp] = gb;
   __syncthreads();
   for (int q = threadIdx.x; q < min(Q, 256); q += PW_THREADS) {
-    float t = 0.f;
-#pragma unroll
-    for (int w = 0; w < PW_WARPS; ++w) t += s_gw[w][q];
+    float t = 0.f, u = 0.f;
+#pragma unroll
+    for (int w = 0; w < PW_WARPS; ++w) { t += s_gw[w][q]; u += s_gd[w][q]; }
     atomicAdd(dw2 + q, t);
+    if (db1 != nullptr) atomicAdd(db1 + q, u);
   }
   if (threadIdx.x == 0) {
     float t = 0.f;
@@ -251,12 +263,12 @@
 
 template <int VPL>
 static int pool_bwd_launch(const void* x, const void* e, int ldq, int Q, const float* w2, const float* a_in, const float* dout,
-                           void* dx, void* du, float* dw2, float* db2, int n, int S, cudaStream_t st) {
+                           void* dx, void* du, float* dw2, float* db2, float* db1, int n, int S, cudaStream_t st) {
   const int smem = PW_WARPS * (PW_RING * VPL * 512 + 2 * POOL_SMAX * 4);
   TNR_SET_SMEM(attnpool_bwd_kernel<VPL>, smem);
   attnpool_bwd_kernel<VPL><<<(n + PW_WARPS - 1) / PW_WARPS, PW_THREADS, smem, st>>>(
       reinterpret_cast<const __nv_bfloat16*>(x), reinterpret_cast<const __nv_bfloat16*>(e), ldq, Q, w2, a_in, dout,
-      reinterpret_cast<__nv_bfloat16*>(dx), reinterpret_cast<__nv_bfloat16*>(du), dw2, db2, n, S);
+      reinterpret_cast<__nv_bfloat16*>(dx), reinterpret_cast<__nv_bfloat16*>(du), dw2, db2, db1, n, S);
   TNR_LAUNCH_CHECK();
   return 0;
 }
@@ -278,8 +290,8 @@
 }
 
 extern "C" __attribute__((visibility("default"))) int tnr_attnpool_bwd(const void* x_bf16, const void* e_bf16, int ldq, int Q, const float* w2, const float* a_in,
-                                const float* dout, void* dx_bf16, void* du_bf16, float* dw2, float* db2, int n, int S,
-                                int C, void* stream) {
+                                const float* dout, void* dx_bf16, void* du_bf16, float* dw2, float* db2, float* db1,
+                                int n, int S, int C, void* stream) {
   TNR_REQUIRE(S >= 1 && S <= POOL_SMAX, "tnr_attnpool_bwd: S=%d out of range (1..%d)", S, POOL_SMAX);
   TNR_REQUIRE(C % 256 == 0 && C <= 1024 && Q % 8 == 0 && ldq % 8 == 0,
               "tnr_attnpool_bwd: C must be 256/512/768/1024 and Q, ldq multiples of 8 (C=%d Q=%d ldq=%d)", C, Q, ldq);
@@ -288,9 +300,9 @@
   if (n == 0) return 0;
   cudaStream_t st = reinterpret_cast<cudaStream_t>(stream);
   switch (C / 256) {
-    case 1: return pool_bwd_launch<1>(x_bf16, e_bf16, ldq, Q, w2, a_in, dout, dx_bf16, du_bf16, dw2, db2, n, S, st);
-    case 2: return pool_bwd_launch<2>(x_bf16, e_bf16, ldq, Q, w2, a_in, dout, dx_bf16, du_bf16, dw2, db2, n, S, st);
-    case 3: return pool_bwd_launch<3>(x_bf16, e_bf16, ldq, Q, w2, a_in, dout, dx_bf16, du_bf16, dw2, db2, n, S, st);
-    default: return pool_bwd_launch<4>(x_bf16, e_bf16, ldq, Q, w2, a_in, dout, dx_bf16, du_bf16, dw2, db2, n, S, st);
-  }
-}
+    case 1: return pool_bwd_launch<1>(x_bf16, e_bf16, ldq, Q, w2, a_in, dout, dx_bf16, du_bf16, dw2, db2, db1, n, S, st);
+    case 2: return pool_bwd_launch<2>(x_bf16, e_bf16, ldq, Q, w2, a_in, dout, dx_bf16, du_bf16, dw2, db2, db1, n, S, st);
+    case 3: return pool_bwd_launch<3>(x_bf16, e_bf16, ldq, Q, w2, a_in, dout, dx_bf16, du_bf16, dw2, db2, db1, n, S, st);
+    default: return pool_bwd_launch<4>(x_bf16, e_bf16, ldq, Q, w2, a_in, dout, dx_bf16, du_bf16, dw2, db2, db1, n, S, st);
+  }
+}
diff --git a/tiny-newsrec_b200/engine.py b/tiny-newsrec_b200/engine.py
--- a/tiny-newsrec_b200/engine.py
+++ b/tiny-newsrec_b200/engine.py
@@ -318,7 +318,7 @@
         g = flat.g_view(p) if rows is None else flat.grad[flat.off(p):flat.off(p) + rows * p.shape[1]].view(rows, p.shape[1])
         ops.gemm(dy, xin, g, a_t=True, b_t=True, split_k=self._splitk(M, xin.shape[1], dy.shape[0]), accumulate=True)
 
-    def backward(self, d_news, flat, on_layer_done=None, ws=None, on_grads_ready=None):
+    def backward(self, d_news, flat, on_layer_done=None, ws=None, on_grads_ready=None, g_scale=None):
         ws = self.last_ws if ws is None else ws
         n, L, low, x = ws["n"], ws["L"], ws["low"], ws["x"]
         drop = ws.get("drop")
@@ -329,22 +329,20 @@
         at, dense = self.mod.attn, self.mod.dense
         if self.scratch_ln is None or self.scratch_ln.device != d_news.device:
             self.scratch_ln = torch.zeros(2 * E, device=d_news.device, dtype=F32)
-        ops.cast_f32_bf16(d_news, ws["dnews_bf"])
         dnb = ws["dnews_bf"]
+        ops.scale_cast_colsum(d_news, g_scale, dnb, flat.g_view(dense.bias) if flat.has(dense.weight) else None)
         if flat.has(dense.weight):
             self._wgrad(flat, dense.weight, dnb, ws["pooled"])
-            ops.colsum(dnb, flat.g_view(dense.bias))
         ops.gemm(dnb, self._w(flat, dense.weight), ws["dpooled"], b_t=True)
         xl = ws["xlast"]
         if flat.has(at.att_fc1.weight):
-            dw2, db2 = flat.g_view(at.att_fc2.weight).view(-1), flat.g_view(at.att_fc2.bias)
+            dw2, db2, db1 = flat.g_view(at.att_fc2.weight).view(-1), flat.g_view(at.att_fc2.bias), flat.g_view(at.att_fc1.bias)
         else:
-            dw2, db2 = self.scratch_ln[:self.Q], self.scratch_ln[E:E + 1]
+            dw2, db2, db1 = self.scratch_ln[:self.Q], self.scratch_ln[E:E + 1], None
         ops.attnpool_bwd(xl, ws["e"], self.Q, at.att_fc2.weight.view(-1), ws["a"], ws["dpooled"], ws["dx2"], ws["du"],
-                         dw2, db2, n, L)
+                         dw2, db2, n, L, db1=db1)
         if flat.has(at.att_fc1.weight):
             self._wgrad(flat, at.att_fc1.weight, ws["du"], xl)
-            ops.colsum(ws["du"], flat.g_view(at.att_fc1.bias))
         if low >= nl:
             return
         dx = ws["dx"]
diff --git a/tiny-newsrec_b200/model_bert.py b/tiny-newsrec_b200/model_bert.py
--- a/tiny-newsrec_b200/model_bert.py
+++ b/tiny-newsrec_b200/model_bert.py
@@ -297,6 +297,7 @@
         self.hw = {}
         self.anchor = torch.zeros(1, device=device, requires_grad=True)
         self.comm_hook = None
+        self.side_stream = {}
 
     def valid(self, module):
         want = tuple(id(p) for p in _trainable_signature(module))
@@ -342,7 +343,6 @@
         if training:
             drop = self.ne.drop_state(dev)
             drop.advance()
-        news = self.enc.forward(x, flat, save=want_grad, out=w["news"], drop=drop)
         mask = history_mask.contiguous().float()
         label = label.contiguous()
         at = self.ue.attn
@@ -352,6 +352,16 @@
                    and tuple(ext.shape) == tuple(T.shape) and ext.dtype == F32 and ext.is_contiguous())
         if adopted:
             T = ext
+        main = torch.cuda.current_stream(dev)
+        side = None
+        if M:
+            side = self.side_stream.get(dev)
+            if side is None:
+                side = self.side_stream[dev] = torch.cuda.Stream(dev)
+            side.wait_stream(main)
+            with torch.cuda.stream(side):
+                self._teacher_forward(T, TP, th_list, tc_list, adopted, mask, use_mask, w, B, H, K, D)
+        news = self.enc.forward(x, flat, save=want_grad, out=w["news"], drop=drop)
         pool_vecs, pool_mask, pool_use_mask = news[:B * H], mask, use_mask
         if self.nrms:
             nb = w.setdefault("nrms", [dict() for _ in range(1 + M)])
@@ -362,25 +372,9 @@
             pool_vecs, pool_mask, pool_use_mask = fr["ctx"], fr["pool_mask"], True
         encs = [dict(vecs=pool_vecs, pad_doc=self.ue.pad_doc.view(-1), W1=at.att_fc1.weight, b1=at.att_fc1.bias,
                      w2=at.att_fc2.weight.view(-1), b2=at.att_fc2.bias, user=w["user"], a=w["a"], e=w["e"])]
-        for i in range(M):
-            if not adopted:
-                T[i, :B * H].copy_(th_list[i].reshape(B * H, D))
-                T[i, B * H:R].copy_(tc_list[i].reshape(B * K, D))
-            t = self.teachers[i]
-            tv = T[i, :B * H]
-            if self.nrms:
-                tv = nrms_self_attention(t.multi_head_self_attn, t.pad_doc, tv, mask, use_mask, B, H, nb[1 + i])["ctx"]
-            encs.append(dict(vecs=tv, pad_doc=t.pad_doc.view(-1), W1=t.attn.att_fc1.weight, b1=t.attn.att_fc1.bias,
-                             w2=t.attn.att_fc2.weight.view(-1), b2=t.attn.att_fc2.bias, user=T[i, R:], a=w["ta"][i], e=None))
         ops.user_encoder_fwd_multi(encs, pool_mask, pool_use_mask, B, H)
-        if M:
-            ws, bs = [lin.weight for lin in self.transform], [lin.bias for lin in self.transform]
-            sw, sb = _const_stride(ws), _const_stride(bs)
-            if sw is not None and sb is not None:
-                ops.sgemm_nt(T, ws[0], bs[0], TP, R + B, D, D, M, (R + B) * D, sw, sb, (R + B) * D)
-            else:
-                for i in range(M):
-                    ops.sgemm_nt(T[i], ws[i], bs[i], TP[i], R + B, D, D, 1, 0, 0, 0, 0)
+        if side is not None:
+            main.wait_stream(side)
         ops.kd_loss(news, w["user"], label, T if M else None, TP if M else None, M, B, H, K, D, temperature, coef,
                     want_grad, w["score"], w["losses"], w["d_news"], w["d_user"], G if M else None)
         if want_grad:
@@ -411,6 +405,30 @@
         self.last = w
         return w
 
+    def _teacher_forward(self, T, TP, th_list, tc_list, adopted, mask, use_mask, w, B, H, K, D):
+        M, R = len(th_list), B * (H + K)
+        encs = []
+        for i in range(M):
+            if not adopted:
+                T[i, :B * H].copy_(th_list[i].reshape(B * H, D))
+                T[i, B * H:R].copy_(tc_list[i].reshape(B * K, D))
+            t = self.teachers[i]
+            tv, t_mask, t_use_mask = T[i, :B * H], mask, use_mask
+            if self.nrms:
+                nb = w.setdefault("nrms", [dict() for _ in range(1 + M)])
+                fr = nrms_self_attention(t.multi_head_self_attn, t.pad_doc, tv, mask, use_mask, B, H, nb[1 + i])
+                tv, t_mask, t_use_mask = fr["ctx"], fr["pool_mask"], True
+            encs.append(dict(vecs=tv, pad_doc=t.pad_doc.view(-1), W1=t.attn.att_fc1.weight, b1=t.attn.att_fc1.bias,
+                             w2=t.attn.att_fc2.weight.view(-1), b2=t.attn.att_fc2.bias, user=T[i, R:], a=w["ta"][i], e=None))
+        ops.user_encoder_fwd_multi(encs, t_mask, t_use_mask, B, H)
+        ws, bs = [lin.weight for lin in self.transform], [lin.bias for lin in self.transform]
+        sw, sb = _const_stride(ws), _const_stride(bs)
+        if sw is not None and sb is not None:
+            ops.sgemm_nt(T, ws[0], bs[0], TP, R + B, D, D, M, (R + B) * D, sw, sb, (R + B) * D)
+        else:
+            for i in range(M):
+                ops.sgemm_nt(T[i], ws[i], bs[i], TP[i], R + B, D, D, 1, 0, 0, 0, 0)
+
     def _nrms_backward(self, w, mask, use_mask, dpad, dW1, db1, dw2, db2, B, H, D):
         fr, at, mh = w["fr"], self.ue.attn, self.ue.multi_head_self_attn
         Rh, Dh, dev = B * H, fr["ctx"].shape[1], mask.device
@@ -437,12 +455,10 @@
     def step_backward(self, g_total):
         w = self.last
         flat = self.flat
-        w["d_news"].mul_(g_total)
         if self.head_end > self.head_begin:
-            self.stage.mul_(g_total)
-            flat.grad[self.head_begin:self.head_end].add_(self.stage[:self.head_end - self.head_begin])
+            ops.axpy_dev(self.stage[:self.head_end - self.head_begin], g_total, flat.grad[self.head_begin:self.head_end])
         if self.comm_hook is None:
-            self.enc.backward(w["d_news"], flat)
+            self.enc.backward(w["d_news"], flat, g_scale=g_total)
             return
         done_to = [flat.numel]
         sent = []
@@ -477,7 +493,7 @@
                 sent.append((lo, hi))
 
         self.enc.backward(w["d_news"], flat, on_layer_done=layer_done,
-                          on_grads_ready=grads_ready if getattr(self, "fine_grained_comm", True) else None)
+                          on_grads_ready=grads_ready if getattr(self, "fine_grained_comm", True) else None, g_scale=g_total)
         if done_to[0] > 0:
             self.comm_hook(flat, 0, done_to[0])
 
@@ -514,12 +530,14 @@
     def forward(ctx, anchor, state, args):
         w = state.step_forward(*args)
         ctx.state = state
+        ctx.set_materialize_grads(False)
         losses = w["losses"]
         return losses[3].clone(), losses[0].clone(), losses[1].clone(), losses[2].clone(), w["score"].clone()
 
     @staticmethod
     def backward(ctx, g_total, g_distill, g_emb, g_target, g_score):
-        ctx.state.step_backward(g_total)
+        if g_total is not None:
+            ctx.state.step_backward(g_total)
         return None, None, None
 
 
diff --git a/tiny-newsrec_b200/ops.py b/tiny-newsrec_b200/ops.py
--- a/tiny-newsrec_b200/ops.py
+++ b/tiny-newsrec_b200/ops.py
@@ -180,6 +180,21 @@
     return out
 
 
+@_timed
+def scale_cast_colsum(x, scale, y, colsum=None):
+    lib = _ready(x)
+    _chk(x, _f32, "scale_cast_colsum.x")
+    if not x.is_contiguous() or not y.is_contiguous() or x.dim() != 2 or tuple(y.shape) != tuple(x.shape):
+        raise _lib.TinyRecError("scale_cast_colsum: x and y must be contiguous 2-D tensors of one shape")
+    if scale is not None and scale.numel() != 1:
+        raise _lib.TinyRecError("scale_cast_colsum: scale must be a one-element tensor")
+    _lib.check(lib.tnr_scale_cast_colsum(_ptr(x), _ptr(_chk(scale, _f32, "scale_cast_colsum.scale") if scale is not None else None),
+                                         x.shape[0], x.shape[1], _ptr(_chk(y, _bf16, "scale_cast_colsum.y")),
+                                         _ptr(_chk(colsum, _f32, "scale_cast_colsum.colsum") if colsum is not None else None),
+                                         _stream()), "tnr_scale_cast_colsum")
+    return y
+
+
 def _chk_relbias(relpos, A, L):
     _chk(relpos, _f32, "relpos")
     if tuple(relpos.shape) != (A, 2 * L - 1) or not relpos.is_contiguous():
@@ -240,13 +255,14 @@
 
 
 @_timed
-def attnpool_bwd(x, e, Q, w2, a_in, dout, dx, du, dw2, db2, n, S):
+def attnpool_bwd(x, e, Q, w2, a_in, dout, dx, du, dw2, db2, n, S, db1=None):
     lib = _ready(x)
     C = x.shape[1]
     _lib.check(lib.tnr_attnpool_bwd(_ptr(x), _ptr(e), e.stride(0), Q, _ptr(w2), _ptr(_chk(a_in, _f32, "a_in")),
                                     _ptr(_chk(dout, _f32, "dout")), _ptr(_chk(dx, _bf16, "dx")),
                                     _ptr(_chk(du, _bf16, "du")), _ptr(_chk(dw2, _f32, "dw2")),
-                                    _ptr(_chk(db2, _f32, "db2")), n, S, C, _stream()), "tnr_attnpool_bwd")
+                                    _ptr(_chk(db2, _f32, "db2")), _ptr(_chk(db1, _f32, "db1") if db1 is not None else None),
+                                    n, S, C, _stream()), "tnr_attnpool_bwd")
 
 
 @_timed
@@ -254,6 +270,16 @@
     lib = _ready(x)
     _lib.check(lib.tnr_cast_f32_bf16(_ptr(_chk(x, _f32, "cast.x")), _ptr(_chk(y, _bf16, "cast.y")), x.numel(),
                                      _stream()), "tnr_cast_f32_bf16")
+    return y
+
+
+@_timed
+def axpy_dev(x, scale, y):
+    lib = _ready(x)
+    if x.numel() != y.numel() or scale.numel() != 1 or not x.is_contiguous() or not y.is_contiguous():
+        raise _lib.TinyRecError("axpy_dev: x, y contiguous of one size, scale one element")
+    _lib.check(lib.tnr_axpy_dev(_ptr(_chk(x, _f32, "axpy.x")), _ptr(_chk(scale, _f32, "axpy.scale")),
+                                _ptr(_chk(y, _f32, "axpy.y")), x.numel(), _stream()), "tnr_axpy_dev")
     return y
 
 
diff --git a/tiny-newsrec_b200/post_train.py b/tiny-newsrec_b200/post_train.py
--- a/tiny-newsrec_b200/post_train.py
+++ b/tiny-newsrec_b200/post_train.py
@@ -127,13 +127,10 @@
 
     def step_backward(self, g_total):
         w, flat = self.last, self.flat
-        w["d_news"].mul_(g_total)
-        w["d_user"].mul_(g_total)
         if self.head_end > self.head_begin:
-            self.stage.mul_(g_total)
-            flat.grad[self.head_begin:self.head_end].add_(self.stage[:self.head_end - self.head_begin])
-        self.enc.backward(w["d_news"], flat, ws=w["ws_title"])
-        self.enc.backward(w["d_user"], flat, ws=w["ws_body"])
+            ops.axpy_dev(self.stage[:self.head_end - self.head_begin], g_total, flat.grad[self.head_begin:self.head_end])
+        self.enc.backward(w["d_news"], flat, ws=w["ws_title"], g_scale=g_total)
+        self.enc.backward(w["d_user"], flat, ws=w["ws_body"], g_scale=g_total)
 
 
 class _DistillFn(torch.autograd.Function):
```

Measured after the change: 4742, median of 6. Within noise of the previous version (-1.6%).
